# underdoc-wang/STC-GNN

Measured on AMD Instinct MI355X. Metric: STC-GNN fwd+bwd samples/sec at N=50k,C=32; SpMM HBM GB/s vs peak, 1/8 GPU, higher is better.
Workload: dtype f32; 1 GPU; full STC-GNN train step (fwd + ComboLoss + bwd + grad all-reduce + Adam), csr-fixed, 224x224 queen grid N=50176 nnz=398724, C=32, hidden=16, K=2, layers=2, T=18+6; global_batch=8, batch_per_gpu=8, parallelism=batch-shard x1, operand_format=f16x2, grad_bucket_bytes=88132, grad_large_bytes=0, input_seeds=X, Y: Bernoulli(0.1635), torch seed 1000 + rank

## Files before the change

### include/stc_hip.h

```cpp
#ifndef STC_HIP_H
#define STC_HIP_H

#include <stddef.h>
#include <stdint.h>

#ifdef __cplusplus
extern "C" {
#endif

#define STC_ABI_VERSION 37
#define STC_MAX_K 4

#define STC_FMT_BF16X3 0
#define STC_FMT_F16X2 1
#define STC_ACT_AMAX_SLOTS 256

#define STC_OK 0
#define STC_EINVAL (-1)
#define STC_EALIGN (-2)
#define STC_ELIMIT (-3)
#define STC_EUNSUPPORTED (-4)

int stc_version(void);
const char* stc_last_error(void);
int stc_set_dispatch_level(int32_t level);

int stc_csr_spmm_f32(const int32_t* rowptr, const int32_t* colidx, const float* val,
                     int32_t n_rows, int32_t n_cols,
                     const float* X, const float* Y0, float* Y,
                     int32_t batch, int32_t F, float alpha, float beta, void* stream);

#define STC_SPMM_BLOCK_ROWS 4
int stc_bcsr_spmm_f32(const int32_t* blk_ptr, const int32_t* blk_cols, const float* blk_vals,
                      int32_t n_rows, int32_t n_cols,
                      const float* X, const float* Y0, float* Y,
                      int32_t batch, int32_t F, float alpha, float beta, void* stream);

#define STC_PATCH_ROWS 32
#define STC_PATCH_MAX_SRC 64
#define STC_PATCH_MAX_WIDTH 32
int stc_patch_spmm_f32(const int32_t* patch_src, const int32_t* patch_rows, const int32_t* patch_cnt,
                       const uint8_t* patch_idx, const float* patch_val, int32_t n_patches, int32_t width,
                       int32_t n_rows, int32_t n_cols, const float* X, const float* Y0, float* Y,
                       int32_t batch, int32_t F, float alpha, float beta, void* stream);

int stc_csr_spmm_bf16(const int32_t* rowptr, const int32_t* colidx, const float* val,
                      int32_t n_rows, int32_t n_cols,
                      const void* X, const void* Y0, void* Y,
                      int32_t batch, int32_t F, float alpha, float beta, void* stream);
int stc_bcsr_spmm_bf16(const int32_t* blk_ptr, const int32_t* blk_cols, const float* blk_vals,
                       int32_t n_rows, int32_t n_cols,
                       const void* X, const void* Y0, void* Y,
                       int32_t batch, int32_t F, float alpha, float beta, void* stream);

int stc_patch_spmm_bf16(const int32_t* patch_src, const int32_t* patch_rows, const int32_t* patch_cnt,
                        const uint8_t* patch_idx, const float* patch_val, int32_t n_patches, int32_t width,
                        int32_t n_rows, int32_t n_cols, const void* X, const void* Y0, void* Y,
                        int32_t batch, int32_t F, float alpha, float beta, void* stream);

#define STC_RING2_INTERIOR 32
#define STC_RING2_FIRST 64
#define STC_RING2_SECOND 96
#define STC_RING2_WIDTH 8
int stc_ring2_sum_f32(const int32_t* l2_rows, const int32_t* l1_rows, const int32_t* int_rows, const int32_t* t1, const int32_t* t2,
                      int32_t n_patches, int32_t n_rows,
                      const float* A, const float* A2, int32_t n_add, const float* const* add,
                      const float* U, const float* Cand, float* Y, float* Z,
                      int32_t batch, int32_t C, int32_t h, void* stream);
int stc_ring2_blend_f32(const int32_t* l2_rows, const int32_t* l1_rows, const int32_t* int_rows, const int32_t* t1, const int32_t* t2,
                        int32_t n_patches, int32_t n_rows,
                        const float* Bm, const float* A, const float* U, const float* H,
                        float* Cand, float* Hnew, float* SHnew,
                        int32_t batch, int32_t C, int32_t h, void* stream);
int stc_ring2_blend_first_f32(const int32_t* l2_rows, const int32_t* l1_rows, const int32_t* int_rows, const int32_t* t1, const int32_t* t2,
                              int32_t n_patches, int32_t n_rows,
                              const float* Bm, const float* A, const float* U,
                              float* Cand, float* Hnew, float* SHnew,
                              int32_t batch, int32_t C, int32_t h, void* stream);
int stc_ring2_chain_f32(const int32_t* l2_rows, const int32_t* l1_rows, const int32_t* int_rows, const int32_t* t1, const int32_t* t2,
                        int32_t n_patches, int32_t n_rows,
                        const float* A, const float* A2, float alpha1, int32_t n_add1, const float* const* add1, float* V,
                        float alpha2, int32_t n_add0, const float* const* add0, const float* scale0, float* Z,
                        int32_t batch, int32_t C, int32_t h, void* stream);

int stc_bdg_node_bf16_supported(int32_t Ks, int32_t Kc, int32_t C, int32_t L, int32_t Ho);
int stc_bdg_node_fwd_bf16(const void* const* Z, int32_t Ks, const float* Tc, int32_t Kc,
                          const float* W, const float* bias, void* Y,
                          int64_t nodes, int32_t C, int32_t L, int32_t Lw, int32_t Ho, void* stream);
int stc_bdg_node_bwd_bf16(const void* const* Z, int32_t Ks, const float* Tc, int32_t Kc,
                          const float* W, const void* dY,
                          void* const* dZ, float* dW, float* db,
                          void* workspace, size_t workspace_bytes,
                          int64_t nodes, int32_t C, int32_t L, int32_t Lw, int32_t Ho, void* stream);

int stc_cell_planar_bf16_supported(int32_t Ks, int32_t Kc, int32_t C, int32_t h);
int stc_cell_gates_fwd_planar_bf16(const void* X, const void* H, const void* SX, const void* SH,
                                   const float* Tc, const float* W, const float* bias,
                                   void* U, void* Rg, void* RH,
                                   const float* Wc, const float* bc, void* A, void* Bm,
                                   int64_t nodes, int32_t C, int32_t Lw, int32_t h, void* stream);
int stc_cell_gates_bwd_planar_bf16(const void* X, const void* H, const void* SX, const void* SH,
                                   const float* Tc, const float* W,
                                   const void* dCandIn, const void* Cand, const void* U, const void* Rg, const void* dHnew,
                                   void* const* dZ, float* dW, float* db, void* dH,
                                   void* workspace, size_t workspace_bytes,
                                   int64_t nodes, int32_t C, int32_t Lw, int32_t h, void* stream);
int stc_cell_bwd_planar_bf16_supported(int32_t C, int32_t Lw, int32_t h);
int stc_cell_bwd_planar_bf16(const void* X, const void* H, const void* SX, const void* SH,
                             const float* Tc, const float* Wg, const float* Wc,
                             const void* U, const void* Rg, const void* Cand, const void* dHnew, const void* dBm,
                             void* dX, void* dSX, void* dH, void* dSH,
                             float* dWg, float* dbg, float* dWc, float* dbc,
                             void* workspace, size_t workspace_bytes,
                             int64_t nodes, int32_t C, int32_t Lw, int32_t h, void* stream);
int stc_bdg_node_post_bwd_bf16(const void* X, const void* X2, const float* Tc, const float* W, const void* dA, const void* dB,
                               void* dX, void* dX2, float* dW, float* db, void* workspace, size_t workspace_bytes,
                               int64_t nodes, int32_t C, int32_t Lw, int32_t Ho, void* stream);
int stc_spmm_blend_fwd_bf16(const int32_t* rowptr, const int32_t* colidx, const float* val,
                            const int32_t* blk_ptr, const int32_t* blk_cols, const float* blk_vals,
                            int32_t n_rows, int32_t n_cols, const void* Bm, const void* A,
                            const void* U, const void* H, void* Cand, void* Hnew,
                            int32_t batch, int32_t C, int32_t h, void* stream);
int stc_spmm_sum_bf16(const int32_t* rowptr, const int32_t* colidx, const float* val,
                      const int32_t* blk_ptr, const int32_t* blk_cols, const float* blk_vals,
                      int32_t n_rows, int32_t n_cols, const void* X, const void* X2,
                      int32_t n_add, const void* const* add,
                      void* Y, const void* U, const void* Cand, void* dY,
                      int32_t batch, int32_t C, int32_t h, void* stream);
int stc_gru_blend_bwd_bf16(const void* dHnew, const void* U, const void* Cand, void* dCpre, int64_t n, void* stream);
int stc_head_fwd_bf16(const void* H, const float* w, const float* b, float* y, int64_t rows, int32_t h, void* stream);
int stc_head_bwd_bf16(const void* H, const float* w, const float* y, const float* dy, void* dH, float* dwb,
                      void* workspace, size_t workspace_bytes, int64_t rows, int32_t h, void* stream);

int stc_dense_agg_f32(const float* S, int32_t n_rows, int32_t n_cols, const float* X, const float* Y0, float* Y,
                      int32_t batch, int32_t F, float alpha, float beta, void* stream);

int stc_csr_sddmm_f32(const int32_t* rowptr, const int32_t* colidx,
                      int32_t n_rows, int32_t n_cols,
                      const float* A, const float* Bm, float* out,
                      int32_t batch, int32_t F, float alpha, int32_t accumulate, void* stream);

int stc_cheby_dense_fwd_f32(const float* G, int32_t n, int32_t K, float* T, void* stream);
int stc_cheby_dense_bwd_f32(const float* G, const float* T, float* dT, int32_t n, int32_t K,
                            float* dG, void* stream);

int stc_bdg_node_fwd_f32(const float* const* Z, int32_t Ks, const float* Tc, int32_t Kc,
                         const float* W, const float* bias, float* Y,
                         int64_t nodes, int32_t C, int32_t L, int32_t Lw, int32_t Ho, void* stream);

size_t stc_bdg_node_bwd_workspace_bytes(int32_t Ks, int32_t Kc, int32_t C, int32_t L, int32_t Ho,
                                        int32_t want_dTc);
int stc_bdg_node_bwd_f32(const float* const* Z, int32_t Ks, const float* Tc, int32_t Kc,
                         const float* W, const float* dY,
                         float* const* dZ, float* dW, float* db, float* dTc,
                         void* workspace, size_t workspace_bytes,
                         int64_t nodes, int32_t C, int32_t L, int32_t Lw, int32_t Ho, void* stream);

int stc_gru_gates_fwd_f32(const float* G, const float* Xt, const float* H,
                          float* U, float* Rg, float* CandIn,
                          int64_t rows, int32_t cin, int32_t h, int32_t pad, void* stream);
int stc_gru_gates_bwd_f32(const float* dCandIn, const float* dU, const float* H,
// ... 45 lines not shown
                           float* copy1, int32_t copy1_ld, int32_t copy1_off,
                           int64_t nodes, int32_t C, int32_t L, int32_t Lw, int32_t h, void* stream);

int stc_cell_planar_supported(int32_t Ks, int32_t Kc, int32_t C, int32_t h);
int stc_cell_gates_fwd_planar_f32(const float* X, const float* H, const float* SX, const float* SH,
                                  const float* Tc, const float* W, const float* bias,
                                  float* U, float* Rg, float* RH,
                                  const float* Wc, const float* bc, float* A, float* Bm,
                                  int32_t operand_format,
                                  float* act_amax,
                                  int64_t nodes, int32_t C, int32_t Lw, int32_t h, void* stream);
int stc_cell_gates_bwd_planar_f32(const float* X, const float* H, const float* SX, const float* SH,
                                  const float* Tc, const float* W,
                                  const float* dCandIn, const float* Cand, const float* U, const float* Rg, const float* dHnew,
                                  float* const* dZ, float* dW, float* db, float* dH,
                                  int32_t operand_format,
                                  const float* act_amax,
                                  void* workspace, size_t workspace_bytes,
                                  int64_t nodes, int32_t C, int32_t Lw, int32_t h, void* stream);

int stc_cell_bwd_planar_supported(int32_t C, int32_t h);
size_t stc_cell_bwd_planar_workspace_bytes(int32_t C, int32_t Lw, int32_t h);
int stc_cell_bwd_planar_f32(const float* X, const float* H, const float* SX, const float* SH,
                            const float* Tc, const float* Wg, const float* Wc,
                            const float* U, const float* Rg, const float* Cand, const float* dHnew, const float* dBm,
                            float* dX, float* dSX, float* dH, float* dSH,
                            float* dWg, float* dbg, float* dWc, float* dbc,
                            int32_t accumulate_x, int32_t accumulate_h,
                            int32_t operand_format, const float* act_amax,
                            void* workspace, size_t workspace_bytes,
                            int64_t nodes, int32_t C, int32_t Lw, int32_t h, void* stream);

int stc_cell_first_supported(int32_t C, int32_t h);
int stc_cell_gates_fwd_first_f32(const float* X, const float* SX, const float* Tc, const float* W, const float* bias, float* U,
                                 const float* Wc, const float* bc, float* A, float* Bm,
                                 int32_t operand_format, float* act_amax,
                                 int64_t nodes, int32_t C, int32_t Lw, int32_t h, void* stream);
size_t stc_cell_bwd_first_workspace_bytes(int32_t C, int32_t Lw, int32_t h);
int stc_cell_bwd_first_f32(const float* X, const float* SX, const float* Tc, const float* Wg, const float* Wc,
                           const float* U, const float* Cand, const float* dHnew, const float* dBm,
                           float* dX, float* dSX, float* dWg, float* dbg, float* dWc, float* dbc,
                           int32_t accumulate_x, int32_t operand_format, const float* act_amax,
                           void* workspace, size_t workspace_bytes,
                           int64_t nodes, int32_t C, int32_t Lw, int32_t h, void* stream);

int stc_cell_planar_k_supported(int32_t K, int32_t C, int32_t h);
int stc_cell_gates_fwd_planar_k_f32(const float* const* Zx, const float* const* Zh, int32_t K, const float* Tc, const float* W, const float* bias,
                                    float* U, float* Rg, float* RH, int32_t operand_format,
                                    float* act_amax,
                                    int64_t nodes, int32_t C, int32_t Lw, int32_t h, void* stream);
int stc_cell_cand_fwd_planar_k_f32(const float* const* Zx, const float* const* Zh, int32_t K, const float* Tc, const float* W, const float* bias,
                                   const float* U, const float* H, float* Cand, float* Hnew, int32_t operand_format, float* act_amax,
                                   int64_t nodes, int32_t C, int32_t Lw, int32_t h, void* stream);
int stc_cell_gates_bwd_planar_k_f32(const float* const* Zx, const float* const* Zh, int32_t K, const float* Tc, const float* W,
                                    const float* dRH, const float* Cand, const float* U, const float* Rg, const float* dHnew,
                                    float* const* dZx, float* const* dZh, float* dW, float* db, float* dH, int32_t accumulate_x,
                                    int32_t operand_format,
                                    const float* act_amax,
                                    void* workspace, size_t workspace_bytes, int64_t nodes, int32_t C, int32_t Lw, int32_t h, void* stream);
int stc_cell_cand_bwd_planar_k_f32(const float* const* Zx, const float* const* Zh, int32_t K, const float* Tc, const float* W,
                                   const float* dHnew, const float* U, const float* Cand,
                                   float* const* dZx, float* const* dZh, float* dW, float* db,
                                   int32_t operand_format,
                                   const float* act_amax,
                                   void* workspace, size_t workspace_bytes, int64_t nodes, int32_t C, int32_t Lw, int32_t h, void* stream);

#define STC_SPMM_SUM_MAX_ADD 8
#define STC_SPMM_SUM_BF16_MAX_ADD 5
#define STC_RING2_MAX_ADD 5
int stc_spmm_sum_f32(const int32_t* rowptr, const int32_t* colidx, const float* val,
                     const int32_t* blk_ptr, const int32_t* blk_cols, const float* blk_vals,
                     int32_t n_rows, int32_t n_cols, const float* X, const float* X2, float alpha,
                     int32_t n_add, const float* const* add, const int32_t* add_ld, const int32_t* add_off, const float* add_scale,
                     float* Y, const float* U, const float* Cand, float* dY,
                     float* amax, int32_t n_amax,
                     int32_t batch, int32_t C, int32_t h, void* stream);

int stc_head_fwd_f32(const float* H, const float* w, const float* b, float* y,
                     int64_t rows, int32_t h, void* stream);
size_t stc_head_bwd_workspace_bytes(int32_t h);
int stc_head_bwd_f32(const float* H, const float* w, const float* y, const float* dy,
                     float* dH, float* dwb, void* workspace, size_t workspace_bytes,
                     int64_t rows, int32_t h, void* stream);

int stc_cell_small_supported(int32_t Ks, int32_t Kc, int32_t C, int32_t cin, int32_t h);
size_t stc_cell_small_workspace_bytes(int32_t n_nodes, int32_t C, int32_t cin, int32_t batch, int32_t Ks);
int stc_cell_small_param_rows(void);
int stc_cell_small_fwd_f32(const int32_t* rowptr, const int32_t* colidx, const float* val, int32_t n_nodes, int32_t nnz,
                           int32_t graph_is_dense, const int32_t* rowptr2, const int32_t* colidx2, const float* val2, int32_t nnz2,
                           const float* X, int32_t cin, const float* H, const float* Tc, int32_t Ks, int32_t Kc,
                           const float* Wg, const float* bg, const float* Wc, const float* bc,
                           float* U, float* R, float* Cand, float* Hnew, float* RH, float* Zg, float* Zc, float* Zg2, float* Zc2, float* Z0,
                           float* Z0c, float* Z1c, float* Z2c, int32_t phase, int32_t splits, int32_t batch, int32_t C, void* stream);
int stc_cell_small_bwd_f32(const int32_t* rowptr, const int32_t* colidx, const float* val, int32_t n_nodes, int32_t nnz,
                           int32_t graph_is_dense, const int32_t* rowptr2, const int32_t* colidx2, const float* val2, int32_t nnz2,
                           const float* X, int32_t cin, const float* H, const float* Tc, int32_t Ks, int32_t Kc,
                           const float* Wg, const float* Wc, const float* U, const float* R, const float* Cand,
                           const float* RH, const float* Zg, const float* Zc, const float* Zg2, const float* Zc2, const float* dHnew,
                           float* dX, int32_t accumulate_x, float* dH, int32_t accumulate_h,
                           float* dparams, int64_t params_ld, int32_t has_bg, int32_t has_bc,
                           float* dZ1c, float* dZ1g, float* dYg, float* dYc, float* dZ2c, float* dZ2g,
                           void* workspace, size_t workspace_bytes, int32_t phase, int32_t splits, int32_t batch, int32_t C, void* stream);

int stc_graph_grad_f32(const float* A, const float* B, double* partials, int32_t n_chunks, int32_t cell0, int32_t cell_step, int32_t n_sel,
                       int32_t batch, int32_t N, int32_t F, int64_t chunk_stride, void* stream);
int stc_mix_grad_f32(const float* A, const float* B, double* partials, int32_t n_chunks, int32_t cell0, int32_t cell_step, int32_t n_sel,
                     int32_t batch, int32_t N, int32_t Fa, int32_t Fb, int64_t chunk_stride, void* stream);

int stc_mix_dt_supported(int32_t Ks, int32_t Kc, int32_t C, int32_t L, int32_t Ho);
size_t stc_mix_dt_workspace_bytes(int32_t Ks);
int stc_mix_dt_f32(const float* const* Z, int32_t Ks, const float* W, const float* dY, float* dTc, void* workspace,
                   size_t workspace_bytes, int64_t rows, int32_t C, int32_t L, int32_t Lw, int32_t Ho, void* stream);

size_t stc_mixed_fusion_workspace_bytes(int32_t D, int32_t want_dA);
int stc_mixed_fusion_fwd_f32(const float* WA, const float* bA, const float* WP, const float* bP, const float* A, const float* P,
                             float* gate, float* G, int32_t D, void* stream);
int stc_mixed_fusion_bwd_f32(const float* WA, const float* WP, const float* A, const float* P, const float* gate, const float* dG,
                             float* dWA, float* dWP, float* db, float* dP, float* dA,
                             void* workspace, size_t workspace_bytes, int32_t D, void* stream);
int stc_mgp_uv_fwd_f32(const float* X, int64_t k_stride, int64_t r_stride, int64_t f_stride, const float* Wu, const float* Wv, float alpha,
                       float* U, float* V, int32_t K, int32_t R, int32_t F, int32_t h, void* stream);
int stc_mgp_uv_bwd_f32(const float* X, int64_t k_stride, int64_t r_stride, int64_t f_stride, const float* U, const float* V,
                       const float* dU, const float* dV, float alpha, float* partials, int32_t K, int32_t R, int32_t F, int32_t h, void* stream);
int stc_mgp_softmax_fwd_f32(const float* P, float* Ps, int32_t R, void* stream);
int stc_mgp_softmax_bwd_f32(const float* P, const float* Ps, const float* dPs, float* rowdot, float* dP, int32_t R, void* stream);
int stc_adam_f32(float* p, const float* g, float* m, float* v, int64_t n, const float* step, double lr, double beta1, double beta2, double eps,
                 double weight_decay, void* stream);


int stc_axpy_f32(float a, const float* x, float* y, int64_t n, void* stream);
int stc_concat2_f32(const float* A, const float* B, float* out,
                    int64_t rows, int32_t a, int32_t b, int32_t pad, void* stream);
int stc_split2_f32(const float* src, const float* addA, const float* addB, float* A, float* B,
                   int64_t rows, int32_t a, int32_t b, int32_t pad, int32_t addA_ld,
                   const float* addA2, const float* addB2, void* stream);

#ifdef __cplusplus
}
#endif
#endif
```

### stc-gnn_amd/STC_GNN.py

```python
from __future__ import annotations

from typing import List, Optional, Sequence, Union

import torch
from torch import nn

from stc_hip import ops
from stc_hip.graph import CsrGraph, SpatialOperand, csr_operand, dense_operand

GraphLike = Union[torch.Tensor, CsrGraph, 'GraphPair']


class GraphPair:

    def __init__(self, Gs, Gc: torch.Tensor, Ks: int, Kc: int):
        if isinstance(Gs, CsrGraph):
            self.spatial: SpatialOperand = csr_operand(Gs, Gc.device)
        elif isinstance(Gs, torch.Tensor) and Gs.layout != torch.strided:
            self.spatial = csr_operand(_as_csr_graph(Gs), Gc.device)
        elif isinstance(Gs, torch.Tensor):
            self.spatial = dense_operand(Gs)
        else:
            raise TypeError(f'Gs must be a tensor or a CsrGraph, got {type(Gs).__name__}')
        self.Ks, self.Kc = Ks, Kc
# ... 196 lines not shown
        params = nn.ParameterDict()
        for key in ('Wu', 'Wv'):
            params[key] = nn.Parameter(torch.randn(in_dim, hidden_dim))
        for p in params.values():
            nn.init.xavier_normal_(p)
        return params

    def _learned(self, X: torch.Tensor, params, rows_axis: int) -> torch.Tensor:
        reduce = None
        if self.batch_sharded:
            from stc_hip.dist import allreduce_sum
            reduce = allreduce_sum
        if ops.mgp_front_supported(X, params['Wu'], params['Wv']):
            return ops.mgp_front(X, params['Wu'], params['Wv'], rows_axis, float(self.alpha), reduce)
        if rows_axis == 3:
            X = X.transpose(2, 3)
        U = torch.tanh(self.alpha * torch.matmul(X, params['Wu']))
        V = torch.tanh(self.alpha * torch.matmul(X, params['Wv']))
        flat_u, flat_v = U.flatten(0, 1), V.flatten(0, 1)
        P = torch.einsum('knh,kmh->nm', flat_u, flat_v)
        if reduce is not None:
            P = reduce(P)
        return torch.softmax(torch.relu(P - P.t()), dim=-1)

    def forward(self, X_seq: torch.Tensor, As: torch.Tensor, Ac: torch.Tensor):
        Gs = self.aggreg_S(As, self._learned(X_seq, self.params_S, 2))
        Gc = self.aggreg_C(Ac, self._learned(X_seq, self.params_C, 3))
        return Gs, Gc


class STCGNN(nn.Module):

    def __init__(self, num_nodes: int, num_categories: int, Ks: int, Kc: int, input_dim: int, hidden_dim: int,
                 num_layers: int, out_horizon: int, use_bias=True, activation=None,
                 graph_mode: str = 'dense-learned', reorder_nodes: bool = True, batch_sharded: bool = False,
                 fusion_rank: Optional[int] = None, storage_dtype: torch.dtype = torch.float32):
        super().__init__()
        if graph_mode not in ('dense-learned', 'csr-fixed'):
            raise ValueError("graph_mode must be 'dense-learned' (reference semantics) or 'csr-fixed'")
        if storage_dtype not in (torch.float32, torch.bfloat16):
            raise ValueError('storage_dtype must be torch.float32 (reference arithmetic) or torch.bfloat16')
        if storage_dtype == torch.bfloat16 and graph_mode != 'csr-fixed':
            raise ValueError("storage_dtype=torch.bfloat16 needs graph_mode='csr-fixed' (BASELINE configuration 5)")
        self.storage_dtype = storage_dtype
        self.graph_mode = graph_mode
        self.reorder_nodes = reorder_nodes
        self.Ks, self.Kc = Ks, Kc
        if graph_mode == 'dense-learned':
            self.mix_graph_pair = MGP_Gen(num_nodes, num_categories, hidden_dim, fusion_rank=fusion_rank)
            self.mix_graph_pair.batch_sharded = batch_sharded
        self.encoder = STC_Encoder(num_nodes, num_categories, Ks, Kc, input_dim, hidden_dim, num_layers,
                                   use_bias, activation, return_all_layers=True)
        self.decoder = STC_Decoder(num_nodes, num_categories, Ks, Kc, hidden_dim, hidden_dim, num_layers,
                                   out_horizon, use_bias, activation)
        self.out_proj = nn.Sequential(nn.Linear(hidden_dim, hidden_dim // 2, bias=use_bias),
                                      nn.Linear(hidden_dim // 2, input_dim, bias=use_bias))

    def prepare_graph(self, graph: CsrGraph, device=None) -> CsrGraph:
        g = graph.with_locality()[0] if self.reorder_nodes else graph
        if device is not None:
            g.on(torch.device(device))
        return graph

    def forward(self, X_seq: torch.Tensor, As: GraphLike, Ac: torch.Tensor):
        assert X_seq.dim() == 4, 'STC-GNN must take in 4D tensor as input X_seq'
        inv = None
        if self.graph_mode == 'dense-learned':
            Gs, Gc = self.mix_graph_pair(X_seq, As, Ac)
        else:
            Gs, Gc = As, Ac
            if isinstance(Gs, torch.Tensor) and Gs.layout != torch.strided:
                Gs = _as_csr_graph(Gs)
            if self.reorder_nodes and isinstance(Gs, CsrGraph):
                Gs, order = Gs.with_locality()
                if order is not None:
                    idx = getattr(Gs, '_order_dev', {}).get(X_seq.device)
                    if idx is None:
                        o = torch.from_numpy(order).to(X_seq.device)
                        idx = (o, torch.argsort(o))
                        Gs._order_dev = {**getattr(Gs, '_order_dev', {}), X_seq.device: idx}
                    X_seq = X_seq.index_select(2, idx[0])
                    inv = idx[1]
        pair = _graphs(Gs, Gc, self.Ks, self.Kc)
        stacked = self._run_cell_graph(pair, X_seq.unsqueeze(-1).to(self.storage_dtype))
        if stacked is None and self.storage_dtype != torch.float32:
            raise ValueError('storage_dtype=torch.bfloat16: shape outside the bf16 cell kernels (Ks = Kc = 2, hidden 16, C in {32, 64}, input_dim <= 4)')
        if stacked is not None:
            y = self._head(stacked).transpose(0, 1)
        else:
            _, states = self.encoder._run(pair, None, X_seq.unsqueeze(-1))
            step_in = states[-1]
            outs = []
            for _ in range(self.decoder.out_horizon):
                step_in, states = self.decoder(pair, None, step_in, states)
                outs.append(step_in)
            y = self._head(torch.stack(outs, dim=1))
        return y if inv is None else y.index_select(2, inv)

    def _run_cell_graph(self, pair: GraphPair, X: torch.Tensor):
        enc, dec = self.encoder.cell_list, self.decoder.cell_list
        cells = list(enc) + list(dec)
        hidden = {c.hidden_dim for c in cells}
        if len(hidden) != 1 or any(c.gates.activation is not None or c.candi.activation is not None for c in cells):
            return None
        h = hidden.pop()
        B, T, N, C, cin0 = X.shape
        if X.requires_grad or not ops.cell_graph_supported(pair.spatial, pair.Tc, self.Ks, C, h, [cin0, h], dtype=X.dtype):
            return None
        n_layers, horizon = len(enc), self.decoder.out_horizon
        if ops.first_step_route(pair.spatial, pair.Tc, self.Ks, C, h, [cin0, h], dtype=X.dtype):
            ext = [X[:, t] for t in range(T)] + [ops.zero_state(c.gates.W, (B, c.num_nodes, c.num_categories, c.hidden_dim), X.dtype) for c in enc]
        else:
            ext = [X[:, t] for t in range(T)] + [c.init_hidden(B).to(X.dtype) for c in enc]
        eid = lambda l, t: l * T + t
        did = lambda l, s_: n_layers * T + s_ * n_layers + l
        schedule = []
        for l in range(n_layers):
            for t in range(T):
                x = ('ext', t) if l == 0 else ('cell', eid(l - 1, t))
                hs = ('ext', T + l) if t == 0 else ('cell', eid(l, t - 1))
                schedule.append((l, x, hs))
        for s_ in range(horizon):
            for l in range(n_layers):
                top_prev = eid(n_layers - 1, T - 1) if s_ == 0 else did(n_layers - 1, s_ - 1)
                x = ('cell', top_prev) if l == 0 else ('cell', did(l - 1, s_))
                hs = ('cell', eid(l, T - 1) if s_ == 0 else did(l, s_ - 1))
                schedule.append((n_layers + l, x, hs))
        stacks = [(c.gates.W, c.gates.b if c.gates.use_bias else None, c.candi.W, c.candi.b if c.candi.use_bias else None) for c in cells]
        outputs = [did(n_layers - 1, s_) for s_ in range(horizon)]
        return ops.stc_cell_graph(pair.spatial, pair.Tc, self.Ks, schedule, outputs, ext, stacks)

    def _head(self, H: torch.Tensor) -> torch.Tensor:
        lin1, lin2 = self.out_proj[0], self.out_proj[1]
        h = lin1.in_features
        if lin2.out_features != 1 or h % 4 or h > 64 or (H.dtype == torch.bfloat16 and h != 16):
            return torch.sigmoid(self.out_proj(H.float())).squeeze(dim=-1)
        w = (lin2.weight @ lin1.weight).reshape(h)
        if lin1.bias is not None:
            b = lin2.weight @ lin1.bias + lin2.bias
        else:
            b = w.new_zeros(1)
        return ops.head(H, w, b)
```

### stc-gnn_amd/csrc/stc_common.h

```cpp
#pragma once
#include <hip/hip_runtime.h>

#include <atomic>
#include <cstdarg>
#include <cstdint>
#include <cstdio>

#include "stc_hip.h"

namespace stc {

char* error_buffer();

inline int fail(int code, const char* fmt, ...) {
    va_list ap;
    va_start(ap, fmt);
    vsnprintf(error_buffer(), 512, fmt, ap);
    va_end(ap);
    return code;
}

inline int hip_status(hipError_t e, const char* what) {
    if (e == hipSuccess) return STC_OK;
    snprintf(error_buffer(), 512, "%s: %s", what, hipGetErrorString(e));
// ... 3 lines not shown
inline bool aligned16(const void* p) { return (reinterpret_cast<uintptr_t>(p) & 15u) == 0; }

constexpr int kNumXcd = 8;
constexpr int kNumCu = 256;
constexpr int kWave = 64;
constexpr size_t kMaxLdsBytes = 160 * 1024;

template <typename K>
inline hipError_t allow_lds(K kernel, size_t bytes) {
    if (bytes <= 48 * 1024) return hipSuccess;
    return hipFuncSetAttribute(reinterpret_cast<const void*>(kernel),
                               hipFuncAttributeMaxDynamicSharedMemorySize, (int)bytes);
}

constexpr int kMaxGrantDevices = 16;
struct Grants { std::atomic<size_t> per_device[kMaxGrantDevices]; };
template <class K>
inline hipError_t allow_lds_once(K kern, size_t bytes, Grants& grants) {
    int dev = -1;
    if (hipGetDevice(&dev) != hipSuccess) dev = -1;
    std::atomic<size_t>* granted = dev >= 0 && dev < kMaxGrantDevices ? &grants.per_device[dev] : nullptr;
    if (granted && bytes <= granted->load(std::memory_order_relaxed)) return hipSuccess;
    const hipError_t e = allow_lds(kern, bytes);
    if (e == hipSuccess && granted) granted->store(bytes, std::memory_order_relaxed);
    return e;
}

template <typename K>
inline int resident_blocks(K kernel, int threads, size_t lds, int fallback_per_cu = 1) {
    int per_cu = 0, dev = 0, cus = kNumCu;
    bool failed = false;
    if (hipOccupancyMaxActiveBlocksPerMultiprocessor(&per_cu, kernel, threads, lds) != hipSuccess || per_cu < 1) {
        per_cu = fallback_per_cu;
        failed = true;
    }
    if (hipGetDevice(&dev) == hipSuccess) {
        int v = 0;
        if (hipDeviceGetAttribute(&v, hipDeviceAttributeMultiprocessorCount, dev) == hipSuccess && v > 0) cus = v;
        else failed = true;
    } else {
        failed = true;
    }
    if (failed) (void)hipGetLastError();
    return per_cu * cus;
}

#define STC_REQUIRE(cond, code, ...) \
    do {                             \
        if (!(cond)) return ::stc::fail(code, __VA_ARGS__); \
    } while (0)

#define STC_LAUNCH_CHECK(what) \
    do {                        \
        hipError_t e__ = hipGetLastError(); \
        if (e__ != hipSuccess) return ::stc::hip_status(e__, what); \
    } while (0)

}

__device__ __forceinline__ int stc_xcd_tile(int bid, int n_tiles) {
    const int per = (n_tiles + stc::kNumXcd - 1) / stc::kNumXcd;
    const int tile = (bid % stc::kNumXcd) * per + bid / stc::kNumXcd;
    return tile < n_tiles && (bid / stc::kNumXcd) < per ? tile : -1;
}

template <class T>
__device__ __forceinline__ T stc_ld_once(const T* p) { return __builtin_nontemporal_load(p); }
template <class T>
__device__ __forceinline__ void stc_st_once(T* p, const T& v) { __builtin_nontemporal_store(v, p); }

__device__ __forceinline__ float stc_sigmoid(float v) {
    return __builtin_amdgcn_rcpf(1.f + __builtin_amdgcn_exp2f(-1.4426950408889634f * v));
}
__device__ __forceinline__ float stc_tanh(float v) {
    const float big = 1.f - 2.f * __builtin_amdgcn_rcpf(1.f + __builtin_amdgcn_exp2f(2.8853900817779268f * v));
    const float t = v * v;
    float p = fmaf(t, 62.f / 2835.f, -17.f / 315.f);
    p = fmaf(p, t, 2.f / 15.f);
    p = fmaf(p, t, -1.f / 3.f);
    const float small = fmaf(p * t, v, v);
    return fabsf(v) < 0.25f ? small : big;
}

__device__ __forceinline__ float stc_wave_sum(float v) {
#pragma unroll
    for (int off = 32; off > 0; off >>= 1) v += __shfl_xor(v, off, 64);
    return v;
}
```

### stc-gnn_amd/csrc/stc_gates.hip

```cpp
#include "stc_common.h"

#include <initializer_list>

namespace {

constexpr int EW_THREADS = 256;

inline dim3 ew_grid(long long n) {
    long long blocks = (n + EW_THREADS - 1) / EW_THREADS;
    const long long cap = (long long)stc::kNumCu * 8;
    return dim3((unsigned)(blocks < cap ? (blocks > 0 ? blocks : 1) : cap));
}

__device__ __forceinline__ float sigmoidf_(float x) { return 1.f / (1.f + expf(-x)); }

__global__ __launch_bounds__(EW_THREADS) void gru_gates_fwd_kernel(
    const float* __restrict__ G, const float* __restrict__ Xt, const float* __restrict__ H,
    float* __restrict__ U, float* __restrict__ Rg, float* __restrict__ CandIn,
    long long rows, int cin, int h, int pad) {
    const int L = cin + h + pad;
    const long long n = rows * L;
    for (long long e = (long long)blockIdx.x * EW_THREADS + threadIdx.x; e < n; e += (long long)gridDim.x * EW_THREADS) {
        const long long r = e / L;
        const int l = (int)(e - r * L);
        if (l < cin) {
            CandIn[e] = Xt[r * cin + l];
        } else if (l >= cin + h) {
            CandIn[e] = 0.f;
        } else {
            const int k = l - cin;
            const float u = sigmoidf_(G[r * 2 * h + k]);
            const float g = sigmoidf_(G[r * 2 * h + h + k]);
            U[r * h + k] = u;
            Rg[r * h + k] = g;
            CandIn[e] = g * H[r * h + k];
        }
    }
}

__global__ __launch_bounds__(EW_THREADS) void gru_gates_bwd_kernel(
    const float* __restrict__ dCandIn, const float* __restrict__ dU, const float* __restrict__ H,
    const float* __restrict__ U, const float* __restrict__ Rg, const float* dH_in,
    float* __restrict__ dG, float* __restrict__ dXt, float* dH,
    long long rows, int cin, int h, int pad) {
    const int L = cin + h + pad;
    const long long n = rows * L;
    for (long long e = (long long)blockIdx.x * EW_THREADS + threadIdx.x; e < n; e += (long long)gridDim.x * EW_THREADS) {
        const long long r = e / L;
        const int l = (int)(e - r * L);
        if (l < cin) {
            dXt[r * cin + l] = dCandIn[e];
        } else if (l < cin + h) {
            const int k = l - cin;
            const long long i = r * h + k;
            const float u = U[i], g = Rg[i], d = dCandIn[e];
            dG[r * 2 * h + k] = dU[i] * u * (1.f - u);
            dG[r * 2 * h + h + k] = d * H[i] * g * (1.f - g);
            dH[i] = dH_in ? fmaf(d, g, dH_in[i]) : d * g;
        }
    }
}

__global__ __launch_bounds__(EW_THREADS) void gru_blend_fwd_kernel(
    const float* __restrict__ Cpre, const float* __restrict__ U, const float* __restrict__ H,
    float* __restrict__ Cand, float* __restrict__ Hnew, long long n) {
    for (long long e = (long long)blockIdx.x * EW_THREADS + threadIdx.x; e < n; e += (long long)gridDim.x * EW_THREADS) {
        const float c = tanhf(Cpre[e]);
        const float u = U[e];
        Cand[e] = c;
        Hnew[e] = (1.f - u) * H[e] + u * c;
    }
}

__global__ __launch_bounds__(EW_THREADS) void gru_blend_bwd_kernel(
    const float* __restrict__ dHnew, const float* __restrict__ U, const float* __restrict__ H,
    const float* __restrict__ Cand, float* __restrict__ dCpre, float* __restrict__ dU, float* __restrict__ dH,
    long long n) {
    for (long long e = (long long)blockIdx.x * EW_THREADS + threadIdx.x; e < n; e += (long long)gridDim.x * EW_THREADS) {
        const float g = dHnew[e], u = U[e], c = Cand[e];
        dCpre[e] = g * u * (1.f - c * c);
        if (dU) dU[e] = g * (c - H[e]);
        if (dH) dH[e] = g * (1.f - u);
    }
}


__device__ __forceinline__ float4 sig4(float4 x) { return make_float4(sigmoidf_(x.x), sigmoidf_(x.y), sigmoidf_(x.z), sigmoidf_(x.w)); }
__device__ __forceinline__ float4 mul4(float4 a, float4 b) { return make_float4(a.x * b.x, a.y * b.y, a.z * b.z, a.w * b.w); }

__global__ __launch_bounds__(EW_THREADS) void gru_gates_fwd_vec_kernel(
    const float4* __restrict__ G, const float4* __restrict__ Xt, const float4* __restrict__ H,
    float4* __restrict__ U, float4* __restrict__ Rg, float4* __restrict__ CandIn,
    long long rows, int cin4, int h4, int pad4) {
    const int L4 = cin4 + h4 + pad4;
    const long long n = rows * L4;
    for (long long e = (long long)blockIdx.x * EW_THREADS + threadIdx.x; e < n; e += (long long)gridDim.x * EW_THREADS) {
        const long long r = e / L4;
// ... 79 lines not shown
}

__device__ __forceinline__ float4 add4(float4 a, float4 b) { return make_float4(a.x + b.x, a.y + b.y, a.z + b.z, a.w + b.w); }

__global__ __launch_bounds__(EW_THREADS) void split2_vec_kernel(const float4* __restrict__ src, const float4* addA, const float4* addB,
                                                                 float4* A, float4* B, long long rows, int a4, int b4, int pad4, int ldA4,
                                                                 const float4* addA2, const float4* addB2) {
    const int L4 = a4 + b4 + pad4;
    const long long n = rows * L4;
    for (long long e = (long long)blockIdx.x * EW_THREADS + threadIdx.x; e < n; e += (long long)gridDim.x * EW_THREADS) {
        const long long r = e / L4;
        const int l = (int)(e - r * L4);
        if (l < a4) {
            if (A) {
                const long long i = r * a4 + l;
                float4 v = addA ? add4(src[e], addA[r * ldA4 + l]) : src[e];
                if (addA2) v = add4(v, addA2[i]);
                A[i] = v;
            }
        } else if (l < a4 + b4) {
            if (B) {
                const long long i = r * b4 + (l - a4);
                float4 v = addB ? add4(src[e], addB[i]) : src[e];
                if (addB2) v = add4(v, addB2[i]);
                B[i] = v;
            }
        }
    }
}

inline bool vec_ok(std::initializer_list<const void*> ptrs, std::initializer_list<long long> widths) {
    for (const void* p : ptrs)
        if (p && !stc::aligned16(p)) return false;
    for (long long w : widths)
        if (w % 4) return false;
    return true;
}
#define F4C(p) reinterpret_cast<const float4*>(p)
#define F4M(p) reinterpret_cast<float4*>(p)

constexpr int HEAD_MAX_H = 64;
constexpr int HEAD_PARTS = 1024;

template <int LPR>
__global__ __launch_bounds__(EW_THREADS) void head_fwd_kernel(const float* __restrict__ H, const float* __restrict__ w,
                                                               const float* __restrict__ b, float* __restrict__ y,
                                                               long long rows, int h) {
    constexpr int RPB = EW_THREADS / LPR;
    const int h4 = h / 4, q = threadIdx.x % LPR;
    float4 wq = make_float4(0.f, 0.f, 0.f, 0.f);
    if (q < h4) wq = reinterpret_cast<const float4*>(w)[q];
    const float bias = b[0];
    for (long long r = (long long)blockIdx.x * RPB + threadIdx.x / LPR; r < rows; r += (long long)gridDim.x * RPB) {
        float s = 0.f;
        if (q < h4) {
            const float4 v = reinterpret_cast<const float4*>(H + r * h)[q];
            s = fmaf(v.x, wq.x, fmaf(v.y, wq.y, fmaf(v.z, wq.z, v.w * wq.w)));
        }
#pragma unroll
        for (int off = LPR / 2; off > 0; off >>= 1) s += __shfl_xor(s, off, 64);
        if (q == 0) y[r] = sigmoidf_(s + bias);
    }
}

template <int LPR>
__global__ __launch_bounds__(EW_THREADS) void head_bwd_kernel(const float* __restrict__ H, const float* __restrict__ w,
                                                               const float* __restrict__ y, const float* __restrict__ dy,
                                                               float* __restrict__ dH, float* __restrict__ partial,
                                                               long long rows, int h) {
    constexpr int RPB = EW_THREADS / LPR;
    __shared__ float red[EW_THREADS][5];
    const int h4 = h / 4, q = threadIdx.x % LPR;
    float4 wq = make_float4(0.f, 0.f, 0.f, 0.f);
    if (q < h4) wq = reinterpret_cast<const float4*>(w)[q];
    float4 acc = make_float4(0.f, 0.f, 0.f, 0.f);
    float accg = 0.f;
    for (long long r = (long long)blockIdx.x * RPB + threadIdx.x / LPR; r < rows; r += (long long)gridDim.x * RPB) {
        const float yy = y[r];
        const float g = dy[r] * yy * (1.f - yy);
        if (q == 0) accg += g;
        if (q < h4) {
            const float4 v = reinterpret_cast<const float4*>(H + r * h)[q];
            reinterpret_cast<float4*>(dH + r * h)[q] = make_float4(g * wq.x, g * wq.y, g * wq.z, g * wq.w);
            acc.x = fmaf(g, v.x, acc.x); acc.y = fmaf(g, v.y, acc.y); acc.z = fmaf(g, v.z, acc.z); acc.w = fmaf(g, v.w, acc.w);
        }
    }
    red[threadIdx.x][0] = acc.x; red[threadIdx.x][1] = acc.y; red[threadIdx.x][2] = acc.z; red[threadIdx.x][3] = acc.w;
    red[threadIdx.x][4] = accg;
    __syncthreads();
    if ((int)threadIdx.x <= h) {
        const int k = threadIdx.x;
        const int lane_q = k < h ? k / 4 : 0, comp = k < h ? k % 4 : 4;
        float v = 0.f;
        for (int t = lane_q; t < EW_THREADS; t += LPR) v += red[t][comp];
        partial[(size_t)blockIdx.x * (h + 1) + k] = v;
    }
}

using head_u4 = __attribute__((ext_vector_type(4))) unsigned;
using head_bf2 = __attribute__((ext_vector_type(2))) __bf16;
__device__ __forceinline__ void head_unpack8(const head_u4 v, float (&r)[8]) {
#pragma unroll
    for (int i = 0; i < 4; ++i) { r[2 * i] = __uint_as_float(v[i] << 16); r[2 * i + 1] = __uint_as_float(v[i] & 0xffff0000u); }
}
__device__ __forceinline__ unsigned head_pk(float a, float b) {
    const head_bf2 v = {(__bf16)a, (__bf16)b};
    return __builtin_bit_cast(unsigned, v);
}

__global__ __launch_bounds__(EW_THREADS) void head_fwd_bf16_kernel(const head_u4* __restrict__ H, const float* __restrict__ w,
                                                                    const float* __restrict__ b, float* __restrict__ y, long long rows) {
    constexpr int RPB = EW_THREADS / 2;
    const int q = threadIdx.x & 1;
    float wq[8];
#pragma unroll
    for (int i = 0; i < 8; ++i) wq[i] = w[8 * q + i];
    const float bias = b[0];
    for (long long r = (long long)blockIdx.x * RPB + threadIdx.x / 2; r < rows; r += (long long)gridDim.x * RPB) {
        float v[8];
        head_unpack8(H[2 * r + q], v);
        float s = 0.f;
#pragma unroll
        for (int i = 0; i < 8; ++i) s = fmaf(v[i], wq[i], s);
        s += __shfl_xor(s, 1, 64);
        if (q == 0) y[r] = sigmoidf_(s + bias);
    }
}

__global__ __launch_bounds__(EW_THREADS) void head_bwd_bf16_kernel(const head_u4* __restrict__ H, const float* __restrict__ w,
                                                                    const float* __restrict__ y, const float* __restrict__ dy,
                                                                    head_u4* __restrict__ dH, float* __restrict__ partial, long long rows) {
    constexpr int RPB = EW_THREADS / 2, h = 16;
    __shared__ float red[EW_THREADS][9];
    const int q = threadIdx.x & 1;
    float wq[8], acc[8], accg = 0.f;
#pragma unroll
    for (int i = 0; i < 8; ++i) { wq[i] = w[8 * q + i]; acc[i] = 0.f; }
    for (long long r = (long long)blockIdx.x * RPB + threadIdx.x / 2; r < rows; r += (long long)gridDim.x * RPB) {
        const float yy = y[r];
        const float g = dy[r] * yy * (1.f - yy);
        if (q == 0) accg += g;
        float v[8];
        head_unpack8(H[2 * r + q], v);
        dH[2 * r + q] = head_u4{head_pk(g * wq[0], g * wq[1]), head_pk(g * wq[2], g * wq[3]), head_pk(g * wq[4], g * wq[5]), head_pk(g * wq[6], g * wq[7])};
#pragma unroll
        for (int i = 0; i < 8; ++i) acc[i] = fmaf(g, v[i], acc[i]);
    }
#pragma unroll
    for (int i = 0; i < 8; ++i) red[threadIdx.x][i] = acc[i];
    red[threadIdx.x][8] = accg;
    __syncthreads();
    if ((int)threadIdx.x <= h) {
        const int k = threadIdx.x;
        const int lane_q = k < h ? k / 8 : 0, comp = k < h ? k % 8 : 8;
        float v = 0.f;
        for (int t = lane_q; t < EW_THREADS; t += 2) v += red[t][comp];
        partial[(size_t)blockIdx.x * (h + 1) + k] = v;
    }
}

__global__ __launch_bounds__(EW_THREADS) void head_reduce_kernel(const float* __restrict__ partial, int n_parts, int stride, float* __restrict__ out) {
    __shared__ float red[EW_THREADS];
    const int e = blockIdx.x;
    float s = 0.f;
    for (int p = threadIdx.x; p < n_parts; p += EW_THREADS) s += partial[(size_t)p * stride + e];
    red[threadIdx.x] = s;
// ... 107 lines not shown
        hipLaunchKernelGGL(gru_gates_fwd_kernel, ew_grid(n), dim3(EW_THREADS), 0, s, G, Xt, H, U, Rg, CandIn, (long long)rows, cin, h, pad);
    STC_LAUNCH_CHECK("stc_gru_gates_fwd_f32 launch");
    return STC_OK;
}

extern "C" int stc_gru_gates_bwd_f32(const float* dCandIn, const float* dU, const float* H, const float* U, const float* Rg,
                                     const float* dH_in, float* dG, float* dXt, float* dH,
                                     int64_t rows, int32_t cin, int32_t h, int32_t pad, void* stream) {
    STC_REQUIRE(cin >= 0 && h >= 1 && pad >= 0, STC_EINVAL, "stc_gru_gates_bwd_f32: bad widths cin=%d h=%d pad=%d", cin, h, pad);
    STC_EW_PROLOGUE("stc_gru_gates_bwd_f32", rows, dCandIn && dU && H && U && Rg && dG && dH && (cin == 0 || dXt));
    const long long n = (long long)rows * (cin + h + pad);
    if (vec_ok({dCandIn, dU, H, U, Rg, dH_in, dG, dXt, dH}, {cin, h, pad}))
        hipLaunchKernelGGL(gru_gates_bwd_vec_kernel, ew_grid(n / 4), dim3(EW_THREADS), 0, s, F4C(dCandIn), F4C(dU), F4C(H), F4C(U), F4C(Rg),
                           F4C(dH_in), F4M(dG), F4M(dXt), F4M(dH), (long long)rows, cin / 4, h / 4, pad / 4);
    else
        hipLaunchKernelGGL(gru_gates_bwd_kernel, ew_grid(n), dim3(EW_THREADS), 0, s, dCandIn, dU, H, U, Rg, dH_in, dG, dXt, dH, (long long)rows, cin, h, pad);
    STC_LAUNCH_CHECK("stc_gru_gates_bwd_f32 launch");
    return STC_OK;
}

extern "C" int stc_gru_blend_fwd_f32(const float* Cpre, const float* U, const float* H, float* Cand, float* Hnew,
                                     int64_t n, void* stream) {
    STC_EW_PROLOGUE("stc_gru_blend_fwd_f32", n, Cpre && U && H && Cand && Hnew);
    if (vec_ok({Cpre, U, H, Cand, Hnew}, {n}))
        hipLaunchKernelGGL(gru_blend_fwd_vec_kernel, ew_grid(n / 4), dim3(EW_THREADS), 0, s, F4C(Cpre), F4C(U), F4C(H), F4M(Cand), F4M(Hnew), (long long)n / 4);
    else
        hipLaunchKernelGGL(gru_blend_fwd_kernel, ew_grid(n), dim3(EW_THREADS), 0, s, Cpre, U, H, Cand, Hnew, (long long)n);
    STC_LAUNCH_CHECK("stc_gru_blend_fwd_f32 launch");
    return STC_OK;
}

extern "C" int stc_gru_blend_bwd_f32(const float* dHnew, const float* U, const float* H, const float* Cand,
                                     float* dCpre, float* dU, float* dH, int64_t n, void* stream) {
    STC_EW_PROLOGUE("stc_gru_blend_bwd_f32", n, dHnew && U && Cand && dCpre && (H || !dU));
    if (vec_ok({dHnew, U, H, Cand, dCpre, dU, dH}, {n}))
        hipLaunchKernelGGL(gru_blend_bwd_vec_kernel, ew_grid(n / 4), dim3(EW_THREADS), 0, s, F4C(dHnew), F4C(U), F4C(H), F4C(Cand), F4M(dCpre), F4M(dU),
                           F4M(dH), (long long)n / 4);
    else
        hipLaunchKernelGGL(gru_blend_bwd_kernel, ew_grid(n), dim3(EW_THREADS), 0, s, dHnew, U, H, Cand, dCpre, dU, dH, (long long)n);
    STC_LAUNCH_CHECK("stc_gru_blend_bwd_f32 launch");
    return STC_OK;
}


extern "C" int stc_head_fwd_f32(const float* H, const float* w, const float* b, float* y, int64_t rows, int32_t h, void* stream) {
    STC_REQUIRE(h >= 4 && h <= HEAD_MAX_H && h % 4 == 0, STC_ELIMIT, "stc_head_fwd_f32: h=%d must be a multiple of 4 in [4,%d]", h, HEAD_MAX_H);
    STC_EW_PROLOGUE("stc_head_fwd_f32", rows, H && w && b && y);
    STC_REQUIRE(stc::aligned16(H), STC_EALIGN, "stc_head_fwd_f32: H not 16-byte aligned");
    STC_REQUIRE(stc::aligned16(w), STC_EALIGN, "stc_head_fwd_f32: w not 16-byte aligned");
    const int h4 = h / 4;
#define STC_HEAD_FWD(LPR_) hipLaunchKernelGGL(head_fwd_kernel<LPR_>, ew_grid(rows * LPR_), dim3(EW_THREADS), 0, s, H, w, b, y, (long long)rows, h)
    if (h4 <= 1) STC_HEAD_FWD(1); else if (h4 <= 2) STC_HEAD_FWD(2); else if (h4 <= 4) STC_HEAD_FWD(4); else if (h4 <= 8) STC_HEAD_FWD(8); else STC_HEAD_FWD(16);
#undef STC_HEAD_FWD
    STC_LAUNCH_CHECK("stc_head_fwd_f32 launch");
    return STC_OK;
}

extern "C" size_t stc_head_bwd_workspace_bytes(int32_t h) { return h < 1 ? 0 : (size_t)HEAD_PARTS * (h + 1) * sizeof(float); }

extern "C" int stc_head_bwd_f32(const float* H, const float* w, const float* y, const float* dy, float* dH, float* dwb,
                                void* workspace, size_t workspace_bytes, int64_t rows, int32_t h, void* stream) {
    STC_REQUIRE(h >= 4 && h <= HEAD_MAX_H && h % 4 == 0, STC_ELIMIT, "stc_head_bwd_f32: h=%d must be a multiple of 4 in [4,%d]", h, HEAD_MAX_H);
    STC_REQUIRE(rows >= 0 && dwb, STC_EINVAL, "stc_head_bwd_f32: negative rows or null dwb");
    hipStream_t s = static_cast<hipStream_t>(stream);
    if (rows == 0) return stc::hip_status(hipMemsetAsync(dwb, 0, (size_t)(h + 1) * sizeof(float), s), "memset dwb");
    STC_REQUIRE(H && w && y && dy && dH, STC_EINVAL, "stc_head_bwd_f32: null pointer");
    STC_REQUIRE(stc::aligned16(H) && stc::aligned16(dH) && workspace && stc::aligned16(workspace), STC_EALIGN,
                "stc_head_bwd_f32: H/dH/workspace must be 16-byte aligned");
    STC_REQUIRE(workspace_bytes >= stc_head_bwd_workspace_bytes(h), STC_EINVAL, "stc_head_bwd_f32: workspace too small");
    STC_REQUIRE(stc::aligned16(w), STC_EALIGN, "stc_head_bwd_f32: w not 16-byte aligned");
    const int h4 = h / 4;
    const int lpr = h4 <= 1 ? 1 : h4 <= 2 ? 2 : h4 <= 4 ? 4 : h4 <= 8 ? 8 : 16;
    long long blocks = (rows * lpr + EW_THREADS - 1) / EW_THREADS;
    const int grid = (int)(blocks < HEAD_PARTS ? blocks : HEAD_PARTS);
    float* partial = static_cast<float*>(workspace);
#define STC_HEAD_BWD(LPR_) hipLaunchKernelGGL(head_bwd_kernel<LPR_>, dim3(grid), dim3(EW_THREADS), 0, s, H, w, y, dy, dH, partial, (long long)rows, h)
    if (lpr == 1) STC_HEAD_BWD(1); else if (lpr == 2) STC_HEAD_BWD(2); else if (lpr == 4) STC_HEAD_BWD(4); else if (lpr == 8) STC_HEAD_BWD(8); else STC_HEAD_BWD(16);
#undef STC_HEAD_BWD
    hipLaunchKernelGGL(head_reduce_kernel, dim3(h + 1), dim3(EW_THREADS), 0, s, partial, grid, h + 1, dwb);
    STC_LAUNCH_CHECK("stc_head_bwd_f32 launch");
    return STC_OK;
}

extern "C" int stc_head_fwd_bf16(const void* H, const float* w, const float* b, float* y, int64_t rows, int32_t h, void* stream) {
    STC_REQUIRE(h == 16, STC_EUNSUPPORTED, "stc_head_fwd_bf16: hidden width %d (built for 16)", h);
    STC_EW_PROLOGUE("stc_head_fwd_bf16", rows, H && w && b && y);
    STC_REQUIRE(stc::aligned16(H), STC_EALIGN, "stc_head_fwd_bf16: H not 16-byte aligned");
    hipLaunchKernelGGL(head_fwd_bf16_kernel, ew_grid(rows * 2), dim3(EW_THREADS), 0, s, static_cast<const head_u4*>(H), w, b, y, (long long)rows);
    STC_LAUNCH_CHECK("stc_head_fwd_bf16 launch");
    return STC_OK;
}

extern "C" int stc_head_bwd_bf16(const void* H, const float* w, const float* y, const float* dy, void* dH, float* dwb,
                                 void* workspace, size_t workspace_bytes, int64_t rows, int32_t h, void* stream) {
    STC_REQUIRE(h == 16, STC_EUNSUPPORTED, "stc_head_bwd_bf16: hidden width %d (built for 16)", h);
    STC_REQUIRE(rows >= 0 && dwb, STC_EINVAL, "stc_head_bwd_bf16: negative rows or null dwb");
    hipStream_t s = static_cast<hipStream_t>(stream);
    if (rows == 0) return stc::hip_status(hipMemsetAsync(dwb, 0, (size_t)(h + 1) * sizeof(float), s), "memset dwb");
    STC_REQUIRE(H && w && y && dy && dH, STC_EINVAL, "stc_head_bwd_bf16: null pointer");
    STC_REQUIRE(stc::aligned16(H) && stc::aligned16(dH) && workspace && stc::aligned16(workspace), STC_EALIGN,
                "stc_head_bwd_bf16: H/dH/workspace must be 16-byte aligned");
    STC_REQUIRE(workspace_bytes >= stc_head_bwd_workspace_bytes(h), STC_EINVAL, "stc_head_bwd_bf16: workspace too small");
    long long blocks = (rows * 2 + EW_THREADS - 1) / EW_THREADS;
    const int grid = (int)(blocks < HEAD_PARTS ? blocks : HEAD_PARTS);
    float* partial = static_cast<float*>(workspace);
    hipLaunchKernelGGL(head_bwd_bf16_kernel, dim3(grid), dim3(EW_THREADS), 0, s, static_cast<const head_u4*>(H), w, y, dy,
                       static_cast<head_u4*>(dH), partial, (long long)rows);
    hipLaunchKernelGGL(head_reduce_kernel, dim3(h + 1), dim3(EW_THREADS), 0, s, partial, grid, h + 1, dwb);
    STC_LAUNCH_CHECK("stc_head_bwd_bf16 launch");
    return STC_OK;
}

extern "C" int stc_axpy_f32(float a, const float* x, float* y, int64_t n, void* stream) {
    STC_EW_PROLOGUE("stc_axpy_f32", n, x && y);
    hipLaunchKernelGGL(axpy_kernel, ew_grid(n), dim3(EW_THREADS), 0, s, a, x, y, (long long)n);
    STC_LAUNCH_CHECK("stc_axpy_f32 launch");
    return STC_OK;
}

extern "C" int stc_concat2_f32(const float* A, const float* B, float* out, int64_t rows, int32_t a, int32_t b, int32_t pad, void* stream) {
    STC_REQUIRE(a >= 0 && b >= 0 && pad >= 0, STC_EINVAL, "stc_concat2_f32: negative width");
    const long long n = (long long)rows * (a + b + pad);
    STC_EW_PROLOGUE("stc_concat2_f32", n, out && (a == 0 || A) && (b == 0 || B));
    if (vec_ok({A, B, out}, {a, b, pad}))
        hipLaunchKernelGGL(concat2_vec_kernel, ew_grid(n / 4), dim3(EW_THREADS), 0, s, F4C(A), F4C(B), F4M(out), (long long)rows, a / 4, b / 4, pad / 4);
    else
        hipLaunchKernelGGL(concat2_kernel, ew_grid(n), dim3(EW_THREADS), 0, s, A, B, out, (long long)rows, a, b, pad);
    STC_LAUNCH_CHECK("stc_concat2_f32 launch");
    return STC_OK;
}

extern "C" int stc_split2_f32(const float* src, const float* addA, const float* addB, float* A, float* B,
                              int64_t rows, int32_t a, int32_t b, int32_t pad, int32_t addA_ld,
                              const float* addA2, const float* addB2, void* stream) {
    STC_REQUIRE(a >= 0 && b >= 0 && pad >= 0, STC_EINVAL, "stc_split2_f32: negative width");
    STC_REQUIRE(addA_ld == 0 || addA_ld >= a, STC_EINVAL, "stc_split2_f32: addA_ld=%d is smaller than the width a=%d", addA_ld, a);
    const int ldA = addA_ld ? addA_ld : a;
    const long long n = (long long)rows * (a + b + pad);
    STC_EW_PROLOGUE("stc_split2_f32", n, src && (A || B));
    if (vec_ok({src, addA, addB, A, B, addA2, addB2}, {a, b, pad, ldA}))
        hipLaunchKernelGGL(split2_vec_kernel, ew_grid(n / 4), dim3(EW_THREADS), 0, s, F4C(src), F4C(addA), F4C(addB), F4M(A), F4M(B),
                           (long long)rows, a / 4, b / 4, pad / 4, ldA / 4, F4C(addA2), F4C(addB2));
    else
        hipLaunchKernelGGL(split2_kernel, ew_grid(n), dim3(EW_THREADS), 0, s, src, addA, addB, A, B, (long long)rows, a, b, pad, ldA, addA2, addB2);
    STC_LAUNCH_CHECK("stc_split2_f32 launch");
    return STC_OK;
}

extern "C" int stc_cheby_dense_fwd_f32(const float* G, int32_t n, int32_t K, float* T, void* stream) {
    STC_REQUIRE(n >= 1 && n <= 128 && K >= 1 && K <= STC_MAX_K, STC_ELIMIT, "stc_cheby_dense_fwd_f32: n=%d (<=128) K=%d (<=%d)", n, K, STC_MAX_K);
    STC_REQUIRE(G && T, STC_EINVAL, "stc_cheby_dense_fwd_f32: null pointer");
    hipStream_t s = static_cast<hipStream_t>(stream);
    const int nn = n * n;
    const dim3 grid((nn + EW_THREADS - 1) / EW_THREADS), block(EW_THREADS);
    hipLaunchKernelGGL(cheby_init_kernel, grid, block, 0, s, G, n, K, T);
    for (int k = 2; k < K; ++k)
        hipLaunchKernelGGL(cheby_step_kernel, grid, block, 0, s, G, T + (size_t)(k - 1) * nn, T + (size_t)(k - 2) * nn, T + (size_t)k * nn, n);
    STC_LAUNCH_CHECK("stc_cheby_dense_fwd_f32 launch");
    return STC_OK;
}

extern "C" int stc_cheby_dense_bwd_f32(const float* G, const float* T, float* dT, int32_t n, int32_t K, float* dG, void* stream) {
    STC_REQUIRE(n >= 1 && n <= 128 && K >= 1 && K <= STC_MAX_K, STC_ELIMIT, "stc_cheby_dense_bwd_f32: n=%d (<=128) K=%d (<=%d)", n, K, STC_MAX_K);
    STC_REQUIRE(G && T && dT && dG, STC_EINVAL, "stc_cheby_dense_bwd_f32: null pointer");
    hipStream_t s = static_cast<hipStream_t>(stream);
    const int nn = n * n;
// ... 24 lines not shown
```

### stc-gnn_amd/csrc/stc_spmm_ring2.hip

```cpp
#include "stc_spmm_host.h"

namespace {

constexpr int R2_THREADS = 256, R2_WAVES = R2_THREADS / 64;
constexpr int R2_INT = STC_RING2_INTERIOR;
constexpr int R2_L1 = STC_RING2_FIRST;
constexpr int R2_L2 = STC_RING2_SECOND;
constexpr int R2_W = STC_RING2_WIDTH;
constexpr int R2_Q = 32;
constexpr int R2_STAGE = R2_L2 / (2 * R2_WAVES);
constexpr int R2_S1 = R2_L1 / (2 * R2_WAVES);
constexpr int R2_S2 = R2_INT / (2 * R2_WAVES);
constexpr int R2_MAX_ADD = STC_RING2_MAX_ADD;

using v4f = __attribute__((ext_vector_type(4))) float;

struct Ring2Plan {
    const int32_t *l2_rows, *l1_rows, *int_rows;
    const int32_t *t1, *t2;
    int n_patches;
};

struct Ring2Args {
    Ring2Plan pl;
    const v4f *A, *A2;
    const v4f* add[R2_MAX_ADD];
    int n_add;
    const v4f *U, *Cand;
    v4f *Y, *Y2, *Z;
    int n, F4;
    float alpha1, alpha2;
    const v4f* add0[R2_MAX_ADD];
    float scale0[R2_MAX_ADD];
};

enum { R2_SUM = 0, R2_BLEND = 1, R2_CHAIN = 2, R2_BLEND0 = 3 };

__device__ __forceinline__ void lds_only_barrier() { asm volatile("s_waitcnt lgkmcnt(0)\n\ts_barrier" ::: "memory"); }

template <int MODE, bool HAS_A2, int NADD, int N0 = 0>
__global__ __launch_bounds__(R2_THREADS, 2) void ring2_sum_kernel(Ring2Args a) {
    static_assert((MODE != R2_BLEND && MODE != R2_BLEND0) || (NADD == 1 && !HAS_A2), "the blend forms: one addend (A), one gathered operand (Bm)");
    static_assert((MODE == R2_CHAIN) == (N0 > 0), "interior addends: the chain form, at least one");
    extern __shared__ __attribute__((aligned(16))) unsigned char lds[];
    v4f* tile = reinterpret_cast<v4f*>(lds);
    int2* tab1 = reinterpret_cast<int2*>(lds + (size_t)R2_L2 * R2_Q * 16);
    int2* tab2 = tab1 + R2_L1 * R2_W;

    const int p = stc_xcd_tile(blockIdx.x, a.pl.n_patches);
    if (p < 0) return;
    const int b = blockIdx.y;
    const int tid = threadIdx.x, lane = tid & 63, half = lane >> 5, q = lane & 31;
    const int wave = __builtin_amdgcn_readfirstlane(tid >> 6);
    const int hw = wave * 2 + half;
    const int n_chunks = a.F4 / R2_Q;

    for (int e = tid; e < R2_L1 * R2_W; e += R2_THREADS) tab1[e] = reinterpret_cast<const int2*>(a.pl.t1)[(size_t)p * R2_L1 * R2_W + e];
    for (int e = tid; e < R2_INT * R2_W; e += R2_THREADS) tab2[e] = reinterpret_cast<const int2*>(a.pl.t2)[(size_t)p * R2_INT * R2_W + e];

    int stage_row[R2_STAGE], l1_row[R2_S1], in_row[R2_S2];
#pragma unroll
    for (int k = 0; k < R2_STAGE; ++k) stage_row[k] = a.pl.l2_rows[(size_t)p * R2_L2 + k * 8 + hw];
#pragma unroll
    for (int i = 0; i < R2_S1; ++i) l1_row[i] = a.pl.l1_rows[(size_t)p * R2_L1 + i * 8 + hw];
#pragma unroll
    for (int i = 0; i < R2_S2; ++i) in_row[i] = a.pl.int_rows[(size_t)p * R2_INT + i * 8 + hw];

    const unsigned base = (unsigned)b * (unsigned)a.n * (unsigned)a.F4 + (unsigned)q;
    unsigned stage_off[R2_STAGE], l1_off[R2_S1];
#pragma unroll
    for (int k = 0; k < R2_STAGE; ++k) stage_off[k] = base + (unsigned)stage_row[k] * (unsigned)a.F4;
#pragma unroll
    for (int i = 0; i < R2_S1; ++i) l1_off[i] = base + (unsigned)(l1_row[i] >= 0 ? (l1_row[i] & 0x3FFFFFFF) : 0) * (unsigned)a.F4;
    v4f st[R2_STAGE];
    auto request = [&](int chunk) {
#pragma unroll
        for (int k = 0; k < R2_STAGE; ++k) {
            const unsigned at = stage_off[k] + chunk * R2_Q;
            st[k] = a.A[at];
            if (HAS_A2) st[k] += a.A2[at];
        }
    };
    constexpr int NOP = MODE == R2_CHAIN ? NADD : MODE == R2_BLEND0 ? NADD + 1 : NADD + 2, NOPA = NOP > 0 ? NOP : 1;
    auto slot_at = [&](int i, int chunk) { return l1_off[i] + (unsigned)(chunk * R2_Q); };
    auto request_slot = [&](v4f (&o)[NOPA], int i, int chunk) {
        const unsigned at = slot_at(i, chunk);
#pragma unroll
        for (int k = 0; k < NADD; ++k) o[k] = a.add[k][at];
        if constexpr (MODE != R2_CHAIN) {
            o[NADD] = a.U[at];
            if constexpr (MODE != R2_BLEND0) o[NADD + 1] = a.Cand[at];
        }
    };
    v4f opn[NOPA];
    request(0);
    request_slot(opn, 0, 0);
    for (int chunk = 0; chunk < n_chunks; ++chunk) {
        if (chunk) lds_only_barrier();
#pragma unroll
        for (int k = 0; k < R2_STAGE; ++k) tile[(k * 8 + hw) * R2_Q + q] = st[k];
        lds_only_barrier();
        const bool more = chunk + 1 < n_chunks;
        v4f dy[R2_S1];
#pragma unroll
        for (int i = 0; i < R2_S1; ++i) {
            const int slot = i * 8 + hw, row = l1_row[i];
            const bool interior = row >= 0 && (row & (1 << 30));
            v4f cur[NOPA];
#pragma unroll
            for (int k = 0; k < NOP; ++k) cur[k] = opn[k];
            if (i + 1 < R2_S1) {
                request_slot(opn, i + 1, chunk);
            } else if (more) {
                request(chunk + 1);
                request_slot(opn, 0, chunk + 1);
            }
            v4f acc = {0.f, 0.f, 0.f, 0.f};
#pragma unroll
            for (int w = 0; w < R2_W; ++w) {
                const int2 t = tab1[slot * R2_W + w];
                const v4f x = *reinterpret_cast<const v4f*>(lds + t.x + q * 16);
                const float v = __int_as_float(t.y);
#pragma unroll
                for (int c = 0; c < 4; ++c) acc[c] = fmaf(v, x[c], acc[c]);
            }
            v4f dh = MODE == R2_CHAIN ? a.alpha1 * acc : acc;
#pragma unroll
            for (int k = 0; k < NADD; ++k) dh += cur[k];
            if constexpr (MODE == R2_CHAIN) {
                if (a.Y != nullptr && interior) __builtin_nontemporal_store(dh, a.Y + slot_at(i, chunk));
                dy[i] = dh;
            } else if constexpr (MODE == R2_SUM) {
                const v4f u = cur[NOPA - 2], cd = cur[NOPA - 1];
                if (interior) __builtin_nontemporal_store(dh, a.Y + slot_at(i, chunk));
#pragma unroll
                for (int c = 0; c < 4; ++c) dy[i][c] = dh[c] * u[c] * (1.f - cd[c] * cd[c]);
            } else {
                const v4f u = cur[NADD], cd = MODE == R2_BLEND0 ? v4f{0.f, 0.f, 0.f, 0.f} : cur[NOPA - 1];
                v4f cand;
#pragma unroll
                for (int c = 0; c < 4; ++c) {
                    cand[c] = stc_tanh(dh[c]);
                    if constexpr (MODE == R2_BLEND0) dy[i][c] = u[c] * cand[c];
                    else dy[i][c] = (1.f - u[c]) * cd[c] + u[c] * cand[c];
                }
                if (interior) {
                    if (a.Y != nullptr) __builtin_nontemporal_store(cand, a.Y + slot_at(i, chunk));
                    __builtin_nontemporal_store(dy[i], a.Y2 + slot_at(i, chunk));
                }
            }
        }
        lds_only_barrier();
#pragma unroll
        for (int i = 0; i < R2_S1; ++i) tile[(i * 8 + hw) * R2_Q + q] = dy[i];
        v4f own[R2_S2][N0 > 0 ? N0 : 1];
        if constexpr (MODE == R2_CHAIN) {
#pragma unroll
            for (int i = 0; i < R2_S2; ++i)
#pragma unroll
                for (int k = 0; k < N0; ++k)
                    own[i][k] = a.add0[k][base + (unsigned)(in_row[i] >= 0 ? in_row[i] : 0) * (unsigned)a.F4 + (unsigned)(chunk * R2_Q)];
        }
        lds_only_barrier();
#pragma unroll
        for (int i = 0; i < R2_S2; ++i) {
            const int r = i * 8 + hw, row = in_row[i];
            v4f acc = {0.f, 0.f, 0.f, 0.f};
#pragma unroll
            for (int w = 0; w < R2_W; ++w) {
                const int2 t = tab2[r * R2_W + w];
                const v4f x = *reinterpret_cast<const v4f*>(lds + t.x + q * 16);
                const float v = __int_as_float(t.y);
#pragma unroll
                for (int c = 0; c < 4; ++c) acc[c] = fmaf(v, x[c], acc[c]);
            }
            if constexpr (MODE == R2_CHAIN) {
                acc *= a.alpha2;
#pragma unroll
                for (int k = 0; k < N0; ++k) acc += a.scale0[k] * own[i][k];
            }
            if (row >= 0) __builtin_nontemporal_store(acc, a.Z + (base + (unsigned)row * (unsigned)a.F4 + (unsigned)(chunk * R2_Q)));
        }
    }
}

template <int MODE, bool HAS_A2>
int launch_ring2(const Ring2Args& a, int batch, hipStream_t s, int n_add0 = 0) {
    const size_t lds = (size_t)R2_L2 * R2_Q * 16 + (size_t)(R2_L1 + R2_INT) * R2_W * sizeof(int2);
    static_assert((size_t)R2_L2 * R2_Q * 16 + (size_t)(R2_L1 + R2_INT) * R2_W * sizeof(int2) <= 64 * 1024, "within the default dynamic-LDS limit: no attribute to set");
    using Kernel = void (*)(Ring2Args);
    Kernel kern = nullptr;
    if constexpr (MODE == R2_BLEND || MODE == R2_BLEND0) {
        kern = ring2_sum_kernel<MODE, false, 1>;
    } else if constexpr (MODE == R2_CHAIN) {
        static constexpr Kernel table[3][R2_MAX_ADD] = {
#define STC_R2_ROW(NA) {ring2_sum_kernel<R2_CHAIN, HAS_A2, NA, 1>, ring2_sum_kernel<R2_CHAIN, HAS_A2, NA, 2>, ring2_sum_kernel<R2_CHAIN, HAS_A2, NA, 3>, \
                        ring2_sum_kernel<R2_CHAIN, HAS_A2, NA, 4>, ring2_sum_kernel<R2_CHAIN, HAS_A2, NA, 5>}
            STC_R2_ROW(0), STC_R2_ROW(1), STC_R2_ROW(2)};
#undef STC_R2_ROW
        kern = table[a.n_add][n_add0 - 1];
    } else {
        switch (a.n_add) {
            case 0: kern = ring2_sum_kernel<R2_SUM, HAS_A2, 0>; break;
            case 1: kern = ring2_sum_kernel<R2_SUM, HAS_A2, 1>; break;
            case 2: kern = ring2_sum_kernel<R2_SUM, HAS_A2, 2>; break;
            case 3: kern = ring2_sum_kernel<R2_SUM, HAS_A2, 3>; break;
            case 4: kern = ring2_sum_kernel<R2_SUM, HAS_A2, 4>; break;
            default: kern = ring2_sum_kernel<R2_SUM, HAS_A2, 5>; break;
        }
    }
    const int per = (a.pl.n_patches + stc::kNumXcd - 1) / stc::kNumXcd;
    hipLaunchKernelGGL(kern, dim3(per * stc::kNumXcd, batch), dim3(R2_THREADS), lds, s, a);
    return stc::launched("stc_ring2 launch");
}

int check_ring2(const char* who, const void* l2_rows, const void* l1_rows, const void* int_rows, const void* t1, const void* t2, int n_patches, int n_rows,
                int batch, int C, int h) {
    STC_REQUIRE(h == 16 && C >= 1 && (C * h) % (4 * R2_Q) == 0, STC_EUNSUPPORTED, "%s: rows of C * h = %d floats (hidden 16, whole 512-byte chunks)", who, C * h);
    STC_REQUIRE(batch <= 65535 && n_patches >= 0, STC_EINVAL, "%s: bad sizes", who);
    if (int rc = stc::check_state_rows(who, n_rows, batch, C, h, true)) return rc;
    STC_REQUIRE((long long)batch * n_rows * (C * h / 4) < (1ll << 28), STC_ELIMIT, "%s: planes of %lld 16-byte pieces (32-bit offsets: < 2^28)", who,
                (long long)batch * n_rows * (C * h / 4));
    if (batch == 0 || n_rows == 0) return STC_OK;
    STC_REQUIRE(n_patches >= 1 && (long long)n_patches * R2_INT >= n_rows, STC_EINVAL, "%s: %d patches cannot cover %d rows", who, n_patches, n_rows);
    STC_REQUIRE(l2_rows && l1_rows && int_rows && t1 && t2, STC_EINVAL, "%s: null plan array", who);
    STC_REQUIRE(reinterpret_cast<uintptr_t>(t1) % 8 == 0 && reinterpret_cast<uintptr_t>(t2) % 8 == 0, STC_EALIGN, "%s: tables must be 8-byte aligned", who);
    return STC_OK;
}

}

#if !defined(STC_RING2_FIRST_UNIT)

extern "C" int stc_ring2_sum_f32(const int32_t* l2_rows, const int32_t* l1_rows, const int32_t* int_rows, const int32_t* t1, const int32_t* t2,
                                 int32_t n_patches, int32_t n_rows,
                                 const float* A, const float* A2, int32_t n_add, const float* const* add,
                                 const float* U, const float* Cand, float* Y, float* Z,
                                 int32_t batch, int32_t C, int32_t h, void* stream) {
    if (int rc = stc::check_addend_count("stc_ring2_sum_f32", "addend", n_add, 0, R2_MAX_ADD, STC_ELIMIT)) return rc;
    if (int rc = check_ring2("stc_ring2_sum_f32", l2_rows, l1_rows, int_rows, t1, t2, n_patches, n_rows, batch, C, h)) return rc;
    if (batch == 0 || n_rows == 0) return STC_OK;
    STC_REQUIRE(A && U && Cand && Y && Z && (n_add == 0 || add), STC_EINVAL, "stc_ring2_sum_f32: null pointer");
    STC_REQUIRE(stc::aligned16(A) && (!A2 || stc::aligned16(A2)) && stc::aligned16(U) && stc::aligned16(Cand) && stc::aligned16(Y) && stc::aligned16(Z),
                STC_EALIGN, "stc_ring2_sum_f32: planes must be 16-byte aligned");
    STC_REQUIRE(Y != A && Y != A2 && Z != A && Z != A2 && Y != Z && Y != U && Y != Cand && Z != U && Z != Cand, STC_EINVAL,
                "stc_ring2_sum_f32: results must not alias the gathered operands, the first ring's gate planes or each other");
    Ring2Args a{};
    a.pl = Ring2Plan{l2_rows, l1_rows, int_rows, t1, t2, n_patches};
    a.A = reinterpret_cast<const v4f*>(A);
    a.A2 = reinterpret_cast<const v4f*>(A2);
    a.n_add = n_add;
    if (int rc = stc::check_addends("stc_ring2_sum_f32", "addend", add, n_add, Y, Z)) return rc;
    for (int i = 0; i < n_add; ++i) a.add[i] = reinterpret_cast<const v4f*>(add[i]);
    a.U = reinterpret_cast<const v4f*>(U);
    a.Cand = reinterpret_cast<const v4f*>(Cand);
    a.Y = reinterpret_cast<v4f*>(Y);
    a.Z = reinterpret_cast<v4f*>(Z);
    a.n = n_rows;
    a.F4 = C * h / 4;
    hipStream_t s = static_cast<hipStream_t>(stream);
    return A2 ? launch_ring2<R2_SUM, true>(a, batch, s) : launch_ring2<R2_SUM, false>(a, batch, s);
}

extern "C" int stc_ring2_blend_f32(const int32_t* l2_rows, const int32_t* l1_rows, const int32_t* int_rows, const int32_t* t1, const int32_t* t2,
                                   int32_t n_patches, int32_t n_rows,
                                   const float* Bm, const float* A, const float* U, const float* H,
                                   float* Cand, float* Hnew, float* SHnew,
                                   int32_t batch, int32_t C, int32_t h, void* stream) {
    if (int rc = check_ring2("stc_ring2_blend_f32", l2_rows, l1_rows, int_rows, t1, t2, n_patches, n_rows, batch, C, h)) return rc;
    if (batch == 0 || n_rows == 0) return STC_OK;
    STC_REQUIRE(Bm && A && U && H && Hnew && SHnew, STC_EINVAL, "stc_ring2_blend_f32: null pointer");
    for (const void* q : {(const void*)Bm, (const void*)A, (const void*)U, (const void*)H, (const void*)Cand, (const void*)Hnew, (const void*)SHnew})
        STC_REQUIRE(stc::aligned16(q), STC_EALIGN, "stc_ring2_blend_f32: planes must be 16-byte aligned");
    for (const float* out : {Cand, Hnew, SHnew})
        STC_REQUIRE(out != Bm && out != A && out != U && out != H, STC_EINVAL, "stc_ring2_blend_f32: a result aliases an operand (the first ring re-reads them)");
    STC_REQUIRE(Cand != Hnew && Cand != SHnew && Hnew != SHnew, STC_EINVAL, "stc_ring2_blend_f32: results alias each other");
    Ring2Args a{};
    a.pl = Ring2Plan{l2_rows, l1_rows, int_rows, t1, t2, n_patches};
    a.A = reinterpret_cast<const v4f*>(Bm);
    a.n_add = 1;
    a.add[0] = reinterpret_cast<const v4f*>(A);
    a.U = reinterpret_cast<const v4f*>(U);
    a.Cand = reinterpret_cast<const v4f*>(H);
    a.Y = reinterpret_cast<v4f*>(Cand);
    a.Y2 = reinterpret_cast<v4f*>(Hnew);
    a.Z = reinterpret_cast<v4f*>(SHnew);
    a.n = n_rows;
    a.F4 = C * h / 4;
    return launch_ring2<R2_BLEND, false>(a, batch, static_cast<hipStream_t>(stream));
}

extern "C" int stc_ring2_chain_f32(const int32_t* l2_rows, const int32_t* l1_rows, const int32_t* int_rows, const int32_t* t1, const int32_t* t2,
                                   int32_t n_patches, int32_t n_rows,
                                   const float* A, const float* A2, float alpha1, int32_t n_add1, const float* const* add1, float* V,
                                   float alpha2, int32_t n_add0, const float* const* add0, const float* scale0, float* Z,
                                   int32_t batch, int32_t C, int32_t h, void* stream) {
    if (int rc = stc::check_addend_count("stc_ring2_chain_f32", "first-ring addend", n_add1, 0, 2, STC_ELIMIT)) return rc;
    if (int rc = stc::check_addend_count("stc_ring2_chain_f32", "interior addend", n_add0, 1, R2_MAX_ADD, STC_ELIMIT)) return rc;
    if (int rc = check_ring2("stc_ring2_chain_f32", l2_rows, l1_rows, int_rows, t1, t2, n_patches, n_rows, batch, C, h)) return rc;
    if (batch == 0 || n_rows == 0) return STC_OK;
    STC_REQUIRE(A && Z && add0 && (n_add1 == 0 || add1), STC_EINVAL, "stc_ring2_chain_f32: null pointer");
    STC_REQUIRE(stc::aligned16(A) && (!A2 || stc::aligned16(A2)) && (!V || stc::aligned16(V)) && stc::aligned16(Z), STC_EALIGN,
                "stc_ring2_chain_f32: planes must be 16-byte aligned");
    STC_REQUIRE(Z != A && Z != A2 && V != A && (!V || V != A2) && V != Z, STC_EINVAL, "stc_ring2_chain_f32: results must not alias the gathered operands or each other");
    Ring2Args a{};
    a.pl = Ring2Plan{l2_rows, l1_rows, int_rows, t1, t2, n_patches};
    a.A = reinterpret_cast<const v4f*>(A);
    a.A2 = reinterpret_cast<const v4f*>(A2);
    a.n_add = n_add1;
    if (int rc = stc::check_addends("stc_ring2_chain_f32", "first-ring addend", add1, n_add1, Z, V)) return rc;
    if (int rc = stc::check_addends("stc_ring2_chain_f32", "interior addend", add0, n_add0, Z, V)) return rc;
    for (int i = 0; i < n_add1; ++i) a.add[i] = reinterpret_cast<const v4f*>(add1[i]);
    for (int i = 0; i < n_add0; ++i) {
        a.add0[i] = reinterpret_cast<const v4f*>(add0[i]);
        a.scale0[i] = scale0 ? scale0[i] : 1.f;
// ... 42 lines not shown
```

### stc-gnn_amd/stc_hip/_lib.py

```python
from __future__ import annotations

import ctypes as C
import os
from typing import Optional, Sequence

import torch

from .graph import is_full_pattern

_PKG_ROOT = os.path.dirname(os.path.dirname(os.path.abspath(__file__)))
LIB_PATH = os.path.join(_PKG_ROOT, 'libstc_hip.so')
ABI_VERSION = 37
FMT_BF16X3, FMT_F16X2 = 0, 1
MAX_K = 4
SPMM_SUM_MAX_ADD, SPMM_SUM_BF16_MAX_ADD, RING2_MAX_ADD = 8, 5, 5
PATCH_ROWS, PATCH_MAX_SRC = 32, 64
RING2_INTERIOR, RING2_FIRST, RING2_SECOND, RING2_WIDTH = 32, 64, 96, 8


class StcError(RuntimeError):
    """A C-ABI call returned non-zero, or the HIP extension cannot be used."""


_p = C.c_void_p
_i32 = C.c_int32
_i64 = C.c_int64
_f32 = C.c_float
_int, _size = C.c_int, C.c_size_t
_pp, _pi, _pf = C.POINTER(_p), C.POINTER(_i32), C.POINTER(_f32)

_ABI = {
    'stc_version': (_int, []),
    'stc_last_error': (C.c_char_p, []),
    'stc_set_dispatch_level': (_int, [_i32]),
    'stc_csr_spmm_f32': (_int, [_p, _p, _p, _i32, _i32, _p, _p, _p, _i32, _i32, _f32, _f32, _p]),
    'stc_bcsr_spmm_f32': (_int, [_p, _p, _p, _i32, _i32, _p, _p, _p, _i32, _i32, _f32, _f32, _p]),
    'stc_patch_spmm_f32': (_int, [_p] * 5 + [_i32] * 4 + [_p, _p, _p, _i32, _i32, _f32, _f32, _p]),
    'stc_patch_spmm_bf16': (_int, [_p] * 5 + [_i32] * 4 + [_p, _p, _p, _i32, _i32, _f32, _f32, _p]),
    'stc_csr_spmm_bf16': (_int, [_p, _p, _p, _i32, _i32, _p, _p, _p, _i32, _i32, _f32, _f32, _p]),
    'stc_bcsr_spmm_bf16': (_int, [_p, _p, _p, _i32, _i32, _p, _p, _p, _i32, _i32, _f32, _f32, _p]),
    'stc_dense_agg_f32': (_int, [_p, _i32, _i32, _p, _p, _p, _i32, _i32, _f32, _f32, _p]),
    'stc_csr_sddmm_f32': (_int, [_p, _p, _i32, _i32, _p, _p, _p, _i32, _i32, _f32, _i32, _p]),
    'stc_ring2_sum_f32': (_int, [_p] * 5 + [_i32, _i32, _p, _p, _i32, _pp, _p, _p, _p, _p, _i32, _i32, _i32, _p]),
    'stc_ring2_blend_f32': (_int, [_p] * 5 + [_i32, _i32] + [_p] * 7 + [_i32, _i32, _i32, _p]),
    'stc_ring2_blend_first_f32': (_int, [_p] * 5 + [_i32, _i32] + [_p] * 6 + [_i32, _i32, _i32, _p]),
    'stc_ring2_chain_f32': (_int, [_p] * 5 + [_i32, _i32, _p, _p, _f32, _i32, _pp, _p, _f32, _i32, _pp, _pf, _p, _i32, _i32, _i32, _p]),
    'stc_spmm_blend_fwd_f32': (_int, [_p] * 6 + [_i32, _i32] + [_p] * 6 + [_p, _i32, _i32, _p, _i32, _p, _i32, _i32] + [_i32] * 3 + [_p]),
    'stc_spmm_blend_fwd_bf16': (_int, [_p] * 6 + [_i32, _i32] + [_p] * 6 + [_i32] * 3 + [_p]),
    'stc_spmm_sum_f32': (_int, [_p] * 6 + [_i32, _i32, _p, _p, _f32, _i32, _pp, _pi, _pi, _pf, _p, _p, _p, _p, _p, _i32, _i32, _i32, _i32, _p]),
    'stc_spmm_sum_bf16': (_int, [_p] * 6 + [_i32, _i32, _p, _p, _i32, _pp, _p, _p, _p, _p, _i32, _i32, _i32, _p]),
    'stc_cheby_dense_fwd_f32': (_int, [_p, _i32, _i32, _p, _p]),
    'stc_cheby_dense_bwd_f32': (_int, [_p, _p, _p, _i32, _i32, _p, _p]),
    'stc_bdg_node_fwd_f32': (_int, [_pp, _i32, _p, _i32, _p, _p, _p, _i64, _i32, _i32, _i32, _i32, _p]),
    'stc_bdg_node_bwd_workspace_bytes': (_size, [_i32, _i32, _i32, _i32, _i32, _i32]),
    'stc_bdg_node_bwd_f32': (_int, [_pp, _i32, _p, _i32, _p, _p, _pp, _p, _p, _p, _p, _size, _i64, _i32, _i32, _i32, _i32, _p]),
    'stc_bdg_node_bf16_supported': (_int, [_i32, _i32, _i32, _i32, _i32]),
    'stc_bdg_node_fwd_bf16': (_int, [_pp, _i32, _p, _i32, _p, _p, _p, _i64, _i32, _i32, _i32, _i32, _p]),
    'stc_bdg_node_bwd_bf16': (_int, [_pp, _i32, _p, _i32, _p, _p, _pp, _p, _p, _p, _size, _i64, _i32, _i32, _i32, _i32, _p]),
    'stc_mix_dt_supported': (_int, [_i32] * 5),
    'stc_mix_dt_workspace_bytes': (_size, [_i32]),
    'stc_mix_dt_f32': (_int, [_pp, _i32, _p, _p, _p, _p, _size, _i64, _i32, _i32, _i32, _i32, _p]),
    'stc_bdg_node_post_supported': (_int, [_i32, _i32, _i32, _i32, _i32]),
    'stc_bdg_node_post_fwd_f32': (_int, [_p, _p, _p, _p, _p, _p, _p, _i64, _i32, _i32, _i32, _i32, _p]),
    'stc_bdg_node_post_bwd_f32': (_int, [_p, _p, _p, _p, _p, _p, _p, _p, _p, _p, _i32, _p, _p, _p, _size, _i64, _i32, _i32, _i32, _i32, _p]),
    'stc_bdg_node_post_bwd_bf16': (_int, [_p] * 11 + [_size, _i64, _i32, _i32, _i32, _p]),
    'stc_cell_planar_supported': (_int, [_i32, _i32, _i32, _i32]),
    'stc_cell_gates_fwd_planar_f32': (_int, [_p] * 14 + [_i32, _p, _i64, _i32, _i32, _i32, _p]),
    'stc_cell_gates_bwd_planar_f32': (_int, [_p] * 11 + [_pp, _p, _p, _p, _i32, _p, _p, _size, _i64, _i32, _i32, _i32, _p]),
    'stc_cell_bwd_planar_supported': (_int, [_i32, _i32]),
    'stc_cell_bwd_planar_workspace_bytes': (_size, [_i32, _i32, _i32]),
    'stc_cell_bwd_planar_f32': (_int, [_p] * 20 + [_i32, _i32, _i32, _p, _p, _size, _i64, _i32, _i32, _i32, _p]),
    'stc_cell_first_supported': (_int, [_i32, _i32]),
    'stc_cell_gates_fwd_first_f32': (_int, [_p] * 10 + [_i32, _p, _i64, _i32, _i32, _i32, _p]),
    'stc_cell_bwd_first_workspace_bytes': (_size, [_i32, _i32, _i32]),
    'stc_cell_bwd_first_f32': (_int, [_p] * 15 + [_i32, _i32, _p, _p, _size, _i64, _i32, _i32, _i32, _p]),
    'stc_cell_planar_bf16_supported': (_int, [_i32, _i32, _i32, _i32]),
    'stc_cell_gates_fwd_planar_bf16': (_int, [_p] * 14 + [_i64, _i32, _i32, _i32, _p]),
    'stc_cell_gates_bwd_planar_bf16': (_int, [_p] * 11 + [_pp, _p, _p, _p, _p, _size, _i64, _i32, _i32, _i32, _p]),
    'stc_cell_bwd_planar_bf16_supported': (_int, [_i32, _i32, _i32]),
    'stc_cell_bwd_planar_bf16': (_int, [_p] * 20 + [_p, _size, _i64, _i32, _i32, _i32, _p]),
    'stc_cell_planar_k_supported': (_int, [_i32, _i32, _i32]),
    'stc_cell_gates_fwd_planar_k_f32': (_int, [_pp, _pp, _i32, _p, _p, _p, _p, _p, _p, _i32, _p, _i64, _i32, _i32, _i32, _p]),
    'stc_cell_cand_fwd_planar_k_f32': (_int, [_pp, _pp, _i32, _p, _p, _p, _p, _p, _p, _p, _i32, _p, _i64, _i32, _i32, _i32, _p]),
    'stc_cell_gates_bwd_planar_k_f32': (_int, [_pp, _pp, _i32, _p, _p, _p, _p, _p, _p, _p, _pp, _pp, _p, _p, _p, _i32, _i32, _p, _p, _size, _i64, _i32, _i32, _i32, _p]),
    'stc_cell_cand_bwd_planar_k_f32': (_int, [_pp, _pp, _i32, _p, _p, _p, _p, _p, _pp, _pp, _p, _p, _i32, _p, _p, _size, _i64, _i32, _i32, _i32, _p]),
    'stc_cell_fused_supported': (_int, [_i32, _i32, _i32, _i32, _i32]),
    'stc_cell_gates_fwd_f32': (_int, [_pp, _i32, _p, _i32, _p, _p, _p, _p, _p, _p, _i64, _i32, _i32, _i32, _i32, _i32, _p]),
    'stc_cell_gates_bwd_f32': (_int, [_pp, _i32, _p, _i32, _p, _p, _p, _p, _p, _p, _p, _p, _i32, _pp, _p, _p, _p, _p, _p, _size, _i64, _i32, _i32, _i32, _i32, _i32, _p]),
    'stc_cell_cand_bwd_f32': (_int, [_pp, _i32, _p, _i32, _p, _p, _p, _p, _pp, _p, _p, _p, _size, _i64, _i32, _i32, _i32, _i32, _p]),
    'stc_cell_blend_fwd_f32': (_int, [_pp, _i32, _p, _i32, _p, _p, _p, _p, _p, _p, _p, _i32, _i32, _p, _i32, _p, _i32, _i32, _i64, _i32, _i32, _i32, _i32, _p]),
    'stc_cell_small_supported': (_int, [_i32, _i32, _i32, _i32, _i32]),
    'stc_cell_small_workspace_bytes': (_size, [_i32, _i32, _i32, _i32, _i32]),
    'stc_cell_small_param_rows': (_int, []),
    'stc_cell_small_fwd_f32': (_int, [_p, _p, _p, _i32, _i32, _i32, _p, _p, _p, _i32, _p, _i32, _p, _p, _i32, _i32] + [_p] * 17 + [_i32, _i32, _i32, _i32, _p]),
    'stc_cell_small_bwd_f32': (_int, [_p, _p, _p, _i32, _i32, _i32, _p, _p, _p, _i32, _p, _i32, _p, _p, _i32, _i32] + [_p] * 12
                               + [_i32, _p, _i32, _p, _i64, _i32, _i32, _p, _p, _p, _p, _p, _p, _p, _size, _i32, _i32, _i32, _i32, _p]),
    'stc_graph_grad_f32': (_int, [_p, _p, _p, _i32, _i32, _i32, _i32, _i32, _i32, _i32, _i64, _p]),
    'stc_mix_grad_f32': (_int, [_p, _p, _p, _i32, _i32, _i32, _i32, _i32, _i32, _i32, _i32, _i64, _p]),
    'stc_mixed_fusion_workspace_bytes': (_size, [_i32, _i32]),
    'stc_mixed_fusion_fwd_f32': (_int, [_p] * 8 + [_i32, _p]),
    'stc_mixed_fusion_bwd_f32': (_int, [_p] * 12 + [_size, _i32, _p]),
    'stc_mgp_uv_fwd_f32': (_int, [_p, _i64, _i64, _i64, _p, _p, _f32, _p, _p, _i32, _i32, _i32, _i32, _p]),
    'stc_mgp_uv_bwd_f32': (_int, [_p, _i64, _i64, _i64, _p, _p, _p, _p, _f32, _p, _i32, _i32, _i32, _i32, _p]),
    'stc_mgp_softmax_fwd_f32': (_int, [_p, _p, _i32, _p]),
    'stc_mgp_softmax_bwd_f32': (_int, [_p, _p, _p, _p, _p, _i32, _p]),
    'stc_adam_f32': (_int, [_p] * 4 + [_i64, _p] + [C.c_double] * 5 + [_p]),
    'stc_gru_gates_fwd_f32': (_int, [_p, _p, _p, _p, _p, _p, _i64, _i32, _i32, _i32, _p]),
    'stc_gru_gates_bwd_f32': (_int, [_p, _p, _p, _p, _p, _p, _p, _p, _p, _i64, _i32, _i32, _i32, _p]),
    'stc_gru_blend_fwd_f32': (_int, [_p, _p, _p, _p, _p, _i64, _p]),
    'stc_gru_blend_bwd_f32': (_int, [_p, _p, _p, _p, _p, _p, _p, _i64, _p]),
    'stc_gru_blend_bwd_bf16': (_int, [_p, _p, _p, _p, _i64, _p]),
    'stc_head_fwd_f32': (_int, [_p, _p, _p, _p, _i64, _i32, _p]),
    'stc_head_fwd_bf16': (_int, [_p, _p, _p, _p, _i64, _i32, _p]),
    'stc_head_bwd_workspace_bytes': (_size, [_i32]),
    'stc_head_bwd_f32': (_int, [_p, _p, _p, _p, _p, _p, _p, _size, _i64, _i32, _p]),
    'stc_head_bwd_bf16': (_int, [_p, _p, _p, _p, _p, _p, _p, _size, _i64, _i32, _p]),
    'stc_axpy_f32': (_int, [_f32, _p, _p, _i64, _p]),
    'stc_concat2_f32': (_int, [_p, _p, _p, _i64, _i32, _i32, _i32, _p]),
    'stc_split2_f32': (_int, [_p, _p, _p, _p, _p, _i64, _i32, _i32, _i32, _i32, _p, _p, _p]),
}
EXPORTS = tuple(_ABI)


def _declare(lib):
    for name, (restype, argtypes) in _ABI.items():
        fn = getattr(lib, name)
        fn.restype, fn.argtypes = restype, argtypes


_LIB = None


def load_library(path: str = LIB_PATH):
    global _LIB
    if _LIB is not None:
        return _LIB
    if not os.path.exists(path):
        raise StcError(
            f'{path} not found: the HIP kernels are not built. Run '
            f'`make -C {os.path.join(_PKG_ROOT, "csrc")}` (or `python -c "import __graft_entry__ as g; g.build()"`). '
            'There is no CPU fallback for the STC-GNN hot path.')
    lib = C.CDLL(path)
    _declare(lib)
    v = lib.stc_version()
    if v != ABI_VERSION:
        raise StcError(f'{path}: ABI version {v}, host expects {ABI_VERSION}')
    _LIB = lib
    return lib


class KernelTimer:

    def __init__(self, only=None):
        self.spans = []
        self.only = None if only is None else frozenset(only)

    def add(self, name, start, end, nbytes, tag=None):
        self.spans.append((name, start, end, nbytes, tag))

    def summary(self):
        torch.cuda.synchronize()
        out = {}
        for name, s, e, nb, tag in self.spans:
            d = out.setdefault(name, dict(launches=0, ms=0.0, bytes=0))
            ms = s.elapsed_time(e)
            for acc in (d,) if tag is None else (d, d.setdefault('tags', {}).setdefault(tag, dict(launches=0, ms=0.0, bytes=0))):
                acc['launches'] += 1
                acc['ms'] += ms
                acc['bytes'] += nb
        self.spans = []
        return out


def _ptr(t: Optional[torch.Tensor]):
    return None if t is None else t.data_ptr()


def _tensor(name, t, shape=None, dtype=torch.float32):
    if not isinstance(t, torch.Tensor) or not t.is_cuda:
        raise StcError(f'{name}: expected a ROCm (cuda) tensor, got {type(t).__name__}'
                       f'{"" if not isinstance(t, torch.Tensor) else " on " + str(t.device)}; no CPU fallback')
    if t.dtype != dtype:
        raise StcError(f'{name}: expected {dtype}, got {t.dtype}' + (' (the reference path is fp32-only)' if dtype == torch.float32 else ''))
    if not t.is_contiguous():
        raise StcError(f'{name}: tensor must be contiguous')
    if shape is not None and tuple(t.shape) != tuple(shape):
        raise StcError(f'{name}: shape {tuple(t.shape)}, expected {tuple(shape)}')
    return t


def _storage(t):
    return torch.bfloat16 if t.dtype == torch.bfloat16 else torch.float32


class HipKernels:

    name = 'hip-gfx950'
    operand_format = {'f16x2': FMT_F16X2, 'bf16x3': FMT_BF16X3}[os.environ.get('STC_OPERAND_FORMAT', 'f16x2')]
    HEAVY_ROW_SUM = 24.0
    patch_spmm = os.environ.get('STC_PATCH_SPMM', '1') != '0'
    patch_min_items = 1000
    optional_gate_stores = True
    first_step_cells = True

    def __init__(self):
        self.lib = load_library()
        if not torch.cuda.is_available():
            raise StcError('no ROCm device visible: the STC-GNN hot path runs on MI355X only (no CPU fallback)')
        self._workspace = {}
        self._retired = []
        self.timer: Optional[KernelTimer] = None

    ACT_AMAX_SLOTS = 256

    def act_amax_buffer(self, like, *lead):
        if self.operand_format != FMT_F16X2:
            return None
        return torch.zeros(*lead, self.ACT_AMAX_SLOTS, dtype=torch.float32, device=like.device)

    def _act_amax(self, what, given, rows, on):
        if given is None or self.operand_format != FMT_F16X2:
            return None
        _tensor(what + '.act_amax', given, (rows, self.ACT_AMAX_SLOTS))
        self._same_device(on, given)
        return given.data_ptr()

    def for_graph(self, row_sum_bound: float):
        if self.operand_format != FMT_F16X2 or not (row_sum_bound > self.HEAVY_ROW_SUM):
            return self
        view = getattr(self, '_b3_view', None)
        if view is None:
            import copy
            view = copy.copy(self)
            view.operand_format = FMT_BF16X3
            view._bf16_front = None
            self._b3_view = view
        view.timer = self.timer
        return view

    def set_dispatch_level(self, level: int):
        rc = self.lib.stc_set_dispatch_level(int(level))
        if rc != 0:
            self._failed(f'stc_set_dispatch_level({level})', rc)

    def _failed(self, what, rc):
        msg = self.lib.stc_last_error()
        raise StcError(f'{what} failed with code {rc}: {msg.decode() if msg else "?"}')

    def _launch(self, name, on, *args, nbytes=0, tag=None):
        fn = getattr(self.lib, name)
        index = on.device.index
        timer = self.timer
        if timer is not None and timer.only is not None and name not in timer.only:
            timer = None
        if timer is None and index == torch._C._cuda_getDevice():
            rc = fn(*args, torch._C._cuda_getCurrentRawStream(index))
        else:
            with torch.cuda.device(on.device):
                stream = torch.cuda.current_stream(on.device)
                if timer is None:
                    rc = fn(*args, stream.cuda_stream)
                else:
                    start, end = torch.cuda.Event(enable_timing=True), torch.cuda.Event(enable_timing=True)
                    start.record(stream)
                    rc = fn(*args, stream.cuda_stream)
                    end.record(stream)
                    timer.add(name, start, end, nbytes, tag)
        if rc != 0:
            self._failed(name, rc)

    @staticmethod
    def _i32(name, t, numel=None):
        _tensor(name, t, None, torch.int32)
        if numel is not None and t.numel() != numel:
            raise StcError(f'{name}: {t.numel()} elements, expected {numel}')
        return t

    def _same_device(self, *ts):
        devs = {t.device for t in ts if t is not None}
        if len(devs) > 1:
            raise StcError(f'tensors on different devices: {devs}')

    def csr_spmm(self, rowptr, colidx, val, n_rows, n_cols, X, Y0, Y, alpha, beta, plan=None):
        self._spmm(_storage(X), rowptr, colidx, val, n_rows, n_cols, X, Y0, Y, alpha, beta, plan)

    def csr_spmm_bf16(self, rowptr, colidx, val, n_rows, n_cols, X, Y0, Y, alpha, beta, plan=None):
# ... 36 lines not shown
        self._i32('spmm.pt_src', pt_src, n_p * PATCH_MAX_SRC)
        self._i32('spmm.pt_rows', pt_rows, n_p * PATCH_ROWS)
        self._i32('spmm.pt_cnt', pt_cnt, n_p * PATCH_ROWS)
        if pt_idx.dtype != torch.uint8 or not pt_idx.is_contiguous() or pt_idx.shape != (n_p, PATCH_ROWS, width):
            raise StcError(f'spmm.pt_idx must be a contiguous uint8 tensor of shape {(n_p, PATCH_ROWS, width)}')
        _tensor('spmm.pt_val', pt_val, (n_p, PATCH_ROWS, width))
        self._same_device(on, pt_src, pt_rows, pt_cnt, pt_idx, pt_val)
        return [_ptr(pt_src), _ptr(pt_rows), _ptr(pt_cnt), _ptr(pt_idx), _ptr(pt_val), n_p, width]

    def _patch_wanted(self, plan, items, wide, plain):
        return plan is not None and len(plan) > 3 and self.patch_spmm and items >= self.patch_min_items * ((6 if wide else 3) if plain else 1)

    def _csr_ptrs(self, rowptr, colidx, val, n_rows):
        self._i32('spmm.rowptr', rowptr, n_rows + 1)
        self._i32('spmm.colidx', colidx)
        _tensor('spmm.val', val, (colidx.numel(),))
        return [_ptr(rowptr), _ptr(colidx), _ptr(val)]

    def _blk_ptrs(self, plan, n_rows):
        blk_ptr, blk_cols, blk_vals = plan[:3]
        self._i32('spmm.blk_ptr', blk_ptr, (n_rows + 3) // 4 + 1)
        self._i32('spmm.blk_cols', blk_cols)
        _tensor('spmm.blk_vals', blk_vals, (blk_cols.numel(), 4))
        return [_ptr(blk_ptr), _ptr(blk_cols), _ptr(blk_vals)]

    def _graph_ptrs(self, rowptr, colidx, val, plan, n_rows):
        return self._csr_ptrs(rowptr, colidx, val, n_rows) + ([None, None, None] if plan is None else self._blk_ptrs(plan, n_rows))

    def _spmm_sum_checked(self, dt, max_add, rowptr, colidx, val, X, X2, addends, Y, blend):
        B, n, Cc, h = Y.shape
        _tensor('spmm_sum.Y', Y, None, dt)
        _tensor('spmm_sum.X', X, (B, n, Cc, h), dt)
        if X2 is not None:
            _tensor('spmm_sum.X2', X2, (B, n, Cc, h), dt)
        if len(addends) > max_add:
            raise StcError(f'spmm_sum: at most {max_add} addends, got {len(addends)}')
        for i, ent in enumerate(addends):
            t, off = ent[0], ent[1]
            _tensor(f'spmm_sum.add{i}', t, None, dt)
            if t.shape[:3] != (B, n, Cc) or off < 0 or off + h > t.shape[-1] or (t.shape[-1] | off) & 3:
                raise StcError(f'spmm_sum: addend {i} of shape {tuple(t.shape)} / offset {off} does not fit')
        U = Cand = dY = None
        if blend is not None:
            U, Cand, dY = blend
            for name, t in (('U', U), ('Cand', Cand), ('dY', dY)):
                _tensor('spmm_sum.' + name, t, (B, n, Cc, h), dt)
        self._same_device(rowptr, colidx, val, X, X2, Y, U, Cand, dY, *[ent[0] for ent in addends])
        return B, n, Cc, h, (U, Cand, dY), (colidx.numel() * 8 + 4 * (n + 1)
                                            + dt.itemsize * B * n * Cc * h * (2 + (X2 is not None) + len(addends) + (3 if blend else 0)))

    def spmm_sum(self, rowptr, colidx, val, plan, X, X2, addends, Y, blend=None, alpha=1.0, amax=None):
        B, n, Cc, h, (U, Cand, dY), nbytes = self._spmm_sum_checked(torch.float32, SPMM_SUM_MAX_ADD, rowptr, colidx, val, X, X2, addends, Y, blend)
        ptrs, lds, offs, scales = (_p * SPMM_SUM_MAX_ADD)(), (_i32 * SPMM_SUM_MAX_ADD)(), (_i32 * SPMM_SUM_MAX_ADD)(), (_f32 * SPMM_SUM_MAX_ADD)()
        for i, ent in enumerate(addends):
            ptrs[i], lds[i], offs[i], scales[i] = ent[0].data_ptr(), ent[0].shape[-1], ent[1], (float(ent[2]) if len(ent) > 2 else 1.0)
        if amax is not None:
            _tensor('spmm_sum.amax', amax)
            self._same_device(Y, amax)
        g = self._graph_ptrs(rowptr, colidx, val, plan, n)
        self._launch('stc_spmm_sum_f32', Y, *g, n, n, _ptr(X), _ptr(X2), float(alpha), len(addends), ptrs, lds, offs, scales, _ptr(Y), _ptr(U), _ptr(Cand), _ptr(dY),
                     _ptr(amax), 0 if amax is None else amax.numel(), B, Cc, h, nbytes=nbytes)

    RING2_MAX_ADD = RING2_MAX_ADD

    @staticmethod
    def ring2_fits(B, n, Cc, h) -> bool:
        return h == 16 and (Cc * h) % 128 == 0 and B * n * (Cc * h // 4) < (1 << 28) and B <= 65535

    def ring2_sum(self, rowptr, colidx, val, ring2, X, X2, addends, U, Cand, Y, Z):
        B, n, Cc, h = Y.shape
        for name, t in (('Y', Y), ('Z', Z), ('X', X), ('U', U), ('Cand', Cand)) + ((('X2', X2),) if X2 is not None else ()):
            _tensor('ring2_sum.' + name, t, (B, n, Cc, h))
        if len(addends) > self.RING2_MAX_ADD:
            raise StcError(f'ring2_sum: at most {self.RING2_MAX_ADD} addends, got {len(addends)}')
        ptrs = (_p * self.RING2_MAX_ADD)()
        for i, t in enumerate(addends):
            _tensor(f'ring2_sum.add{i}', t, (B, n, Cc, h))
            ptrs[i] = t.data_ptr()
        self._same_device(X, X2, U, Cand, Y, Z, *addends)
        self._launch('stc_ring2_sum_f32', Y, *self._ring2_ptrs('ring2_sum', ring2, Y), n, _ptr(X), _ptr(X2), len(addends), ptrs,
                     _ptr(U), _ptr(Cand), _ptr(Y), _ptr(Z), B, Cc, h,
                     nbytes=colidx.numel() * 8 + 4 * (n + 1) + 4 * B * n * Cc * h * (1 + (X2 is not None) + len(addends) + 2 + 2))

    def _ring2_ptrs(self, what, ring2, on):
        l2, l1, own, t1, t2 = ring2
        n_p = l2.shape[0]
        for name, t, shape in (('l2_rows', l2, (n_p, RING2_SECOND)), ('l1_rows', l1, (n_p, RING2_FIRST)), ('int_rows', own, (n_p, RING2_INTERIOR)),
                               ('t1', t1, (n_p, RING2_FIRST, RING2_WIDTH, 2)), ('t2', t2, (n_p, RING2_INTERIOR, RING2_WIDTH, 2))):
            _tensor(f'{what}.{name}', t, shape, torch.int32)
        self._same_device(on, l2, l1, own, t1, t2)
        return [_ptr(l2), _ptr(l1), _ptr(own), _ptr(t1), _ptr(t2), n_p]

    def ring2_blend(self, rowptr, colidx, val, ring2, Bm, A, U, H, Cand, Hnew, SHnew):
        B, n, Cc, h = H.shape
        for name, t in (('Bm', Bm), ('A', A), ('U', U), ('H', H), ('Hnew', Hnew), ('SHnew', SHnew)) + ((('Cand', Cand),) if Cand is not None else ()):
            _tensor('ring2_blend.' + name, t, (B, n, Cc, h))
        self._same_device(Bm, A, U, H, Cand, Hnew, SHnew)
        self._launch('stc_ring2_blend_f32', H, *self._ring2_ptrs('ring2_blend', ring2, H), n, _ptr(Bm), _ptr(A), _ptr(U), _ptr(H), _ptr(Cand), _ptr(Hnew), _ptr(SHnew),
                     B, Cc, h, nbytes=colidx.numel() * 8 + 4 * (n + 1) + 4 * B * n * Cc * h * (6 + (Cand is not None)))

    def ring2_blend_first(self, rowptr, colidx, val, ring2, Bm, A, U, Cand, Hnew, SHnew):
        B, n, Cc, h = U.shape
        for name, t in (('Bm', Bm), ('A', A), ('U', U), ('Hnew', Hnew), ('SHnew', SHnew)) + ((('Cand', Cand),) if Cand is not None else ()):
            _tensor('ring2_blend_first.' + name, t, (B, n, Cc, h))
        self._same_device(Bm, A, U, Cand, Hnew, SHnew)
        self._launch('stc_ring2_blend_first_f32', U, *self._ring2_ptrs('ring2_blend_first', ring2, U), n, _ptr(Bm), _ptr(A), _ptr(U), _ptr(Cand), _ptr(Hnew),
                     _ptr(SHnew), B, Cc, h, nbytes=colidx.numel() * 8 + 4 * (n + 1) + 4 * B * n * Cc * h * (5 + (Cand is not None)))

    def ring2_chain(self, rowptr, colidx, val, ring2, X, X2, alpha1, add1, V, alpha2, add0, Z):
        B, n, Cc, h = Z.shape
        for name, t in (('Z', Z), ('X', X)) + ((('X2', X2),) if X2 is not None else ()) + ((('V', V),) if V is not None else ()):
            _tensor('ring2_chain.' + name, t, (B, n, Cc, h))
        if len(add1) > 2 or not 1 <= len(add0) <= self.RING2_MAX_ADD:
            raise StcError(f'ring2_chain: 0..2 first-ring and 1..{self.RING2_MAX_ADD} interior addends, got {len(add1)} and {len(add0)}')
        p1, p0, s0 = (_p * 2)(), (_p * self.RING2_MAX_ADD)(), (_f32 * self.RING2_MAX_ADD)()
        for i, t in enumerate(add1):
            _tensor(f'ring2_chain.add1[{i}]', t, (B, n, Cc, h))
            p1[i] = t.data_ptr()
        for i, (t, scale) in enumerate(add0):
            _tensor(f'ring2_chain.add0[{i}]', t, (B, n, Cc, h))
            p0[i], s0[i] = t.data_ptr(), float(scale)
        self._same_device(X, X2, V, Z, *add1, *[t for t, _ in add0])
        self._launch('stc_ring2_chain_f32', Z, *self._ring2_ptrs('ring2_chain', ring2, Z), n, _ptr(X), _ptr(X2), float(alpha1), len(add1), p1, _ptr(V),
                     float(alpha2), len(add0), p0, s0, _ptr(Z), B, Cc, h,
                     nbytes=colidx.numel() * 8 + 4 * (n + 1) + 4 * B * n * Cc * h * (1 + (X2 is not None) + len(add1) + (V is not None) + len(add0) + 1))

    def csr_sddmm(self, rowptr, colidx, n_rows, n_cols, A, Bm, out, alpha, accumulate):
        B, nr, F = A.shape
        _tensor('sddmm.A', A, (B, n_rows, F))
        _tensor('sddmm.Bm', Bm, (B, n_cols, F))
        self._i32('sddmm.rowptr', rowptr, n_rows + 1)
        self._i32('sddmm.colidx', colidx)
        _tensor('sddmm.out', out, (colidx.numel(),))
        self._same_device(rowptr, colidx, A, Bm, out)
        self._launch('stc_csr_sddmm_f32', A, _ptr(rowptr), _ptr(colidx), n_rows, n_cols, _ptr(A), _ptr(Bm), _ptr(out), B, F, float(alpha), int(bool(accumulate)))

    def cheby_dense_fwd(self, G, K, T):
        n = G.shape[0]
        _tensor('cheby.G', G, (n, n))
        _tensor('cheby.T', T, (K, n, n))
        self._launch('stc_cheby_dense_fwd_f32', G, _ptr(G), n, K, _ptr(T))

    def cheby_dense_bwd(self, G, T, dT, dG):
        K, n, _ = T.shape
        _tensor('cheby.G', G, (n, n))
        _tensor('cheby.T', T, (K, n, n))
        _tensor('cheby.dT', dT, (K, n, n))
        _tensor('cheby.dG', dG, (n, n))
        self._launch('stc_cheby_dense_bwd_f32', G, _ptr(G), _ptr(T), _ptr(dT), n, K, _ptr(dG))

    @staticmethod
    def _ptr_array(tensors):
        arr = (_p * len(tensors))()
        for i, t in enumerate(tensors):
            arr[i] = t.data_ptr()
        return arr

    def _node_shapes(self, Zs, Tc, W, dt=torch.float32):
        Ks, Kc = len(Zs), Tc.shape[0]
        if not (1 <= Ks <= MAX_K and 1 <= Kc <= MAX_K):
            raise StcError(f'Chebyshev orders Ks={Ks}, Kc={Kc} outside [1,{MAX_K}]')
        R, Cc, L = Zs[0].shape
        Ho = W.shape[1]
        Lw = W.shape[0] // (Ks * Kc)
        if Lw < 1 or Lw > L:
            raise StcError(f'node.W: {W.shape[0]} rows give Lw={Lw} per block, slabs are {L} wide')
# ... 745 lines not shown

    def cell_blend_fwd(self, Zs, Tc, W, bias, U, H, Cand, Hnew, copies=(), side=None):
        Ks, Kc, R, Cc, L, Lw, Ho = self._node_shapes(Zs, Tc, W)
        h = H.shape[-1]
        if Ho != h:
            raise StcError(f'cell_blend: W gives Ho={Ho} for hidden {h}')
        if bias is not None:
            _tensor('cell.bias', bias, (Ho,))
        for name, t in (('U', U), ('H', H), ('Cand', Cand), ('Hnew', Hnew)):
            _tensor('cell.' + name, t, (R, Cc, h))
        cp = self._state_copies('cell_blend', copies, side, R, Cc, h, H)
        self._same_device(*Zs, Tc, W, bias, U, H, Cand, Hnew)
        self._launch('stc_cell_blend_fwd_f32', H, self._ptr_array(Zs), Ks, _ptr(Tc), Kc, _ptr(W), _ptr(bias), _ptr(U), _ptr(H),
                     _ptr(Cand), _ptr(Hnew), *cp, R, Cc, L, Lw, h)

    def gru_gates_fwd(self, G, Xt, H, U, Rg, CandIn):
        rows, h = H.shape[:-1].numel(), H.shape[-1]
        cin = Xt.shape[-1]
        pad = CandIn.shape[-1] - cin - h
        if pad < 0:
            raise StcError(f'gates.CandIn: width {CandIn.shape[-1]} < cin + h = {cin + h}')
        for name, t, w in (('G', G, 2 * h), ('Xt', Xt, cin), ('H', H, h), ('U', U, h), ('Rg', Rg, h),
                           ('CandIn', CandIn, cin + h + pad)):
            _tensor('gates.' + name, t)
            if t.shape[-1] != w or t.numel() != rows * w:
                raise StcError(f'gates.{name}: shape {tuple(t.shape)} does not match rows={rows}, width={w}')
        self._launch('stc_gru_gates_fwd_f32', H, _ptr(G), _ptr(Xt), _ptr(H), _ptr(U), _ptr(Rg), _ptr(CandIn), rows, cin, h, pad)

    def gru_gates_bwd(self, dCandIn, dU, H, U, Rg, dG, dXt, dH, dH_in=None):
        rows, h = H.shape[:-1].numel(), H.shape[-1]
        cin = dXt.shape[-1]
        pad = dCandIn.shape[-1] - cin - h
        if pad < 0:
            raise StcError(f'gates_bwd.dCandIn: width {dCandIn.shape[-1]} < cin + h = {cin + h}')
        for name, t, w in (('dCandIn', dCandIn, cin + h + pad), ('dU', dU, h), ('H', H, h), ('U', U, h), ('Rg', Rg, h),
                           ('dG', dG, 2 * h), ('dXt', dXt, cin), ('dH', dH, h)) + ((('dH_in', dH_in, h),) if dH_in is not None else ()):
            _tensor('gates_bwd.' + name, t)
            if t.shape[-1] != w or t.numel() != rows * w:
                raise StcError(f'gates_bwd.{name}: shape {tuple(t.shape)} does not match rows={rows}, width={w}')
        self._launch('stc_gru_gates_bwd_f32', H, _ptr(dCandIn), _ptr(dU), _ptr(H), _ptr(U), _ptr(Rg), _ptr(dH_in), _ptr(dG), _ptr(dXt), _ptr(dH), rows, cin, h, pad)

    def _same_numel(self, what, *ts):
        n = ts[0].numel()
        for i, t in enumerate(ts):
            _tensor(f'{what}[{i}]', t)
            if t.numel() != n:
                raise StcError(f'{what}: operand {i} has {t.numel()} elements, expected {n}')
        return n

    def gru_blend_fwd(self, Cpre, U, H, Cand, Hnew):
        n = self._same_numel('blend', Cpre, U, H, Cand, Hnew)
        self._launch('stc_gru_blend_fwd_f32', H, _ptr(Cpre), _ptr(U), _ptr(H), _ptr(Cand), _ptr(Hnew), n)

    def gru_blend_bwd(self, dHnew, U, H, Cand, dCpre, dU, dH):
        n = self._same_numel('blend_bwd', dHnew, U, Cand, dCpre, *(t for t in (H, dU, dH) if t is not None))
        if dU is not None and H is None:
            raise StcError('blend_bwd: dU needs H')
        self._launch('stc_gru_blend_bwd_f32', U, _ptr(dHnew), _ptr(U), _ptr(H), _ptr(Cand), _ptr(dCpre), _ptr(dU), _ptr(dH), n)

    def head_fwd(self, H, w, b, y):
        h = H.shape[-1]
        rows = H.shape[:-1].numel()
        dt = _storage(H)
        _tensor('head.H', H, None, dt)
        _tensor('head.w', w, (h,))
        _tensor('head.b', b, (1,))
        _tensor('head.y', y, tuple(H.shape[:-1]))
        self._launch('stc_head_fwd_bf16' if dt == torch.bfloat16 else 'stc_head_fwd_f32', H, _ptr(H), _ptr(w), _ptr(b), _ptr(y), rows, h)

    def head_bwd(self, H, w, y, dy, dH, dwb):
        h = H.shape[-1]
        rows = H.shape[:-1].numel()
        dt = _storage(H)
        _tensor('head.H', H, None, dt)
        _tensor('head.w', w, (h,))
        _tensor('head.y', y, tuple(H.shape[:-1]))
        _tensor('head.dy', dy, tuple(H.shape[:-1]))
        _tensor('head.dH', dH, tuple(H.shape), dt)
        _tensor('head.dwb', dwb, (h + 1,))
        ws = self._get_workspace(H.device, self.lib.stc_head_bwd_workspace_bytes(h))
        self._launch('stc_head_bwd_bf16' if dt == torch.bfloat16 else 'stc_head_bwd_f32', H,
                     _ptr(H), _ptr(w), _ptr(y), _ptr(dy), _ptr(dH), _ptr(dwb), _ptr(ws), ws.numel(), rows, h)

    def axpy(self, a, x, y):
        n = self._same_numel('axpy', x, y)
        self._launch('stc_axpy_f32', x, float(a), _ptr(x), _ptr(y), n)

    def _cat_shapes(self, what, A, Bm, whole):
        a, b = A.shape[-1], Bm.shape[-1]
        rows = whole.shape[:-1].numel()
        pad = whole.shape[-1] - a - b
        if pad < 0:
            raise StcError(f'{what}: joined width {whole.shape[-1]} < {a} + {b}')
        for name, t, w in (('A', A, a), ('B', Bm, b), ('whole', whole, a + b + pad)):
            _tensor(f'{what}.{name}', t)
            if t.shape[-1] != w or t.numel() != rows * w:
                raise StcError(f'{what}.{name}: shape {tuple(t.shape)} does not match rows={rows}, width={w}')
        return rows, a, b, pad

    def concat2(self, A, Bm, out):
        rows, a, b, pad = self._cat_shapes('concat2', A, Bm, out)
        self._launch('stc_concat2_f32', out, _ptr(A), _ptr(Bm), _ptr(out), rows, a, b, pad)

    def split2(self, src, A, Bm, addA=None, addB=None, addA_ld=0, addA2=None, addB2=None):
        rows, a, b, pad = self._cat_shapes('split2', A, Bm, src)
        if addA is not None:
            _tensor('split2.addA', addA, A.shape if not addA_ld else A.shape[:-1] + (addA_ld,))
            if addA_ld and addA_ld < a:
                raise StcError(f'split2: addA_ld={addA_ld} is smaller than the width {a}')
        for name, t, like in (('addB', addB, Bm), ('addA2', addA2, A), ('addB2', addB2, Bm)):
            if t is not None:
                _tensor('split2.' + name, t, like.shape)
        self._launch('stc_split2_f32', src, _ptr(src), _ptr(addA), _ptr(addB), _ptr(A), _ptr(Bm), rows, a, b, pad,
                     int(addA_ld if addA is not None else 0), _ptr(addA2), _ptr(addB2))


class _Bf16Planar:

    name = 'hip-gfx950-bf16'

    def __init__(self, base: HipKernels):
        self.b = base

    def cell_fused_supported(self, Ks, Kc, Cc, L, h) -> bool:
        return self.cell_planar_supported(Ks, Kc, Cc, h)

    def cell_planar_supported(self, Ks, Kc, Cc, h) -> bool:
        return bool(self.b.lib.stc_cell_planar_bf16_supported(Ks, Kc, Cc, h))

    def node_post_supported(self, Ks, Kc, Cc, L, Ho) -> bool:
        return self.cell_planar_supported(Ks, Kc, Cc, Ho) and L in (20, 32)

    def csr_spmm(self, rowptr, colidx, val, n_rows, n_cols, X, Y0, Y, alpha, beta, plan=None):
        self.b.csr_spmm_bf16(rowptr, colidx, val, n_rows, n_cols, X, Y0, Y, alpha, beta, plan=plan)

    def cell_gates_fwd_planar(self, X, H, SX, SH, Tc, W, bias, U, Rg, RH, post=None):
        b = self.b
        R, Cc, h, cin, (Wc, bc, A, Bm), nbytes = b._gates_fwd_planar_checked(torch.bfloat16, X, H, SX, SH, Tc, W, bias, U, Rg, RH, post)
        b._launch('stc_cell_gates_fwd_planar_bf16', H, _ptr(X), _ptr(H), _ptr(SX), _ptr(SH), _ptr(Tc), _ptr(W), _ptr(bias),
                  _ptr(U), _ptr(Rg), _ptr(RH), _ptr(Wc), _ptr(bc), _ptr(A), _ptr(Bm), R, Cc, cin + h, h, nbytes=nbytes)

    def spmm_blend_fwd(self, rowptr, colidx, val, plan, Bm, A, U, H, Cand, Hnew, copies=(), side=None):
        b = self.b
        if copies or side is not None:
            raise StcError('bf16 planar path: state copies into interleaved rows do not exist (every cell reads planes)')
        B, n, Cc, h, nbytes = b._spmm_blend_checked(torch.bfloat16, rowptr, colidx, val, Bm, A, U, H, Cand, Hnew)
        g = b._graph_ptrs(rowptr, colidx, val, plan, n)
        b._launch('stc_spmm_blend_fwd_bf16', H, *g, n, n, _ptr(Bm), _ptr(A), _ptr(U), _ptr(H), _ptr(Cand), _ptr(Hnew), B, Cc, h, nbytes=nbytes)

    def spmm_sum(self, rowptr, colidx, val, plan, X, X2, addends, Y, blend=None):
        b = self.b
        B, n, Cc, h, (U, Cand, dY), nbytes = b._spmm_sum_checked(torch.bfloat16, SPMM_SUM_BF16_MAX_ADD, rowptr, colidx, val, X, X2, addends, Y, blend)
        for t, off in addends:
            if off != 0 or tuple(t.shape) != tuple(Y.shape):
                raise StcError('spmm_sum (bf16): addends are whole planes')
        ptrs = (_p * SPMM_SUM_BF16_MAX_ADD)(*[t.data_ptr() for t, _ in addends])
        g = b._graph_ptrs(rowptr, colidx, val, plan, n)
        b._launch('stc_spmm_sum_bf16', Y, *g, n, n, _ptr(X), _ptr(X2), len(addends), ptrs, _ptr(Y), _ptr(U), _ptr(Cand), _ptr(dY), B, Cc, h, nbytes=nbytes)

    def gru_blend_bwd(self, dHnew, U, H, Cand, dCpre, dU, dH):
        if dU is not None or dH is not None:
            raise StcError('gru_blend_bwd (bf16): only the dCpre form exists')
        for name, t in (('dHnew', dHnew), ('U', U), ('Cand', Cand), ('dCpre', dCpre)):
            _tensor('blend_bwd.' + name, t, tuple(dHnew.shape), torch.bfloat16)
        self.b._launch('stc_gru_blend_bwd_bf16', dHnew, _ptr(dHnew), _ptr(U), _ptr(Cand), _ptr(dCpre), dHnew.numel())

# ... 33 lines not shown
```

### stc-gnn_amd/stc_hip/ops.py

```python
from __future__ import annotations

import enum
from typing import Optional

import torch
from torch.autograd import Function
from torch.autograd.function import once_differentiable

from .graph import SpatialOperand
from .small import _alias, _check_guard, _guard, _out_slots, _stacks, _unpack, last_uses, small_graph_supported, stc_small_graph, wavefront

_kernels = None


def kernels():
    global _kernels
    if _kernels is None:
        from ._lib import HipKernels
        _kernels = HipKernels()
    return _kernels


def _c(t: torch.Tensor) -> torch.Tensor:
    return t if t.is_contiguous() else t.contiguous()
# ... 329 lines not shown
            Tcp = Tc if pack == 1 else _block_diag(Tc, pack)
            Zg = _spatial_slabs(XH, fwd_val, op, Ks)
            k.cell_gates_fwd(rows(Zg), Tcp, Wg, bg, *rows((H, U, Rg, CandIn)))
            Zc = _spatial_slabs(CandIn, fwd_val, op, Ks)
            k.cell_blend_fwd(rows(Zc), Tcp, Wc, bc, *rows((U, H, Cand, Hnew)))
        else:
            G, Zg = _bdg_forward(XH, Wg, bg, Tc, fwd_val, op, Ks)
            k.gru_gates_fwd(G, Xt, H, U, Rg, CandIn)
            del G
            Cpre, Zc = _bdg_forward(CandIn, Wc, bc, Tc, fwd_val, op, Ks)
            k.gru_blend_fwd(Cpre, U, H, Cand, Hnew)
        ctx.save_for_backward(H, U, Rg, Cand, Wg, Wc, Tc, *Zg, *Zc)
        ctx.op, ctx.Ks, ctx.cin = op, Ks, cin
        ctx.bias = (bg is not None, bc is not None)
        return Hnew

    @staticmethod
    @once_differentiable
    def backward(ctx, dHnew):
        k = kernels()
        H, U, Rg, Cand, Wg, Wc, Tc, *Z = ctx.saved_tensors
        Ks, op, cin = ctx.Ks, ctx.op, ctx.cin
        Zg, Zc = Z[:Ks], Z[Ks:]
        need_Xt, need_H = ctx.needs_input_grad[0], ctx.needs_input_grad[1]
        need_Tc, need_val = ctx.needs_input_grad[6], ctx.needs_input_grad[7]
        B, N, C, L = Zc[0].shape
        v3 = lambda t: t.view(B, N, C * L)
        bwd = (op.bwd_rowptr, op.bwd_colidx, op.bwd_val, op.bwd_plan)
        pack = 0 if (need_Tc or need_val) else _cell_pack(k, B * N, C, Ks, Tc.shape[0], L, H.shape[-1])
        pro = pack > 0
        dHnew = _c(dHnew)
        dH = torch.empty_like(H)
        dXt = H.new_empty(H.shape[:-1] + (cin,))
        if pro:
            dCpre = dU = dG = None
            g, dWc, dbc, dTc, dval = _bdg_backward_slabs(None, Zc, Wc, Tc, op, Ks, ctx.bias[1], False, False, cand=(dHnew, U, Cand), pack=pack)
        else:
            dCpre, dU = torch.empty_like(H), torch.empty_like(H)
            k.gru_blend_bwd(dHnew, U, H, Cand, dCpre, dU, dH)
            dG = H.new_empty(H.shape[:-1] + (2 * H.shape[-1],))
            g, dWc, dbc, dTc, dval = _bdg_backward_slabs(dCpre, Zc, Wc, Tc, op, Ks, ctx.bias[1], need_Tc, need_val)
        gates_pro, dci = None, g[0]
        if Ks > 1:
            k.csr_spmm(*bwd[:3], N, N, v3(g[1]), v3(g[0]), v3(g[0]), 1.0, 1.0, plan=op.bwd_plan)
        if pro:
            gates_pro = (dci, Cand, H, U, Rg, dHnew, dH)
        else:
            k.gru_gates_bwd(dci, dU, H, U, Rg, dG, dXt, dH, dH_in=dH)
        g, dWg, dbg, dTc2, dval2 = _bdg_backward_slabs(dG, Zg, Wg, Tc, op, Ks, ctx.bias[0], need_Tc, need_val, gates=gates_pro, pack=max(1, pack))
        if need_Xt or need_H:
            if Ks > 1:
                k.csr_spmm(*bwd[:3], N, N, v3(g[1]), v3(g[0]), v3(g[0]), 1.0, 1.0, plan=op.bwd_plan)
            if pro:
                k.split2(g[0], dXt, dH, addA=dci, addB=dH, addA_ld=L)
            else:
                k.split2(g[0], dXt, dH, addA=dXt, addB=dH)
        if need_Tc:
            dTc = dTc + dTc2
        if need_val:
            dval = dval + dval2
        return (dXt if need_Xt else None), (dH if need_H else None), dWg, dbg, dWc, dbc, dTc, dval, None, None


def stc_cell(Xt, H, op: SpatialOperand, Tc, Wg, bg, Wc, bc, Ks: int):
    if Xt.dim() != 4 or H.dim() != 4 or Xt.shape[:-1] != H.shape[:-1]:
        raise ValueError(f'stc_cell: Xt {tuple(Xt.shape)} and H {tuple(H.shape)} must be (B,N,C,*) with equal leading shape')
    B, N, C, h = H.shape
    L = Xt.shape[-1] + h
    Kc = Tc.shape[0]
    if N != op.n or Tc.shape[1] != C:
        raise ValueError(f'stc_cell: graphs are for N={op.n}, C={Tc.shape[1]}; got N={N}, C={C}')
    if Wg.shape != (Ks * Kc * L, 2 * h) or Wc.shape != (Ks * Kc * L, h):
        raise ValueError(f'stc_cell: W shapes {tuple(Wg.shape)}, {tuple(Wc.shape)} do not match Ks*Kc*L={Ks * Kc * L}, h={h}')
    return _StcCell.apply(Xt, H, Wg, bg, Wc, bc, Tc, op.fwd_val, op, Ks)


_CELL_GRAPH = True
_PLANAR = True
_POST_AGG = True
_SMALL = True
_RING2 = True
_RING2_FWD = True
_FIRST_STEP = True

_ZEROS = {}


def _first_step_kernels(k, dtype, C: int, h: int) -> bool:
    return bool(_FIRST_STEP and dtype == torch.float32 and getattr(k, 'first_step_cells', False) and k.cell_first_supported(C, h))


def first_step_route(op: SpatialOperand, Tc, Ks: int, C: int, h: int, x_widths, dtype=torch.float32) -> bool:
    k = kernels()
    return Ks == 2 and _first_step_kernels(k, dtype, C, h) and not (_SMALL and small_graph_supported(k, op, Tc, Ks, C, h, x_widths, dtype))


def zero_state(ref: torch.Tensor, shape, dtype=None) -> torch.Tensor:
    key = (ref.device, dtype or ref.dtype)
    if key not in _ZEROS:
        _ZEROS[key] = torch.zeros((), device=key[0], dtype=key[1])
    return _ZEROS[key].expand(*shape)


def _is_zero_state(t: torch.Tensor) -> bool:
    z = _ZEROS.get((t.device, t.dtype))
    return z is not None and t.dim() == 4 and not any(t.stride()) and t.untyped_storage().data_ptr() == z.untyped_storage().data_ptr()


def cell_graph_supported(op: SpatialOperand, Tc, Ks: int, C: int, h: int, x_widths, dtype=torch.float32) -> bool:
    if not _CELL_GRAPH or h != 16:
        return False
    k = kernels()
    if _SMALL and small_graph_supported(k, op, Tc, Ks, C, h, x_widths, dtype):
        return True
    if Tc.requires_grad or op.fwd_val.requires_grad:
        return False
    if dtype == torch.bfloat16:
        return (_PLANAR and _POST_AGG and Ks == 2 and Tc.shape[0] == 2 and k.bf16.cell_planar_supported(Ks, 2, C, h)
                and all(w == h or 1 <= w <= 4 for w in x_widths))
    return all(k.cell_fused_supported(Ks, Tc.shape[0], C, w + h + (-(w + h)) % 4, h) for w in set(x_widths))


def _amplification(op: SpatialOperand, Ks: int) -> float:
    return float(op.row_sum_bound) ** max(1, Ks - 1)


class _Form(enum.Enum):
    PLANAR3 = 'order-3 planar'
    PLANAR_ONE_BWD = 'planar, one-launch backward'
    PLANAR = 'planar'
    ROWS_POST = 'rows, post-aggregation'
    ROWS_SLABS = 'rows, slabs'

    def saved(self, Ks: int) -> int:
        return 4 + {'PLANAR3': 8, 'PLANAR_ONE_BWD': 3, 'PLANAR': 4, 'ROWS_POST': Ks + 1, 'ROWS_SLABS': 2 * Ks}[self.name]

    @property
    def planar(self) -> bool:
        return self not in (_Form.ROWS_POST, _Form.ROWS_SLABS)


def _cell_forms(k, Ks: int, Kc: int, C: int, h: int, cin, bf16: bool):
    planar2 = (_PLANAR and _POST_AGG and Ks == 2 and k.cell_planar_supported(Ks, Kc, C, h)
               and k.node_post_supported(Ks, Kc, C, 2 * h, h))
    post20 = bool(planar2) and k.node_post_supported(Ks, Kc, C, 20, h)
    planar3 = bool(_PLANAR and not bf16 and Ks == 3 and Kc == 3 and k.cell_planar_k_supported(Ks, C, h))
    forms = []
    for w in cin:
        if planar3 and (w == h or 1 <= w <= 4):
            forms.append(_Form.PLANAR3)
        elif planar2 and (w == h or (post20 and 1 <= w <= 4)):
            one_bwd = k.cell_bwd_planar_supported(C, h, w) if bf16 else k.cell_bwd_planar_supported(C, h)
            forms.append(_Form.PLANAR_ONE_BWD if one_bwd else _Form.PLANAR)
        else:
            post = Ks > 1 and _POST_AGG and k.node_post_supported(Ks, Kc, C, w + h + (-(w + h)) % 4, h)
            forms.append(_Form.ROWS_POST if post else _Form.ROWS_SLABS)
    return forms


class _Pass:

    def __init__(self, k, op: SpatialOperand, Ks: int, Tc, schedule, cin, forms, dims, bf16: bool, zmax_all, graph):
        self.k, self.op, self.Ks, self.Tc, self.schedule, self.cin, self.forms = k, op, Ks, Tc, schedule, cin, forms
        (self.B, self.N, self.C), self.h, self.bf16, self.zmax_all = dims, 16, bf16, zmax_all
        self.graph = graph

    def spmm(self, X, Y0=None, Y=None, alpha=1.0, beta=0.0):
        Y = torch.empty_like(X) if Y is None else Y
        v3 = lambda t: None if t is None else t.view(self.B, self.N, -1)
        self.k.csr_spmm(*self.graph[:3], self.N, self.N, v3(X), v3(Y0), v3(Y), alpha, beta, plan=self.graph[3])
        return Y

    def rows(self, ts):
        return [None if t is None else t.view(self.B * self.N, self.C, t.shape[-1]) for t in ts]

    def act_slots(self, j, which=0):
        return {} if self.zmax_all is None else dict(act_amax=self.zmax_all[j, which])


class _ForwardPass(_Pass):

    def __init__(self, k, op: SpatialOperand, Ks: int, Tc, fwd_val, schedule, ext, cin, forms, bf16: bool, forward_only: bool = False):
        zmax_all = k.act_amax_buffer(ext[0], len(schedule), 2, 2 * Ks) if (not forward_only and not bf16 and any(f.planar for f in forms)) else None
        super().__init__(k, op, Ks, Tc, schedule, cin, forms, ext[0].shape[:3], bf16, zmax_all, (op.fwd_rowptr, op.fwd_colidx, fwd_val, op.fwd_plan))
        self.fwd_val, self.ext = fwd_val, ext
        self.state = [None] * len(schedule)
        self.XH, self.agg = {}, {}
        self.consumers = [[] for _ in schedule]
        for j, (_, x, hs) in enumerate(schedule):
            for src, role in ((hs, 'h'), (x, 'x')):
                if src[0] == 'cell':
                    self.consumers[src[1]].append((j, role))
        self.ring2 = _RING2_FWD and not bf16 and op.fwd_ring2 is not None and k.ring2_fits(self.B, self.N, self.C, self.h)
        self.lean = forward_only and bool(getattr(k, 'optional_gate_stores', False))
        zero = {('ext', i) for i, t in enumerate(ext) if _is_zero_state(t)}
        can = _first_step_kernels(k, ext[0].dtype, self.C, self.h)
        self.first = [can and hs in zero and f is _Form.PLANAR_ONE_BWD for (_, _, hs), f in zip(schedule, forms)]

    def source(self, src):
        if src[0] != 'ext':
            return self.state[src[1]]
        t = self.ext[src[1]]
        if not t.is_contiguous() and _is_zero_state(t):
            t = self.ext[src[1]] = t.new_zeros(t.shape)
        return t

    def plane(self):
        return self.ext[0].new_empty(self.B, self.N, self.C, self.h)

    def rows_of(self, j):
        if j not in self.XH:
            w = self.cin[j]
            self.XH[j] = self.ext[0].new_empty(self.B, self.N, self.C, w + self.h + (-(w + self.h)) % 4)
        return self.XH[j]

    def aggregated(self, src, planes=False):
        if src not in self.agg:
            self.agg[src] = self.cheb_planes(self.source(src)) if planes else self.spmm(self.source(src))
        return self.agg[src]

    def cheb_planes(self, t):
        if not (self.ring2 and t.shape[-1] == self.h):
            s1 = self.spmm(t)
            return [t, s1, self.spmm(s1, t, alpha=2.0, beta=-1.0)]
        s1, s2 = torch.empty_like(t), torch.empty_like(t)
        self.k.ring2_chain(*self.graph[:3], self.op.fwd_ring2, t, None, 1.0, [], s1, 2.0, [(t, -1.0)], s2)
        return [t, s1, s2]

    def copy_plan(self, j):
        B, N, C, h, cin, schedule = self.B, self.N, self.C, self.h, self.cin, self.schedule
        copies, side, late_copies, late_rows = [], None, [], []
        for (d, role) in self.consumers[j]:
            if self.forms[d].planar:
                continue
            Xd = self.rows_of(d)
            view = Xd.view(B * N, C, Xd.shape[-1])
            if role == 'x':
                copies.append((view, 0))
            elif schedule[d][1][0] == 'ext':
                if side is None:
                    copies.insert(0, (view, cin[d]))
                    side = self.ext[schedule[d][1][1]].view(B * N, C, cin[d])
                else:
                    late_rows.append(d)
            elif Xd.shape[-1] > cin[d] + h:
                late_rows.append(d)
            else:
                copies.append((view, cin[d]))
        first = 1 if side is not None else 0
        while len(copies) > 2:
            late_copies.append(copies.pop(len(copies) - 1 if len(copies) - 1 >= first else first))
        return copies, side, late_copies, late_rows

    def finish(self, j, Hnew, late_copies, late_rows):
        for buf, off in late_copies:
            buf[..., off:off + self.h].copy_(Hnew.view(self.B * self.N, self.C, self.h))
        for d in late_rows:
            Xd, xs, w = self.rows_of(d), self.schedule[d][1], self.cin[d]
            if xs[0] == 'ext':
                self.k.concat2(self.ext[xs[1]], Hnew, Xd)
            else:
                Xd[..., w:w + self.h].copy_(Hnew)
                Xd[..., w + self.h:].zero_()
        self.state[j] = Hnew

    def planar3(self, j, Wg, bg, Wc, bc, Hprev, U, Rg, Cand, Hnew, copies, side):
        k, rows, (_, x, hs) = self.k, self.rows, self.schedule[j]
        Zx, Zh, RH = self.aggregated(x, planes=True), self.aggregated(hs, planes=True), torch.empty_like(Hprev)
        k.cell_gates_fwd_planar_k(rows(Zx), rows(Zh), self.Tc, Wg, bg, *rows((U, Rg, RH)), **self.act_slots(j, 0))
        Zr = self.cheb_planes(RH)
        k.cell_cand_fwd_planar_k(rows(Zx), rows(Zr), self.Tc, Wc, bc, *rows((U, Hprev, Cand, Hnew)), **self.act_slots(j, 1))
        return [*Zx, *Zh[1:], *Zr]

    def planar(self, j, Wg, bg, Wc, bc, Hprev, U, Rg, Cand, Hnew, copies, side):
        k, op, rows, (_, x, hs) = self.k, self.op, self.rows, self.schedule[j]
        first = Hprev is None
        Xp, SXp, SHp = self.source(x), self.aggregated(x), None if first else self.aggregated(hs)
        RH = None if (self.forms[j] is _Form.PLANAR_ONE_BWD or self.lean) else self.plane()
        A, Bm = self.plane(), self.plane()
        if first:
            k.cell_gates_fwd_first(*rows((Xp, SXp)), self.Tc, Wg, bg, *rows((U,)), (Wc, bc, *rows((A, Bm))), **self.act_slots(j))
        else:
            k.cell_gates_fwd_planar(*rows((Xp, Hprev, SXp, SHp)), self.Tc, Wg, bg, *rows((U, Rg, RH)), post=(Wc, bc, *rows((A, Bm))), **self.act_slots(j))
        if (self.ring2 and not op.ring2_clusters and not copies and side is None
                and any(self.forms[d].planar for d, _ in self.consumers[j])):
            SHn = self.plane()
            if first:
                k.ring2_blend_first(*self.graph[:3], op.fwd_ring2, Bm, A, U, Cand, Hnew, SHn)
            else:
                k.ring2_blend(*self.graph[:3], op.fwd_ring2, Bm, A, U, Hprev, Cand, Hnew, SHn)
            self.agg[('cell', j)] = SHn
        else:
            k.spmm_blend_fwd(*self.graph, Bm, A, U, self.source(hs) if first else Hprev, Cand, Hnew, copies=copies, side=side)
        return [Xp, SXp, SHp] + ([] if RH is None else [RH])

    def rows_cell(self, j, Wg, bg, Wc, bc, Hprev, U, Rg, Cand, Hnew, copies, side):
        k, op, rows, Tc, (_, x, hs) = self.k, self.op, self.rows, self.Tc, self.schedule[j]
        Xj = self.rows_of(j)
        w = self.cin[j]
        if x[0] == 'ext' and hs[0] == 'ext':
            k.concat2(self.ext[x[1]], Hprev, Xj)
        elif x[0] == 'cell' and hs[0] == 'ext':
            Xj[..., w:w + self.h].copy_(Hprev)
            if Xj.shape[-1] > w + self.h:
                Xj[..., w + self.h:].zero_()
        CandIn = torch.empty_like(Xj)
        Zg = _spatial_slabs(Xj, self.fwd_val, op, self.Ks)
        k.cell_gates_fwd(rows(Zg), Tc, Wg, bg, *rows((Hprev, U, Rg, CandIn)))
        if self.forms[j] is _Form.ROWS_POST:
            A, Bm = torch.empty_like(Hprev), torch.empty_like(Hprev)
            k.node_post_fwd(*rows((CandIn,)), Tc, Wc, bc, *rows((A, Bm)))
            k.spmm_blend_fwd(*self.graph, Bm, A, U, Hprev, Cand, Hnew, copies=copies, side=side)
            return [*Zg, CandIn]
        Zc = _spatial_slabs(CandIn, self.fwd_val, op, self.Ks)
        k.cell_blend_fwd(rows(Zc), Tc, Wc, bc, *rows((U, Hprev, Cand, Hnew)), copies=copies, side=side)
        return [*Zg, *Zc]

    def cell(self, j, stack, out=None):
        first = self.first[j]
        Hprev = None if first else self.source(self.schedule[j][2])
        copies, side, late_copies, late_rows = self.copy_plan(j)
        form = self.forms[j]
        U = self.plane()
        Rg, Cand = (None, None) if (self.lean and form.planar) else (None if first else self.plane(), self.plane())
        Hnew = self.plane() if out is None else out
        run = self.planar3 if form is _Form.PLANAR3 else self.planar if form.planar else self.rows_cell
        more = run(j, *stack, Hprev, U, Rg, Cand, Hnew, copies, side)
        self.finish(j, Hnew, late_copies, late_rows)
        return [Hprev, U, Rg, Cand, *more]

    def wavefront(self):
        return wavefront(self.schedule)

    def last_uses(self, order):
        return last_uses(self.schedule, order)

    def release(self, j, last, keep):
        self.XH.pop(j, None)
        for src in set(self.schedule[j][1:]) | {('cell', j)}:
            if last.get(src, j) == j:
                self.agg.pop(src, None)
                if src[0] == 'cell' and src[1] not in keep:
                    self.state[src[1]] = None


class _BackwardPass(_Pass):

    def __init__(self, k, op: SpatialOperand, Ks: int, Tc, schedule, stacks, cin, forms, dims, bf16: bool, zmax_all):
        super().__init__(k, op, Ks, Tc, schedule, cin, forms, dims, bf16, zmax_all, (op.bwd_rowptr, op.bwd_colidx, op.bwd_val, op.bwd_plan))
        self.stacks = stacks
        self.ring2 = _RING2 and not bf16 and op.bwd_ring2 is not None and k.ring2_fits(self.B, self.N, self.C, self.h)
        self.G = {}
        self.pieces = {}
        self.rows_of_set = {}

    def grads_for(self, s_id):
        if s_id not in self.rows_of_set:
            Wg_, bg_, Wc_, bc_ = self.stacks[s_id]
            sizes = [Wg_.numel(), 0 if bg_ is None else 2 * self.h, Wc_.numel(), 0 if bc_ is None else self.h]
            self.rows_of_set[s_id] = [Wg_.new_zeros(sum(1 for sc in self.schedule if sc[0] == s_id), sum(sizes)), 0, sizes]
        entry = self.rows_of_set[s_id]
        entry[1] += 1
        return self.param_views(s_id, entry[0][entry[1] - 1])

    def param_views(self, s_id, row):
        Wg_, bg_, Wc_, bc_ = self.stacks[s_id]
        parts = row.split(self.rows_of_set[s_id][2])
        return parts[0].view_as(Wg_), None if bg_ is None else parts[1], parts[2].view_as(Wc_), None if bc_ is None else parts[3]

    def leave(self, kid, direct, aggregated):
        pc = self.pieces.setdefault(kid, dict(direct=[], agg=[]))
        pc['direct'] += direct
        pc['agg'].append(aggregated)

    def owed(self, kid, blend=None):
        base = self.G.pop(kid, None)
        pc = self.pieces.pop(kid, None)
        if pc is None:
            if blend is None:
                return base
            dY = torch.empty_like(base)
            self.k.gru_blend_bwd(base, blend[0], None, blend[1], dY, None, None)
            return base, dY
        if 'd2' in pc:
            return self.clenshaw(pc['d0'] + ([base] if base is not None else []), pc['d1'], pc['d2'])
        add = pc['direct'] + ([base] if base is not None else [])
        aggs = pc['agg']
        while len(add) > 5:
            add.append(add.pop() + add.pop())
        while len(aggs) > 2:
            aggs = [aggs[0] + aggs[1]] + aggs[2:]
        out = torch.empty_like(aggs[0])
        dY = torch.empty_like(out) if blend is not None else None
        self.k.spmm_sum(*self.graph, aggs[0], aggs[1] if len(aggs) > 1 else None, [(t, 0) for t in add], out,
                   blend=None if blend is None else (blend[0], blend[1], dY))
        return out if blend is None else (out, dY)

    def owed_ring2(self, kid, U_, Cand_):
        pc = self.pieces.get(kid)
        if not self.ring2 or pc is None:
            return None
        add = pc['direct'] + ([self.G[kid]] if kid in self.G else [])
        if len(add) > 2 or len(pc['agg']) != 1:
            return None
        self.G.pop(kid, None)
        self.pieces.pop(kid)
        out, dBm_ = torch.empty_like(pc['agg'][0]), torch.empty_like(pc['agg'][0])
        self.k.ring2_sum(*self.graph[:3], self.op.bwd_ring2, pc['agg'][0], None, add, U_, Cand_, out, dBm_)
        return out, dBm_

    def leave3(self, kid, d0, d1, d2):
        pc = self.pieces.setdefault(kid, dict(d0=[], d1=[], d2=[]))
        pc['d0'] += list(d0); pc['d1'] += list(d1); pc['d2'] += list(d2)

    def clenshaw(self, d0, d1, d2):
        k = self.k
        while len(d2) > 2:
            d2 = [d2[0] + d2[1]] + d2[2:]
        if self.ring2 and len(d1) <= 2 and 1 <= len(d0) + len(d2) <= k.RING2_MAX_ADD:
            out = torch.empty_like(d2[0])
            k.ring2_chain(*self.graph[:3], self.op.bwd_ring2, d2[0], d2[1] if len(d2) > 1 else None, 2.0, list(d1), None, 1.0,
                          [(a, 1.0) for a in d0] + [(a, -1.0) for a in d2], out)
            return out
        t = torch.empty_like(d2[0])
        k.spmm_sum(*self.graph, d2[0], d2[1] if len(d2) > 1 else None, [(a, 0) for a in d1], t, alpha=2.0)
        adds = [(a, 0) for a in d0] + [(a, 0, -1.0) for a in d2]
        while len(adds) > 8:
            (a, _), (b_, _) = adds.pop(0), adds.pop(0)
            adds.insert(0, (a + b_, 0))
        out = torch.empty_like(t)
        k.spmm_sum(*self.graph, t, None, adds, out, blend=None)
        return out

    def planar3(self, j, Wg, bg, Wc, bc, saved):
        k, rows, Tc, (s_id, x, hs) = self.k, self.rows, self.Tc, self.schedule[j]
        Hprev, U, Rg, Cand, Zx0, Zx1, Zx2, Zh1, Zh2, *Zr = saved
        Zx, Zh = [Zx0, Zx1, Zx2], [Hprev, Zh1, Zh2]
        wide = self.cin[j] == self.h
        new = lambda: torch.empty_like(Hprev)
        dWg, dbg, dWc, dbc = self.grads_for(s_id)
        dHnew = self.owed(j)
        dX, dR = ([new(), new(), new()] if wide else [None] * 3), [new(), new(), new()]
        k.cell_cand_bwd_planar_k(rows(Zx), rows(Zr), Tc, Wc, *rows((dHnew, U, Cand)), rows(dX), rows(dR), dWc, dbc, **self.act_slots(j, 1))
        dRH = self.clenshaw([dR[0]], [dR[1]], [dR[2]])
        del dR
        dHg = [new(), new(), new()]
        k.cell_gates_bwd_planar_k(rows(Zx), rows(Zh), Tc, Wg, *rows((dRH, Cand, U, Rg, dHnew)), rows(dX), rows(dHg), dWg, dbg, None,
                                  accumulate_x=wide, **self.act_slots(j, 0))
        if wide and x[0] == 'cell':
            self.leave3(x[1], dX[:1], dX[1:2], dX[2:])
        if hs[0] == 'cell':
            self.leave3(hs[1], dHg[:1], dHg[1:2], dHg[2:])

    def planar_one_bwd(self, j, Wg, bg, Wc, bc, saved):
        k, (s_id, x, hs) = self.k, self.schedule[j]
        Hprev, U, Rg, Cand, Xp, SXp, SHp = saved
        fused = self.owed_ring2(j, U, Cand)
        if fused is not None:
            dHnew, dBm = fused
        else:
            dHnew, dY = self.owed(j, (U, Cand))
            dBm = self.spmm(dY)
            del dY
        new = lambda: torch.empty_like(U)
        dWg, dbg, dWc, dbc = self.grads_for(s_id)
        taken = set()

        def planes_of_state(src):
            if src[0] != 'cell':
                return new(), new(), False
            pc = self.pieces.get(src[1])
            if not self.bf16 and pc is not None and pc.get('own') is not None and src[1] not in taken:
                taken.add(src[1])
                return pc['own'][0], pc['own'][1], True
            d, a_ = new(), new()
            self.leave(src[1], (d,), a_)
            if self.pieces[src[1]].get('own') is None:
                self.pieces[src[1]]['own'] = (d, a_)
                taken.add(src[1])
            return d, a_, False

        dXd, dSX, acc_x = planes_of_state(x) if self.cin[j] == self.h else (None, None, False)
        if Hprev is None:
            k.cell_bwd_first(*self.rows((Xp, SXp)), self.Tc, Wg, Wc, *self.rows((U, Cand, dHnew, dBm)), self.rows((dXd, dSX)), dWg, dbg, dWc, dbc,
                             accumulate_x=acc_x, **self.act_slots(j))
            return
        dHd, dSH, acc_h = planes_of_state(hs)
        k.cell_bwd_planar(*self.rows((Xp, Hprev, SXp, SHp)), self.Tc, Wg, Wc, *self.rows((U, Rg, Cand, dHnew, dBm)),
                          self.rows((dXd, dSX, dHd, dSH)), dWg, dbg, dWc, dbc,
                          **(dict(accumulate_x=acc_x, accumulate_h=acc_h, **self.act_slots(j)) if not self.bf16 else {}))

    def planar(self, j, Wg, bg, Wc, bc, saved):
        k, rows, Tc, (s_id, x, hs) = self.k, self.rows, self.Tc, self.schedule[j]
        Hprev, U, Rg, Cand, Xp, SXp, SHp, RH = saved
        dHnew, dY = self.owed(j, (U, Cand))
        wide = self.cin[j] == self.h
        zr = None if self.zmax_all is None else self.zmax_all[j, 0]
        post_kw, gates_kw = ({}, {}) if zr is None else (dict(act_amax=(zr[0], zr[2])), dict(act_amax=zr))
        dBm = self.spmm(dY)
        dRH = torch.empty_like(Hprev)
        dWg, dbg, dWc, dbc = self.grads_for(s_id)
        dHd, dSH = torch.empty_like(Hprev), torch.empty_like(Hprev)
        if wide:
            dXc, dXd, dSX = (torch.empty_like(Hprev) for _ in range(3))
            k.node_post_bwd(*rows((Xp,)), Tc, Wc, *rows((dY, dBm, dXc)), dWc, dbc, X2=RH.view(-1, self.C, self.h), dX2=dRH.view(-1, self.C, self.h),
                            **post_kw)
            planes = rows((dXd, dSX, dHd, dSH))
        else:
            k.node_post_bwd(*rows((RH,)), Tc, Wc, *rows((dY, dBm, dRH)), dWc, dbc, X2=Xp.view(-1, self.C, self.cin[j]), **post_kw)
            planes = [None, None] + rows((dHd, dSH))
        del dY, dBm
        k.cell_gates_bwd_planar(*rows((Xp, Hprev, SXp, SHp)), Tc, Wg, *rows((dRH, Cand, U, Rg, dHnew)), planes, dWg, dbg, None, **gates_kw)
        if wide and x[0] == 'cell':
            self.leave(x[1], (dXd, dXc), dSX)
        if hs[0] == 'cell':
            self.leave(hs[1], (dHd,), dSH)

    def rows_cell(self, j, Wg, bg, Wc, bc, saved):
        k, op, Ks, h, Tc, (s_id, x, hs) = self.k, self.op, self.Ks, self.h, self.Tc, self.schedule[j]
        Hprev, U, Rg, Cand, *Z = saved
        Zg, Zc = Z[:Ks], Z[Ks:]
        post = self.forms[j] is _Form.ROWS_POST
        dHnew, dY = self.owed(j, (U, Cand)) if post else (self.owed(j), None)
        dH = torch.empty_like(Hprev)
        if post:
            dBm = self.spmm(dY)
            dci, dWc = torch.empty_like(Zc[0]), torch.empty_like(Wc)
            dbc = Wc.new_empty(h) if bc is not None else None
            k.node_post_bwd(*self.rows((Zc[0],)), Tc, Wc, *self.rows((dY, dBm, dci)), dWc, dbc)
        else:
            g, dWc, dbc, _, _ = _bdg_backward_slabs(None, Zc, Wc, Tc, op, Ks, bc is not None, False, False, cand=(dHnew, U, Cand))
            if Ks > 1:
                self.spmm(g[1], g[0], g[0], 1.0, 1.0)
            dci = g[0]
        g, dWg, dbg, _, _ = _bdg_backward_slabs(None, Zg, Wg, Tc, op, Ks, bg is not None, False, False, gates=(dci, Cand, Hprev, U, Rg, dHnew, dH))
        need_x, need_h = x[0] == 'cell', hs[0] == 'cell'
        if need_x or need_h:
            if Ks > 1:
                self.spmm(g[1], g[0], g[0], 1.0, 1.0)
            dXt = Hprev.new_empty(Hprev.shape[:-1] + (self.cin[j],))
            same = need_x and need_h and x[1] == hs[1]
            owedA = self.G.get(x[1]) if need_x else None
            owedB = self.G.get(hs[1]) if (need_h and not same) else None
            k.split2(g[0], dXt, dH, addA=dci, addB=dH, addA_ld=Zc[0].shape[-1], addA2=owedA, addB2=owedB)
            if need_h and not same:
                self.G[hs[1]] = dH
            if need_x:
                self.G[x[1]] = dXt.add_(dH) if same else dXt
        return dWg, dbg, dWc, dbc


def _begin_forward(op: SpatialOperand, Ks: int, schedule, outputs, n_ext: int, Tc, fwd_val, tensors, forward_only: bool = False):
    k = kernels().for_graph(_amplification(op, Ks))
    _, stacks, Tc, fwd_val = _unpack(0, Tc, fwd_val, tensors[n_ext:])
    ext = [t if _is_zero_state(t) else _c(t) for t in tensors[:n_ext]]
    bf16 = ext[0].dtype == torch.bfloat16
    if bf16:
        k = k.bf16
    h = 16
    B, N, C = ext[0].shape[:3]
    cin = [ext[x[1]].shape[-1] if x[0] == 'ext' else h for _, x, _ in schedule]
    forms = _cell_forms(k, Ks, Tc.shape[0], C, h, cin, bf16)
    if bf16 and not all(f.planar for f in forms):
        raise ValueError('stc_cell_graph: bfloat16 states need an all-planar schedule (Ks = 2, inputs 16 or 1..4 columns wide)')
    p = _ForwardPass(k, op, Ks, Tc, fwd_val, schedule, ext, cin, forms, bf16, forward_only)
    out_stack = ext[0].new_empty(len(outputs), B, N, C, h)
    return p, stacks, out_stack, _out_slots(outputs)


def _forward_only(op: SpatialOperand, Ks: int, schedule, outputs, n_ext: int, Tc, fwd_val, tensors):
    p, stacks, out_stack, out_slot = _begin_forward(op, Ks, schedule, outputs, n_ext, Tc, fwd_val, tensors, forward_only=True)
    order = p.wavefront()
    last = p.last_uses(order)
    for j in order:
        p.cell(j, stacks[schedule[j][0]], out_stack[out_slot[j]] if j in out_slot else None)
        p.release(j, last, out_slot)
    return out_stack


class _StcCellGraph(Function):

    @staticmethod
    def forward(ctx, op: SpatialOperand, Ks: int, schedule, outputs, n_ext: int, Tc, fwd_val, *tensors):
        p, stacks, out_stack, out_slot = _begin_forward(op, Ks, schedule, outputs, n_ext, Tc, fwd_val, tensors)
        saved = []
        for j, (s_id, _, _) in enumerate(schedule):
            saved += p.cell(j, stacks[s_id], _alias(out_stack, out_slot[j]) if j in out_slot else None)
        ctx.save_for_backward(p.Tc, *[t for st in stacks for t in st], *saved)
        ctx.meta = (op, Ks, schedule, tuple(outputs), p.cin, len(stacks), (p.B, p.N, p.C), p.forms)
        ctx.zmax_all = p.zmax_all
        _guard(ctx, out_stack)
        return out_stack

    @staticmethod
    @once_differentiable
    def backward(ctx, grad_stack):
        k = kernels().for_graph(_amplification(ctx.meta[0], ctx.meta[1]))
        bf16 = grad_stack.dtype == torch.bfloat16
        if bf16:
            k = k.bf16
        op, Ks, schedule, outputs, cin, n_sets, dims, forms = ctx.meta
        _check_guard(ctx)
        Tc, *sv = ctx.saved_tensors
        stacks, sv = _stacks(sv[:4 * n_sets]), sv[4 * n_sets:]
        cells = []
        for f in forms:
            cells, sv = cells + [sv[:f.saved(Ks)]], sv[f.saved(Ks):]
        p = _BackwardPass(k, op, Ks, Tc, schedule, stacks, cin, forms, dims, bf16, ctx.zmax_all)
        grad_stack = _c(grad_stack)
        for i, j in enumerate(outputs):
            p.G[j] = grad_stack[i]
        acc = [[None] * 4 for _ in stacks]

        def add_to(s_id, grads):
            acc[s_id] = [a if t is None else t if a is None else a.add_(t) for a, t in zip(acc[s_id], grads)]

        for j in range(len(schedule) - 1, -1, -1):
            if j not in p.G and j not in p.pieces:
                continue
            s_id, f = schedule[j][0], forms[j]
            run = {_Form.PLANAR3: p.planar3, _Form.PLANAR_ONE_BWD: p.planar_one_bwd, _Form.PLANAR: p.planar}.get(f, p.rows_cell)
            grads = run(j, *stacks[s_id], cells[j])
            if not f.planar:
                add_to(s_id, grads)
        for s_id, (buf, _, _) in p.rows_of_set.items():
            add_to(s_id, p.param_views(s_id, buf[0] if buf.shape[0] == 1 else buf.sum(0)))
        flat = [None if prm is None else (g if g is not None else torch.zeros_like(prm)) for st, a in zip(stacks, acc) for prm, g in zip(st, a)]
        n_ext = len(ctx.needs_input_grad) - 7 - len(flat)
        return (None,) * 7 + (None,) * n_ext + tuple(flat)


def stc_cell_graph(op: SpatialOperand, Tc, Ks: int, schedule, outputs, ext, stacks):
    k = kernels()
    if _SMALL and small_graph_supported(k, op, Tc, Ks, ext[0].shape[2], 16, {ext[x[1]].shape[-1] if x[0] == 'ext' else 16 for _, x, _ in schedule},
                                        ext[0].dtype):
        return stc_small_graph(k, op, Tc, Ks, schedule, outputs, ext, stacks)
    flat = [p for st in stacks for p in st]
    if not torch.is_grad_enabled() or not any(t is not None and t.requires_grad for t in (Tc, op.fwd_val, *ext, *flat)):
        with torch.no_grad():
            return _forward_only(op, Ks, list(schedule), list(outputs), len(ext), Tc, op.fwd_val, (*ext, *flat))
    return _StcCellGraph.apply(op, Ks, list(schedule), list(outputs), len(ext), Tc, op.fwd_val, *ext, *flat)


class _MixedFusion(torch.autograd.Function):

    @staticmethod
    def forward(ctx, A, P, WA, bA, WP, bP):
        k = kernels()
        A_, P_ = A.detach().contiguous(), P.detach().contiguous()
        gate, G = k.mixed_fusion_fwd(WA.detach(), bA.detach(), WP.detach(), bP.detach(), A_, P_)
        ctx.save_for_backward(A_, P_, WA, WP, gate)
        return G

    @staticmethod
    def backward(ctx, dG):
        A, P, WA, WP, gate = ctx.saved_tensors
        want_dA = ctx.needs_input_grad[0]
        need = ctx.needs_input_grad
        dWA, dWP, db, dP, dA = kernels().mixed_fusion_bwd(WA.detach(), WP.detach(), A, P, gate, dG.contiguous(), want_dA, want_dW=need[2] or need[4])
        return (dA if need[0] else None, dP if need[1] else None, dWA if need[2] else None, db if need[3] else None,
                dWP if need[4] else None, db if need[5] else None)


def mixed_fusion_supported(A: torch.Tensor, P: torch.Tensor, *params: torch.Tensor) -> bool:
    ts = (A, P) + params
    return (all(t.is_cuda and t.dtype == torch.float32 for t in ts) and all(t.is_contiguous() for t in params)
            and all(t.data_ptr() % 16 == 0 for t in ts)
            and kernels().mixed_fusion_supported(A.numel()))


def mixed_fusion(A, P, WA, bA, WP, bP):
    return _MixedFusion.apply(A, P, WA, bA, WP, bP)


class _MgpUV(torch.autograd.Function):

    @staticmethod
    def forward(ctx, X, Wu, Wv, rows_axis, alpha):
        X_ = X.detach().contiguous()
        U, V = kernels().mgp_uv_fwd(X_, rows_axis, Wu.detach().contiguous(), Wv.detach().contiguous(), alpha)
        ctx.save_for_backward(X_, U, V)
        ctx.meta = (rows_axis, alpha)
        return U, V

    @staticmethod
    @once_differentiable
    def backward(ctx, dU, dV):
        X_, U, V = ctx.saved_tensors
        dWu, dWv = kernels().mgp_uv_bwd(X_, ctx.meta[0], U, V, dU.contiguous(), dV.contiguous(), ctx.meta[1])
        return None, dWu, dWv, None, None


class _MgpSoftmax(torch.autograd.Function):

    @staticmethod
    def forward(ctx, P):
        P_ = P.detach().contiguous()
        Ps = kernels().mgp_softmax_fwd(P_)
        ctx.save_for_backward(P_, Ps)
        return Ps

    @staticmethod
    @once_differentiable
    def backward(ctx, dPs):
        P_, Ps = ctx.saved_tensors
        return kernels().mgp_softmax_bwd(P_, Ps, dPs.contiguous())


def mgp_front_supported(X: torch.Tensor, Wu: torch.Tensor, Wv: torch.Tensor) -> bool:
    return (X.is_cuda and X.dim() == 4 and all(t.is_cuda and t.dtype == torch.float32 for t in (X, Wu, Wv)) and not X.requires_grad
            and Wu.dim() == 2 and Wu.shape == Wv.shape and hasattr(kernels(), 'mgp_uv_fwd'))


def mgp_front(X, Wu, Wv, rows_axis: int, alpha: float, reduce=None):
    U, V = _MgpUV.apply(X, Wu, Wv, rows_axis, alpha)
    P = U.flatten(1) @ V.flatten(1).t()
    if reduce is not None:
        P = reduce(P)
    return _MgpSoftmax.apply(P)
```

Baseline: 32.10 samples/s.

## Fuse output head into ring2 decoder blend and backward sum kernels

Folds the two-layer output projection into a single weight vector and bias and computes the sigmoid head inside the ring2 blend kernel that produces the decoder hidden state. In backward, a new head_bwd_g kernel produces the per-row scalar gradient, and the ring2 sum kernel adds g*w in place of a materialized dH. The aim is to avoid separate head launches and the extra HBM round-trips for the stacked decoder outputs and dH. In exchange it adds a new autograd Function, more template variants and rounding-controlled arithmetic to keep results bit-matched.

```diff
diff --git a/include/stc_hip.h b/include/stc_hip.h
--- a/include/stc_hip.h
+++ b/include/stc_hip.h
@@ -8,7 +8,7 @@
 extern "C" {
 #endif
 
-#define STC_ABI_VERSION 37
+#define STC_ABI_VERSION 38
 #define STC_MAX_K 4
 
 #define STC_FMT_BF16X3 0
@@ -77,6 +77,16 @@
                               const float* Bm, const float* A, const float* U,
                               float* Cand, float* Hnew, float* SHnew,
                               int32_t batch, int32_t C, int32_t h, void* stream);
+int stc_ring2_sum_head_f32(const int32_t* l2_rows, const int32_t* l1_rows, const int32_t* int_rows, const int32_t* t1, const int32_t* t2,
+                           int32_t n_patches, int32_t n_rows,
+                           const float* A, int32_t n_add, const float* const* add, const float* g, const float* w,
+                           const float* U, const float* Cand, float* Y, float* Z,
+                           int32_t batch, int32_t C, int32_t h, void* stream);
+int stc_ring2_blend_head_f32(const int32_t* l2_rows, const int32_t* l1_rows, const int32_t* int_rows, const int32_t* t1, const int32_t* t2,
+                             int32_t n_patches, int32_t n_rows,
+                             const float* Bm, const float* A, const float* U, const float* H, const float* w, const float* b,
+                             float* Cand, float* Hnew, float* SHnew, float* y,
+                             int32_t batch, int32_t C, int32_t h, void* stream);
 int stc_ring2_chain_f32(const int32_t* l2_rows, const int32_t* l1_rows, const int32_t* int_rows, const int32_t* t1, const int32_t* t2,
                         int32_t n_patches, int32_t n_rows,
                         const float* A, const float* A2, float alpha1, int32_t n_add1, const float* const* add1, float* V,
@@ -288,6 +298,9 @@
 int stc_head_bwd_f32(const float* H, const float* w, const float* y, const float* dy,
                      float* dH, float* dwb, void* workspace, size_t workspace_bytes,
                      int64_t rows, int32_t h, void* stream);
+int stc_head_bwd_g_f32(const float* H, const float* w, const float* y, const float* dy,
+                       float* g, float* dH, int64_t dH_from_row, float* dwb, void* workspace, size_t workspace_bytes,
+                       int64_t rows, int32_t h, void* stream);
 
 int stc_cell_small_supported(int32_t Ks, int32_t Kc, int32_t C, int32_t cin, int32_t h);
 size_t stc_cell_small_workspace_bytes(int32_t n_nodes, int32_t C, int32_t cin, int32_t batch, int32_t Ks);
diff --git a/stc-gnn_amd/STC_GNN.py b/stc-gnn_amd/STC_GNN.py
--- a/stc-gnn_amd/STC_GNN.py
+++ b/stc-gnn_amd/STC_GNN.py
@@ -302,11 +302,11 @@
                     X_seq = X_seq.index_select(2, idx[0])
                     inv = idx[1]
         pair = _graphs(Gs, Gc, self.Ks, self.Kc)
-        stacked = self._run_cell_graph(pair, X_seq.unsqueeze(-1).to(self.storage_dtype))
+        stacked = self._run_cell_graph(pair, X_seq.unsqueeze(-1).to(self.storage_dtype), with_head=True)
         if stacked is None and self.storage_dtype != torch.float32:
             raise ValueError('storage_dtype=torch.bfloat16: shape outside the bf16 cell kernels (Ks = Kc = 2, hidden 16, C in {32, 64}, input_dim <= 4)')
         if stacked is not None:
-            y = self._head(stacked).transpose(0, 1)
+            y = (stacked if stacked.dim() == 4 else self._head(stacked)).transpose(0, 1)
         else:
             _, states = self.encoder._run(pair, None, X_seq.unsqueeze(-1))
             step_in = states[-1]
@@ -317,7 +317,7 @@
             y = self._head(torch.stack(outs, dim=1))
         return y if inv is None else y.index_select(2, inv)
 
-    def _run_cell_graph(self, pair: GraphPair, X: torch.Tensor):
+    def _run_cell_graph(self, pair: GraphPair, X: torch.Tensor, with_head: bool = False):
         enc, dec = self.encoder.cell_list, self.decoder.cell_list
         cells = list(enc) + list(dec)
         hidden = {c.hidden_dim for c in cells}
@@ -348,16 +348,19 @@
                 schedule.append((n_layers + l, x, hs))
         stacks = [(c.gates.W, c.gates.b if c.gates.use_bias else None, c.candi.W, c.candi.b if c.candi.use_bias else None) for c in cells]
         outputs = [did(n_layers - 1, s_) for s_ in range(horizon)]
-        return ops.stc_cell_graph(pair.spatial, pair.Tc, self.Ks, schedule, outputs, ext, stacks)
-
-    def _head(self, H: torch.Tensor) -> torch.Tensor:
+        head = self._folded_head(X.dtype) if with_head and ops.head_route(pair.spatial, pair.Tc, self.Ks, C, h, [cin0, h], dtype=X.dtype) else None
+        return ops.stc_cell_graph(pair.spatial, pair.Tc, self.Ks, schedule, outputs, ext, stacks, head=head)
+
+    def _folded_head(self, dtype):
         lin1, lin2 = self.out_proj[0], self.out_proj[1]
         h = lin1.in_features
-        if lin2.out_features != 1 or h % 4 or h > 64 or (H.dtype == torch.bfloat16 and h != 16):
+        if lin2.out_features != 1 or h % 4 or h > 64 or (dtype == torch.bfloat16 and h != 16):
+            return None
+        w = (lin2.weight @ lin1.weight).reshape(h)
+        return w, (lin2.weight @ lin1.bias + lin2.bias if lin1.bias is not None else w.new_zeros(1))
+
+    def _head(self, H: torch.Tensor) -> torch.Tensor:
+        folded = self._folded_head(H.dtype)
+        if folded is None:
             return torch.sigmoid(self.out_proj(H.float())).squeeze(dim=-1)
-        w = (lin2.weight @ lin1.weight).reshape(h)
-        if lin1.bias is not None:
-            b = lin2.weight @ lin1.bias + lin2.bias
-        else:
-            b = w.new_zeros(1)
-        return ops.head(H, w, b)
+        return ops.head(H, *folded)
diff --git a/stc-gnn_amd/csrc/stc_common.h b/stc-gnn_amd/csrc/stc_common.h
--- a/stc-gnn_amd/csrc/stc_common.h
+++ b/stc-gnn_amd/csrc/stc_common.h
@@ -109,6 +109,8 @@
     return fabsf(v) < 0.25f ? small : big;
 }
 
+__device__ __forceinline__ float stc_sigmoid_ieee(float x) { return 1.f / (1.f + expf(-x)); }
+
 __device__ __forceinline__ float stc_wave_sum(float v) {
 #pragma unroll
     for (int off = 32; off > 0; off >>= 1) v += __shfl_xor(v, off, 64);
diff --git a/stc-gnn_amd/csrc/stc_gates.hip b/stc-gnn_amd/csrc/stc_gates.hip
--- a/stc-gnn_amd/csrc/stc_gates.hip
+++ b/stc-gnn_amd/csrc/stc_gates.hip
@@ -12,7 +12,7 @@
     return dim3((unsigned)(blocks < cap ? (blocks > 0 ? blocks : 1) : cap));
 }
 
-__device__ __forceinline__ float sigmoidf_(float x) { return 1.f / (1.f + expf(-x)); }
+__device__ __forceinline__ float sigmoidf_(float x) { return stc_sigmoid_ieee(x); }
 
 __global__ __launch_bounds__(EW_THREADS) void gru_gates_fwd_kernel(
     const float* __restrict__ G, const float* __restrict__ Xt, const float* __restrict__ H,
@@ -258,6 +258,43 @@
         if (q < h4) {
             const float4 v = reinterpret_cast<const float4*>(H + r * h)[q];
             reinterpret_cast<float4*>(dH + r * h)[q] = make_float4(g * wq.x, g * wq.y, g * wq.z, g * wq.w);
+            acc.x = fmaf(g, v.x, acc.x); acc.y = fmaf(g, v.y, acc.y); acc.z = fmaf(g, v.z, acc.z); acc.w = fmaf(g, v.w, acc.w);
+        }
+    }
+    red[threadIdx.x][0] = acc.x; red[threadIdx.x][1] = acc.y; red[threadIdx.x][2] = acc.z; red[threadIdx.x][3] = acc.w;
+    red[threadIdx.x][4] = accg;
+    __syncthreads();
+    if ((int)threadIdx.x <= h) {
+        const int k = threadIdx.x;
+        const int lane_q = k < h ? k / 4 : 0, comp = k < h ? k % 4 : 4;
+        float v = 0.f;
+        for (int t = lane_q; t < EW_THREADS; t += LPR) v += red[t][comp];
+        partial[(size_t)blockIdx.x * (h + 1) + k] = v;
+    }
+}
+
+template <int LPR>
+__global__ __launch_bounds__(EW_THREADS) void head_bwd_g_kernel(const float* __restrict__ H, const float* __restrict__ w,
+                                                                 const float* __restrict__ y, const float* __restrict__ dy,
+                                                                 float* __restrict__ gout, float* __restrict__ dH, long long dH_from,
+                                                                 float* __restrict__ partial, long long rows, int h) {
+    constexpr int RPB = EW_THREADS / LPR;
+    __shared__ float red[EW_THREADS][5];
+    const int h4 = h / 4, q = threadIdx.x % LPR;
+    float4 wq = make_float4(0.f, 0.f, 0.f, 0.f);
+    if (q < h4) wq = reinterpret_cast<const float4*>(w)[q];
+    float4 acc = make_float4(0.f, 0.f, 0.f, 0.f);
+    float accg = 0.f;
+    for (long long r = (long long)blockIdx.x * RPB + threadIdx.x / LPR; r < rows; r += (long long)gridDim.x * RPB) {
+        const float yy = y[r];
+        const float g = dy[r] * yy * (1.f - yy);
+        if (q == 0) {
+            accg += g;
+            gout[r] = g;
+        }
+        if (q < h4) {
+            const float4 v = reinterpret_cast<const float4*>(H + r * h)[q];
+            if (r >= dH_from) reinterpret_cast<float4*>(dH + r * h)[q] = make_float4(g * wq.x, g * wq.y, g * wq.z, g * wq.w);
             acc.x = fmaf(g, v.x, acc.x); acc.y = fmaf(g, v.y, acc.y); acc.z = fmaf(g, v.z, acc.z); acc.w = fmaf(g, v.w, acc.w);
         }
     }
@@ -531,6 +568,32 @@
     return STC_OK;
 }
 
+extern "C" int stc_head_bwd_g_f32(const float* H, const float* w, const float* y, const float* dy, float* g, float* dH, int64_t dH_from_row,
+                                  float* dwb, void* workspace, size_t workspace_bytes, int64_t rows, int32_t h, void* stream) {
+    STC_REQUIRE(h == 16, STC_EUNSUPPORTED, "stc_head_bwd_g_f32: hidden width %d (built for 16)", h);
+    STC_REQUIRE(rows >= 0 && dwb, STC_EINVAL, "stc_head_bwd_g_f32: negative rows or null dwb");
+    STC_REQUIRE(dH_from_row >= 0 && dH_from_row <= rows, STC_EINVAL, "stc_head_bwd_g_f32: dH_from_row %lld outside [0, %lld]", (long long)dH_from_row,
+                (long long)rows);
+    hipStream_t s = static_cast<hipStream_t>(stream);
+    if (rows == 0) return stc::hip_status(hipMemsetAsync(dwb, 0, (size_t)(h + 1) * sizeof(float), s), "memset dwb");
+    STC_REQUIRE(H && w && y && dy && g && (dH || dH_from_row == rows), STC_EINVAL, "stc_head_bwd_g_f32: null pointer");
+    STC_REQUIRE(stc::aligned16(H) && stc::aligned16(dH) && workspace && stc::aligned16(workspace), STC_EALIGN,
+                "stc_head_bwd_g_f32: H/dH/workspace must be 16-byte aligned");
+    STC_REQUIRE(workspace_bytes >= stc_head_bwd_workspace_bytes(h), STC_EINVAL, "stc_head_bwd_g_f32: workspace too small");
+    STC_REQUIRE(stc::aligned16(w), STC_EALIGN, "stc_head_bwd_g_f32: w not 16-byte aligned");
+    STC_REQUIRE(reinterpret_cast<uintptr_t>(g) % 4 == 0, STC_EALIGN, "stc_head_bwd_g_f32: g not 4-byte aligned");
+    STC_REQUIRE(g != y && g != dy && g != H && g != w && dH != H && (const float*)dH != y && (const float*)dH != dy && dH != g, STC_EINVAL,
+                "stc_head_bwd_g_f32: g / dH alias an operand or each other");
+    constexpr int lpr = 4;
+    long long blocks = (rows * lpr + EW_THREADS - 1) / EW_THREADS;
+    const int grid = (int)(blocks < HEAD_PARTS ? blocks : HEAD_PARTS);
+    float* partial = static_cast<float*>(workspace);
+    hipLaunchKernelGGL(head_bwd_g_kernel<lpr>, dim3(grid), dim3(EW_THREADS), 0, s, H, w, y, dy, g, dH, (long long)dH_from_row, partial, (long long)rows, h);
+    hipLaunchKernelGGL(head_reduce_kernel, dim3(h + 1), dim3(EW_THREADS), 0, s, partial, grid, h + 1, dwb);
+    STC_LAUNCH_CHECK("stc_head_bwd_g_f32 launch");
+    return STC_OK;
+}
+
 extern "C" int stc_head_fwd_bf16(const void* H, const float* w, const float* b, float* y, int64_t rows, int32_t h, void* stream) {
     STC_REQUIRE(h == 16, STC_EUNSUPPORTED, "stc_head_fwd_bf16: hidden width %d (built for 16)", h);
     STC_EW_PROLOGUE("stc_head_fwd_bf16", rows, H && w && b && y);
diff --git a/stc-gnn_amd/csrc/stc_spmm_ring2.hip b/stc-gnn_amd/csrc/stc_spmm_ring2.hip
--- a/stc-gnn_amd/csrc/stc_spmm_ring2.hip
+++ b/stc-gnn_amd/csrc/stc_spmm_ring2.hip
@@ -30,16 +30,26 @@
     v4f *Y, *Y2, *Z;
     int n, F4;
     float alpha1, alpha2;
-    const v4f* add0[R2_MAX_ADD];
+    union {
+        const v4f* add0[R2_MAX_ADD];
+        struct { const float *hw, *hb, *hg; float* hy; };
+    };
     float scale0[R2_MAX_ADD];
 };
 
 enum { R2_SUM = 0, R2_BLEND = 1, R2_CHAIN = 2, R2_BLEND0 = 3 };
+enum { R2_HEAD_NONE = 0, R2_HEAD_G = 1, R2_HEAD_Y = 2 };
+
+__device__ __forceinline__ float mul_rounded(float a, float b) {
+#pragma clang fp contract(off)
+    return a * b;
+}
 
 __device__ __forceinline__ void lds_only_barrier() { asm volatile("s_waitcnt lgkmcnt(0)\n\ts_barrier" ::: "memory"); }
 
-template <int MODE, bool HAS_A2, int NADD, int N0 = 0>
+template <int MODE, bool HAS_A2, int NADD, int N0 = 0, int HEAD = R2_HEAD_NONE>
 __global__ __launch_bounds__(R2_THREADS, 2) void ring2_sum_kernel(Ring2Args a) {
+    static_assert(HEAD == R2_HEAD_NONE || (HEAD == R2_HEAD_G && MODE == R2_SUM) || (HEAD == R2_HEAD_Y && MODE == R2_BLEND), "the head rides in the sum or the blend form");
     static_assert((MODE != R2_BLEND && MODE != R2_BLEND0) || (NADD == 1 && !HAS_A2), "the blend forms: one addend (A), one gathered operand (Bm)");
     static_assert((MODE == R2_CHAIN) == (N0 > 0), "interior addends: the chain form, at least one");
     extern __shared__ __attribute__((aligned(16))) unsigned char lds[];
@@ -83,23 +93,36 @@
     };
     constexpr int NOP = MODE == R2_CHAIN ? NADD : MODE == R2_BLEND0 ? NADD + 1 : NADD + 2, NOPA = NOP > 0 ? NOP : 1;
     auto slot_at = [&](int i, int chunk) { return l1_off[i] + (unsigned)(chunk * R2_Q); };
-    auto request_slot = [&](v4f (&o)[NOPA], int i, int chunk) {
+    constexpr bool DEFER = HEAD == R2_HEAD_G && NADD == 2;
+    auto request_slot = [&](v4f (&o)[NOPA], float& g, int i, int chunk, int part = 0) {
         const unsigned at = slot_at(i, chunk);
-#pragma unroll
-        for (int k = 0; k < NADD; ++k) o[k] = a.add[k][at];
+        if (part != 2) {
+            if constexpr (HEAD == R2_HEAD_G) g = a.hg[at >> 2];
+#pragma unroll
+            for (int k = 0; k < NADD; ++k) o[k] = a.add[k][at];
+        }
         if constexpr (MODE != R2_CHAIN) {
-            o[NADD] = a.U[at];
-            if constexpr (MODE != R2_BLEND0) o[NADD + 1] = a.Cand[at];
+            if (part != 1) {
+                o[NADD] = a.U[at];
+                if constexpr (MODE != R2_BLEND0) o[NADD + 1] = a.Cand[at];
+            }
         }
     };
     v4f opn[NOPA];
+    float gn = 0.f, hbias = 0.f;
+    v4f wq = {0.f, 0.f, 0.f, 0.f};
+    if constexpr (HEAD != R2_HEAD_NONE) wq = *reinterpret_cast<const v4f*>(a.hw + 4 * (q & 3));
+    if constexpr (HEAD == R2_HEAD_Y) hbias = a.hb[0];
     request(0);
-    request_slot(opn, 0, 0);
+    request_slot(opn, gn, 0, 0);
     for (int chunk = 0; chunk < n_chunks; ++chunk) {
         if (chunk) lds_only_barrier();
 #pragma unroll
         for (int k = 0; k < R2_STAGE; ++k) tile[(k * 8 + hw) * R2_Q + q] = st[k];
         lds_only_barrier();
+        if constexpr (DEFER) {
+            if (chunk) request_slot(opn, gn, 0, chunk, 2);
+        }
         const bool more = chunk + 1 < n_chunks;
         v4f dy[R2_S1];
 #pragma unroll
@@ -109,11 +132,12 @@
             v4f cur[NOPA];
 #pragma unroll
             for (int k = 0; k < NOP; ++k) cur[k] = opn[k];
+            const float gcur = gn;
             if (i + 1 < R2_S1) {
-                request_slot(opn, i + 1, chunk);
+                request_slot(opn, gn, i + 1, chunk);
             } else if (more) {
                 request(chunk + 1);
-                request_slot(opn, 0, chunk + 1);
+                request_slot(opn, gn, 0, chunk + 1, DEFER ? 1 : 0);
             }
             v4f acc = {0.f, 0.f, 0.f, 0.f};
 #pragma unroll
@@ -127,14 +151,27 @@
             v4f dh = MODE == R2_CHAIN ? a.alpha1 * acc : acc;
 #pragma unroll
             for (int k = 0; k < NADD; ++k) dh += cur[k];
+            if constexpr (HEAD == R2_HEAD_G) {
+#pragma unroll
+                for (int c = 0; c < 4; ++c) dh[c] += mul_rounded(gcur, wq[c]);
+            }
             if constexpr (MODE == R2_CHAIN) {
                 if (a.Y != nullptr && interior) __builtin_nontemporal_store(dh, a.Y + slot_at(i, chunk));
                 dy[i] = dh;
             } else if constexpr (MODE == R2_SUM) {
                 const v4f u = cur[NOPA - 2], cd = cur[NOPA - 1];
                 if (interior) __builtin_nontemporal_store(dh, a.Y + slot_at(i, chunk));
-#pragma unroll
-                for (int c = 0; c < 4; ++c) dy[i][c] = dh[c] * u[c] * (1.f - cd[c] * cd[c]);
+                if constexpr (HEAD == R2_HEAD_G) {
+                    constexpr bool FUSED_FIRST = NADD != 0;
+#pragma unroll
+                    for (int c = 0; c < 4; ++c) {
+                        const float t = (FUSED_FIRST || i > 0) ? fmaf(-cd[c], cd[c], 1.f) : 1.f - mul_rounded(cd[c], cd[c]);
+                        dy[i][c] = dh[c] * u[c] * t;
+                    }
+                } else {
+#pragma unroll
+                    for (int c = 0; c < 4; ++c) dy[i][c] = dh[c] * u[c] * (1.f - cd[c] * cd[c]);
+                }
             } else {
                 const v4f u = cur[NADD], cd = MODE == R2_BLEND0 ? v4f{0.f, 0.f, 0.f, 0.f} : cur[NOPA - 1];
                 v4f cand;
@@ -148,6 +185,12 @@
                     if (a.Y != nullptr) __builtin_nontemporal_store(cand, a.Y + slot_at(i, chunk));
                     __builtin_nontemporal_store(dy[i], a.Y2 + slot_at(i, chunk));
                 }
+                if constexpr (HEAD == R2_HEAD_Y) {
+                    float s = fmaf(dy[i][0], wq[0], fmaf(dy[i][1], wq[1], fmaf(dy[i][2], wq[2], dy[i][3] * wq[3])));
+                    s += __shfl_xor(s, 2, 64);
+                    s += __shfl_xor(s, 1, 64);
+                    if (interior && (q & 3) == 0) a.hy[slot_at(i, chunk) >> 2] = stc_sigmoid_ieee(s + hbias);
+                }
             }
         }
         lds_only_barrier();
@@ -184,11 +227,18 @@
     }
 }
 
+using Kernel = void (*)(Ring2Args);
+
+int launch_ring2_kernel(Kernel kern, const Ring2Args& a, int batch, hipStream_t s) {
+    const size_t lds = (size_t)R2_L2 * R2_Q * 16 + (size_t)(R2_L1 + R2_INT) * R2_W * sizeof(int2);
+    static_assert((size_t)R2_L2 * R2_Q * 16 + (size_t)(R2_L1 + R2_INT) * R2_W * sizeof(int2) <= 64 * 1024, "within the default dynamic-LDS limit: no attribute to set");
+    const int per = (a.pl.n_patches + stc::kNumXcd - 1) / stc::kNumXcd;
+    hipLaunchKernelGGL(kern, dim3(per * stc::kNumXcd, batch), dim3(R2_THREADS), lds, s, a);
+    return stc::launched("stc_ring2 launch");
+}
+
 template <int MODE, bool HAS_A2>
 int launch_ring2(const Ring2Args& a, int batch, hipStream_t s, int n_add0 = 0) {
-    const size_t lds = (size_t)R2_L2 * R2_Q * 16 + (size_t)(R2_L1 + R2_INT) * R2_W * sizeof(int2);
-    static_assert((size_t)R2_L2 * R2_Q * 16 + (size_t)(R2_L1 + R2_INT) * R2_W * sizeof(int2) <= 64 * 1024, "within the default dynamic-LDS limit: no attribute to set");
-    using Kernel = void (*)(Ring2Args);
     Kernel kern = nullptr;
     if constexpr (MODE == R2_BLEND || MODE == R2_BLEND0) {
         kern = ring2_sum_kernel<MODE, false, 1>;
@@ -209,9 +259,7 @@
             default: kern = ring2_sum_kernel<R2_SUM, HAS_A2, 5>; break;
         }
     }
-    const int per = (a.pl.n_patches + stc::kNumXcd - 1) / stc::kNumXcd;
-    hipLaunchKernelGGL(kern, dim3(per * stc::kNumXcd, batch), dim3(R2_THREADS), lds, s, a);
-    return stc::launched("stc_ring2 launch");
+    return launch_ring2_kernel(kern, a, batch, s);
 }
 
 int check_ring2(const char* who, const void* l2_rows, const void* l1_rows, const void* int_rows, const void* t1, const void* t2, int n_patches, int n_rows,
@@ -230,7 +278,89 @@
 
 }
 
-#if !defined(STC_RING2_FIRST_UNIT)
+#if defined(STC_RING2_HEAD_UNIT)
+
+namespace {
+
+int check_head_operands(const char* who, const float* w, const float* x) {
+    STC_REQUIRE(w && x, STC_EINVAL, "%s: null pointer (head operand)", who);
+    STC_REQUIRE(stc::aligned16(w), STC_EALIGN, "%s: w not 16-byte aligned", who);
+    STC_REQUIRE(reinterpret_cast<uintptr_t>(x) % 4 == 0, STC_EALIGN, "%s: head operand not 4-byte aligned", who);
+    return STC_OK;
+}
+
+}
+
+extern "C" int stc_ring2_sum_head_f32(const int32_t* l2_rows, const int32_t* l1_rows, const int32_t* int_rows, const int32_t* t1, const int32_t* t2,
+                                      int32_t n_patches, int32_t n_rows,
+                                      const float* A, int32_t n_add, const float* const* add, const float* g, const float* w,
+                                      const float* U, const float* Cand, float* Y, float* Z,
+                                      int32_t batch, int32_t C, int32_t h, void* stream) {
+    const char* who = "stc_ring2_sum_head_f32";
+    if (int rc = stc::check_addend_count(who, "plane addend", n_add, 0, 2, STC_ELIMIT)) return rc;
+    if (int rc = check_ring2(who, l2_rows, l1_rows, int_rows, t1, t2, n_patches, n_rows, batch, C, h)) return rc;
+    if (batch == 0 || n_rows == 0) return STC_OK;
+    STC_REQUIRE(A && U && Cand && Y && Z && (n_add == 0 || add), STC_EINVAL, "%s: null pointer", who);
+    if (int rc = check_head_operands(who, w, g)) return rc;
+    STC_REQUIRE(stc::aligned16(A) && stc::aligned16(U) && stc::aligned16(Cand) && stc::aligned16(Y) && stc::aligned16(Z), STC_EALIGN,
+                "%s: planes must be 16-byte aligned", who);
+    STC_REQUIRE(Y != A && Z != A && Y != Z && Y != U && Y != Cand && Z != U && Z != Cand && (const float*)Y != g && (const float*)Z != g, STC_EINVAL,
+                "%s: results must not alias the gathered operand, the first ring's gate planes, g or each other", who);
+    Ring2Args a{};
+    a.pl = Ring2Plan{l2_rows, l1_rows, int_rows, t1, t2, n_patches};
+    a.A = reinterpret_cast<const v4f*>(A);
+    a.n_add = n_add;
+    if (int rc = stc::check_addends(who, "plane addend", add, n_add, Y, Z)) return rc;
+    for (int i = 0; i < n_add; ++i) a.add[i] = reinterpret_cast<const v4f*>(add[i]);
+    a.hg = g;
+    a.hw = w;
+    a.U = reinterpret_cast<const v4f*>(U);
+    a.Cand = reinterpret_cast<const v4f*>(Cand);
+    a.Y = reinterpret_cast<v4f*>(Y);
+    a.Z = reinterpret_cast<v4f*>(Z);
+    a.n = n_rows;
+    a.F4 = C * h / 4;
+    static constexpr Kernel table[3] = {ring2_sum_kernel<R2_SUM, false, 0, 0, R2_HEAD_G>, ring2_sum_kernel<R2_SUM, false, 1, 0, R2_HEAD_G>,
+                                        ring2_sum_kernel<R2_SUM, false, 2, 0, R2_HEAD_G>};
+    return launch_ring2_kernel(table[n_add], a, batch, static_cast<hipStream_t>(stream));
+}
+
+extern "C" int stc_ring2_blend_head_f32(const int32_t* l2_rows, const int32_t* l1_rows, const int32_t* int_rows, const int32_t* t1, const int32_t* t2,
+                                        int32_t n_patches, int32_t n_rows,
+                                        const float* Bm, const float* A, const float* U, const float* H, const float* w, const float* b,
+                                        float* Cand, float* Hnew, float* SHnew, float* y,
+                                        int32_t batch, int32_t C, int32_t h, void* stream) {
+    const char* who = "stc_ring2_blend_head_f32";
+    if (int rc = check_ring2(who, l2_rows, l1_rows, int_rows, t1, t2, n_patches, n_rows, batch, C, h)) return rc;
+    if (batch == 0 || n_rows == 0) return STC_OK;
+    STC_REQUIRE(Bm && A && U && H && Hnew && SHnew, STC_EINVAL, "%s: null pointer", who);
+    if (int rc = check_head_operands(who, w, b)) return rc;
+    if (int rc = check_head_operands(who, w, y)) return rc;
+    for (const void* q : {(const void*)Bm, (const void*)A, (const void*)U, (const void*)H, (const void*)Cand, (const void*)Hnew, (const void*)SHnew})
+        STC_REQUIRE(stc::aligned16(q), STC_EALIGN, "%s: planes must be 16-byte aligned", who);
+    for (const float* out : {Cand, Hnew, SHnew, y})
+        STC_REQUIRE(out != Bm && out != A && out != U && out != H && out != w && out != b, STC_EINVAL,
+                    "%s: a result aliases an operand (the first ring re-reads them)", who);
+    STC_REQUIRE(Cand != Hnew && Cand != SHnew && Hnew != SHnew && y != Cand && y != Hnew && y != SHnew, STC_EINVAL, "%s: results alias each other", who);
+    Ring2Args a{};
+    a.pl = Ring2Plan{l2_rows, l1_rows, int_rows, t1, t2, n_patches};
+    a.A = reinterpret_cast<const v4f*>(Bm);
+    a.n_add = 1;
+    a.add[0] = reinterpret_cast<const v4f*>(A);
+    a.U = reinterpret_cast<const v4f*>(U);
+    a.Cand = reinterpret_cast<const v4f*>(H);
+    a.hw = w;
+    a.hb = b;
+    a.Y = reinterpret_cast<v4f*>(Cand);
+    a.Y2 = reinterpret_cast<v4f*>(Hnew);
+    a.Z = reinterpret_cast<v4f*>(SHnew);
+    a.hy = y;
+    a.n = n_rows;
+    a.F4 = C * h / 4;
+    return launch_ring2_kernel(ring2_sum_kernel<R2_BLEND, false, 1, 0, R2_HEAD_Y>, a, batch, static_cast<hipStream_t>(stream));
+}
+
+#elif !defined(STC_RING2_FIRST_UNIT)
 
 extern "C" int stc_ring2_sum_f32(const int32_t* l2_rows, const int32_t* l1_rows, const int32_t* int_rows, const int32_t* t1, const int32_t* t2,
                                  int32_t n_patches, int32_t n_rows,
diff --git a/stc-gnn_amd/csrc/stc_spmm_ring2_head.hip b/stc-gnn_amd/csrc/stc_spmm_ring2_head.hip
--- /dev/null
+++ b/stc-gnn_amd/csrc/stc_spmm_ring2_head.hip
@@ -0,0 +1,2 @@
+#define STC_RING2_HEAD_UNIT
+#include "stc_spmm_ring2.hip"
diff --git a/stc-gnn_amd/stc_hip/_lib.py b/stc-gnn_amd/stc_hip/_lib.py
--- a/stc-gnn_amd/stc_hip/_lib.py
+++ b/stc-gnn_amd/stc_hip/_lib.py
@@ -10,7 +10,7 @@
 
 _PKG_ROOT = os.path.dirname(os.path.dirname(os.path.abspath(__file__)))
 LIB_PATH = os.path.join(_PKG_ROOT, 'libstc_hip.so')
-ABI_VERSION = 37
+ABI_VERSION = 38
 FMT_BF16X3, FMT_F16X2 = 0, 1
 MAX_K = 4
 SPMM_SUM_MAX_ADD, SPMM_SUM_BF16_MAX_ADD, RING2_MAX_ADD = 8, 5, 5
@@ -44,6 +44,8 @@
     'stc_ring2_sum_f32': (_int, [_p] * 5 + [_i32, _i32, _p, _p, _i32, _pp, _p, _p, _p, _p, _i32, _i32, _i32, _p]),
     'stc_ring2_blend_f32': (_int, [_p] * 5 + [_i32, _i32] + [_p] * 7 + [_i32, _i32, _i32, _p]),
     'stc_ring2_blend_first_f32': (_int, [_p] * 5 + [_i32, _i32] + [_p] * 6 + [_i32, _i32, _i32, _p]),
+    'stc_ring2_sum_head_f32': (_int, [_p] * 5 + [_i32, _i32, _p, _i32, _pp, _p, _p, _p, _p, _p, _p, _i32, _i32, _i32, _p]),
+    'stc_ring2_blend_head_f32': (_int, [_p] * 5 + [_i32, _i32] + [_p] * 10 + [_i32, _i32, _i32, _p]),
     'stc_ring2_chain_f32': (_int, [_p] * 5 + [_i32, _i32, _p, _p, _f32, _i32, _pp, _p, _f32, _i32, _pp, _pf, _p, _i32, _i32, _i32, _p]),
     'stc_spmm_blend_fwd_f32': (_int, [_p] * 6 + [_i32, _i32] + [_p] * 6 + [_p, _i32, _i32, _p, _i32, _p, _i32, _i32] + [_i32] * 3 + [_p]),
     'stc_spmm_blend_fwd_bf16': (_int, [_p] * 6 + [_i32, _i32] + [_p] * 6 + [_i32] * 3 + [_p]),
@@ -115,6 +117,7 @@
     'stc_head_bwd_workspace_bytes': (_size, [_i32]),
     'stc_head_bwd_f32': (_int, [_p, _p, _p, _p, _p, _p, _p, _size, _i64, _i32, _p]),
     'stc_head_bwd_bf16': (_int, [_p, _p, _p, _p, _p, _p, _p, _size, _i64, _i32, _p]),
+    'stc_head_bwd_g_f32': (_int, [_p, _p, _p, _p, _p, _p, _i64, _p, _p, _size, _i64, _i32, _p]),
     'stc_axpy_f32': (_int, [_f32, _p, _p, _i64, _p]),
     'stc_concat2_f32': (_int, [_p, _p, _p, _i64, _i32, _i32, _i32, _p]),
     'stc_split2_f32': (_int, [_p, _p, _p, _p, _p, _i64, _i32, _i32, _i32, _i32, _p, _p, _p]),
@@ -202,6 +205,7 @@
     patch_min_items = 1000
     optional_gate_stores = True
     first_step_cells = True
+    head_in_ring2 = True
 
     def __init__(self):
         self.lib = load_library()
@@ -404,6 +408,35 @@
                      _ptr(U), _ptr(Cand), _ptr(Y), _ptr(Z), B, Cc, h,
                      nbytes=colidx.numel() * 8 + 4 * (n + 1) + 4 * B * n * Cc * h * (1 + (X2 is not None) + len(addends) + 2 + 2))
 
+    def ring2_sum_head(self, rowptr, colidx, val, ring2, X, addends, g, w, U, Cand, Y, Z):
+        B, n, Cc, h = Y.shape
+        for name, t in (('Y', Y), ('Z', Z), ('X', X), ('U', U), ('Cand', Cand)):
+            _tensor('ring2_sum_head.' + name, t, (B, n, Cc, h))
+        _tensor('ring2_sum_head.g', g, (B, n, Cc))
+        _tensor('ring2_sum_head.w', w, (h,))
+        if len(addends) > 2:
+            raise StcError(f'ring2_sum_head: at most 2 plane addends, got {len(addends)}')
+        ptrs = (_p * 2)()
+        for i, t in enumerate(addends):
+            _tensor(f'ring2_sum_head.add{i}', t, (B, n, Cc, h))
+            ptrs[i] = t.data_ptr()
+        self._same_device(X, g, w, U, Cand, Y, Z, *addends)
+        self._launch('stc_ring2_sum_head_f32', Y, *self._ring2_ptrs('ring2_sum_head', ring2, Y), n, _ptr(X), len(addends), ptrs, _ptr(g), _ptr(w),
+                     _ptr(U), _ptr(Cand), _ptr(Y), _ptr(Z), B, Cc, h,
+                     nbytes=colidx.numel() * 8 + 4 * (n + 1) + 4 * B * n * Cc * (h * (1 + len(addends) + 2 + 2) + 1))
+
+    def ring2_blend_head(self, rowptr, colidx, val, ring2, Bm, A, U, H, w, b, Cand, Hnew, SHnew, y):
+        B, n, Cc, h = H.shape
+        for name, t in (('Bm', Bm), ('A', A), ('U', U), ('H', H), ('Hnew', Hnew), ('SHnew', SHnew)) + ((('Cand', Cand),) if Cand is not None else ()):
+            _tensor('ring2_blend_head.' + name, t, (B, n, Cc, h))
+        _tensor('ring2_blend_head.w', w, (h,))
+        _tensor('ring2_blend_head.b', b, (1,))
+        _tensor('ring2_blend_head.y', y, (B, n, Cc))
+        self._same_device(Bm, A, U, H, w, b, Cand, Hnew, SHnew, y)
+        self._launch('stc_ring2_blend_head_f32', H, *self._ring2_ptrs('ring2_blend_head', ring2, H), n, _ptr(Bm), _ptr(A), _ptr(U), _ptr(H), _ptr(w), _ptr(b),
+                     _ptr(Cand), _ptr(Hnew), _ptr(SHnew), _ptr(y), B, Cc, h,
+                     nbytes=colidx.numel() * 8 + 4 * (n + 1) + 4 * B * n * Cc * (h * (6 + (Cand is not None)) + 1))
+
     def _ring2_ptrs(self, what, ring2, on):
         l2, l1, own, t1, t2 = ring2
         n_p = l2.shape[0]
@@ -1315,6 +1348,20 @@
         self._launch('stc_head_bwd_bf16' if dt == torch.bfloat16 else 'stc_head_bwd_f32', H,
                      _ptr(H), _ptr(w), _ptr(y), _ptr(dy), _ptr(dH), _ptr(dwb), _ptr(ws), ws.numel(), rows, h)
 
+    def head_bwd_g(self, H, w, y, dy, g, dH, dH_from_row, dwb):
+        h = H.shape[-1]
+        rows = H.shape[:-1].numel()
+        _tensor('head.H', H)
+        _tensor('head.w', w, (h,))
+        for name, t in (('y', y), ('dy', dy), ('g', g)):
+            _tensor('head.' + name, t, tuple(H.shape[:-1]))
+        if dH is not None:
+            _tensor('head.dH', dH, tuple(H.shape))
+        _tensor('head.dwb', dwb, (h + 1,))
+        self._same_device(H, w, y, dy, g, dH, dwb)
+        ws = self._get_workspace(H.device, self.lib.stc_head_bwd_workspace_bytes(h))
+        self._launch('stc_head_bwd_g_f32', H, _ptr(H), _ptr(w), _ptr(y), _ptr(dy), _ptr(g), _ptr(dH), int(dH_from_row), _ptr(dwb), _ptr(ws), ws.numel(), rows, h)
+
     def axpy(self, a, x, y):
         n = self._same_numel('axpy', x, y)
         self._launch('stc_axpy_f32', x, float(a), _ptr(x), _ptr(y), n)
diff --git a/stc-gnn_amd/stc_hip/ops.py b/stc-gnn_amd/stc_hip/ops.py
--- a/stc-gnn_amd/stc_hip/ops.py
+++ b/stc-gnn_amd/stc_hip/ops.py
@@ -435,6 +435,8 @@
 _RING2 = True
 _RING2_FWD = True
 _FIRST_STEP = True
+_HEAD_IN_RING2 = True
+_HEAD_IN_RING2_FWD = True
 
 _ZEROS = {}
 
@@ -446,6 +448,16 @@
 def first_step_route(op: SpatialOperand, Tc, Ks: int, C: int, h: int, x_widths, dtype=torch.float32) -> bool:
     k = kernels()
     return Ks == 2 and _first_step_kernels(k, dtype, C, h) and not (_SMALL and small_graph_supported(k, op, Tc, Ks, C, h, x_widths, dtype))
+
+
+def _head_in_ring2(k, dtype, op: SpatialOperand, Ks: int, h: int) -> bool:
+    return bool(_HEAD_IN_RING2 and _RING2 and dtype == torch.float32 and getattr(k, 'head_in_ring2', False) and Ks == 2 and h == 16
+                and op.bwd_ring2 is not None and op.fwd_ring2 is not None and not op.ring2_clusters)
+
+
+def head_route(op: SpatialOperand, Tc, Ks: int, C: int, h: int, x_widths, dtype=torch.float32) -> bool:
+    k = kernels()
+    return _head_in_ring2(k, dtype, op, Ks, h) and not (_SMALL and small_graph_supported(k, op, Tc, Ks, C, h, x_widths, dtype))
 
 
 def zero_state(ref: torch.Tensor, shape, dtype=None) -> torch.Tensor:
@@ -549,6 +561,21 @@
         zero = {('ext', i) for i, t in enumerate(ext) if _is_zero_state(t)}
         can = _first_step_kernels(k, ext[0].dtype, self.C, self.h)
         self.first = [can and hs in zero and f is _Form.PLANAR_ONE_BWD for (_, _, hs), f in zip(schedule, forms)]
+        self.head = None
+
+    def take_head(self, w, b, out_slot):
+        y = self.ext[0].new_empty(len(out_slot), self.B, self.N, self.C)
+        self.head = (w, b, y, out_slot if _HEAD_IN_RING2_FWD else {}, set())
+        return y
+
+    def finish_head(self, out_stack):
+        w, b, y, _, done = self.head
+        todo = [i for i in range(y.shape[0]) if i not in done]
+        while todo:
+            n = next((m for m in range(1, len(todo)) if todo[m] != todo[0] + m), len(todo))
+            self.k.head_fwd(out_stack[todo[0]:todo[0] + n], w, b, y[todo[0]:todo[0] + n])
+            todo = todo[n:]
+        return y
 
     def source(self, src):
         if src[0] != 'ext':
@@ -640,6 +667,10 @@
             SHn = self.plane()
             if first:
                 k.ring2_blend_first(*self.graph[:3], op.fwd_ring2, Bm, A, U, Cand, Hnew, SHn)
+            elif self.head is not None and j in self.head[3]:
+                w, b, y, slot, done = self.head
+                k.ring2_blend_head(*self.graph[:3], op.fwd_ring2, Bm, A, U, Hprev, w, b, Cand, Hnew, SHn, y[slot[j]])
+                done.add(slot[j])
             else:
                 k.ring2_blend(*self.graph[:3], op.fwd_ring2, Bm, A, U, Hprev, Cand, Hnew, SHn)
             self.agg[('cell', j)] = SHn
@@ -706,6 +737,36 @@
         self.G = {}
         self.pieces = {}
         self.rows_of_set = {}
+        self.Gh, self.head_w = {}, None
+
+    def head_keeps(self, outputs):
+        consumers = {}
+        for d, (_, x, hs) in enumerate(self.schedule):
+            for src in {x, hs}:
+                if src[0] == 'cell':
+                    consumers.setdefault(src[1], []).append(d)
+        one = lambda c: self.forms[c] is _Form.PLANAR_ONE_BWD
+        ok = [bool(self.ring2 and one(j) and consumers.get(j) and all(one(d) for d in consumers[j])) for j in outputs]
+        return ok.index(False) if False in ok else len(ok)
+
+    def seed_head(self, outputs, out_stack, w, y, dy):
+        keep = self.head_keeps(outputs)
+        g, dwb = torch.empty_like(y), w.new_empty(w.numel() + 1)
+        dH = torch.empty_like(out_stack) if keep < len(outputs) else None
+        self.k.head_bwd_g(out_stack, w, y, dy, g, dH, keep * y[0].numel(), dwb)
+        self.head_w = w
+        for i, j in enumerate(outputs):
+            if i < keep:
+                self.Gh[j] = g[i]
+            else:
+                self.G[j] = dH[i]
+        return dwb
+
+    def head_plane(self, kid):
+        g = self.Gh.pop(kid, None)
+        if g is not None:
+            assert kid not in self.G
+            self.G[kid] = g.unsqueeze(-1) * self.head_w
 
     def grads_for(self, s_id):
         if s_id not in self.rows_of_set:
@@ -727,6 +788,7 @@
         pc['agg'].append(aggregated)
 
     def owed(self, kid, blend=None):
+        self.head_plane(kid)
         base = self.G.pop(kid, None)
         pc = self.pieces.pop(kid, None)
         if pc is None:
@@ -754,12 +816,16 @@
         if not self.ring2 or pc is None:
             return None
         add = pc['direct'] + ([self.G[kid]] if kid in self.G else [])
-        if len(add) > 2 or len(pc['agg']) != 1:
+        g = self.Gh.get(kid)
+        if len(add) + (g is not None) > 2 or len(pc['agg']) != 1:
             return None
         self.G.pop(kid, None)
         self.pieces.pop(kid)
         out, dBm_ = torch.empty_like(pc['agg'][0]), torch.empty_like(pc['agg'][0])
-        self.k.ring2_sum(*self.graph[:3], self.op.bwd_ring2, pc['agg'][0], None, add, U_, Cand_, out, dBm_)
+        if g is not None:
+            self.k.ring2_sum_head(*self.graph[:3], self.op.bwd_ring2, pc['agg'][0], add, self.Gh.pop(kid), self.head_w, U_, Cand_, out, dBm_)
+        else:
+            self.k.ring2_sum(*self.graph[:3], self.op.bwd_ring2, pc['agg'][0], None, add, U_, Cand_, out, dBm_)
         return out, dBm_
 
     def leave3(self, kid, d0, d1, d2):
@@ -921,14 +987,16 @@
     return p, stacks, out_stack, _out_slots(outputs)
 
 
-def _forward_only(op: SpatialOperand, Ks: int, schedule, outputs, n_ext: int, Tc, fwd_val, tensors):
+def _forward_only(op: SpatialOperand, Ks: int, schedule, outputs, n_ext: int, Tc, fwd_val, tensors, head=None):
     p, stacks, out_stack, out_slot = _begin_forward(op, Ks, schedule, outputs, n_ext, Tc, fwd_val, tensors, forward_only=True)
+    if head is not None:
+        p.take_head(_c(head[0]), _c(head[1]), out_slot)
     order = p.wavefront()
     last = p.last_uses(order)
     for j in order:
         p.cell(j, stacks[schedule[j][0]], out_stack[out_slot[j]] if j in out_slot else None)
         p.release(j, last, out_slot)
-    return out_stack
+    return out_stack if head is None else p.finish_head(out_stack)
 
 
 class _StcCellGraph(Function):
@@ -948,50 +1016,94 @@
     @staticmethod
     @once_differentiable
     def backward(ctx, grad_stack):
-        k = kernels().for_graph(_amplification(ctx.meta[0], ctx.meta[1]))
-        bf16 = grad_stack.dtype == torch.bfloat16
-        if bf16:
-            k = k.bf16
-        op, Ks, schedule, outputs, cin, n_sets, dims, forms = ctx.meta
         _check_guard(ctx)
-        Tc, *sv = ctx.saved_tensors
-        stacks, sv = _stacks(sv[:4 * n_sets]), sv[4 * n_sets:]
-        cells = []
-        for f in forms:
-            cells, sv = cells + [sv[:f.saved(Ks)]], sv[f.saved(Ks):]
-        p = _BackwardPass(k, op, Ks, Tc, schedule, stacks, cin, forms, dims, bf16, ctx.zmax_all)
-        grad_stack = _c(grad_stack)
-        for i, j in enumerate(outputs):
-            p.G[j] = grad_stack[i]
-        acc = [[None] * 4 for _ in stacks]
-
-        def add_to(s_id, grads):
-            acc[s_id] = [a if t is None else t if a is None else a.add_(t) for a, t in zip(acc[s_id], grads)]
-
-        for j in range(len(schedule) - 1, -1, -1):
-            if j not in p.G and j not in p.pieces:
-                continue
-            s_id, f = schedule[j][0], forms[j]
-            run = {_Form.PLANAR3: p.planar3, _Form.PLANAR_ONE_BWD: p.planar_one_bwd, _Form.PLANAR: p.planar}.get(f, p.rows_cell)
-            grads = run(j, *stacks[s_id], cells[j])
-            if not f.planar:
-                add_to(s_id, grads)
-        for s_id, (buf, _, _) in p.rows_of_set.items():
-            add_to(s_id, p.param_views(s_id, buf[0] if buf.shape[0] == 1 else buf.sum(0)))
-        flat = [None if prm is None else (g if g is not None else torch.zeros_like(prm)) for st, a in zip(stacks, acc) for prm, g in zip(st, a)]
+
+        def seed(p, outputs, rest):
+            for i, j in enumerate(outputs):
+                p.G[j] = grad_stack_c[i]
+
+        grad_stack_c = _c(grad_stack)
+        flat = _cell_graph_backward(ctx, grad_stack.dtype == torch.bfloat16, ctx.saved_tensors, seed)
         n_ext = len(ctx.needs_input_grad) - 7 - len(flat)
         return (None,) * 7 + (None,) * n_ext + tuple(flat)
 
 
-def stc_cell_graph(op: SpatialOperand, Tc, Ks: int, schedule, outputs, ext, stacks):
+def _cell_graph_backward(ctx, bf16: bool, saved_tensors, seed):
+    k = kernels().for_graph(_amplification(ctx.meta[0], ctx.meta[1]))
+    if bf16:
+        k = k.bf16
+    op, Ks, schedule, outputs, cin, n_sets, dims, forms = ctx.meta
+    Tc, *sv = saved_tensors
+    stacks, sv = _stacks(sv[:4 * n_sets]), sv[4 * n_sets:]
+    cells = []
+    for f in forms:
+        cells, sv = cells + [sv[:f.saved(Ks)]], sv[f.saved(Ks):]
+    p = _BackwardPass(k, op, Ks, Tc, schedule, stacks, cin, forms, dims, bf16, ctx.zmax_all)
+    seed(p, outputs, sv)
+    acc = [[None] * 4 for _ in stacks]
+
+    def add_to(s_id, grads):
+        acc[s_id] = [a if t is None else t if a is None else a.add_(t) for a, t in zip(acc[s_id], grads)]
+
+    for j in range(len(schedule) - 1, -1, -1):
+        if j not in p.G and j not in p.Gh and j not in p.pieces:
+            continue
+        s_id, f = schedule[j][0], forms[j]
+        run = {_Form.PLANAR3: p.planar3, _Form.PLANAR_ONE_BWD: p.planar_one_bwd, _Form.PLANAR: p.planar}.get(f, p.rows_cell)
+        grads = run(j, *stacks[s_id], cells[j])
+        if not f.planar:
+            add_to(s_id, grads)
+    for s_id, (buf, _, _) in p.rows_of_set.items():
+        add_to(s_id, p.param_views(s_id, buf[0] if buf.shape[0] == 1 else buf.sum(0)))
+    return [None if prm is None else (g if g is not None else torch.zeros_like(prm)) for st, a in zip(stacks, acc) for prm, g in zip(st, a)]
+
+
+class _StcCellGraphHead(Function):
+
+    @staticmethod
+    def forward(ctx, op: SpatialOperand, Ks: int, schedule, outputs, n_ext: int, Tc, fwd_val, w, b, *tensors):
+        p, stacks, out_stack, out_slot = _begin_forward(op, Ks, schedule, outputs, n_ext, Tc, fwd_val, tensors)
+        w, b = _c(w), _c(b)
+        p.take_head(w, b, out_slot)
+        saved = []
+        for j, (s_id, _, _) in enumerate(schedule):
+            saved += p.cell(j, stacks[s_id], _alias(out_stack, out_slot[j]) if j in out_slot else None)
+        y = p.finish_head(out_stack)
+        ctx.save_for_backward(p.Tc, *[t for st in stacks for t in st], *saved, out_stack, w, y)
+        ctx.meta = (op, Ks, schedule, tuple(outputs), p.cin, len(stacks), (p.B, p.N, p.C), p.forms)
+        ctx.zmax_all = p.zmax_all
+        return y
+
+    @staticmethod
+    @once_differentiable
+    def backward(ctx, dy):
+        dwb = []
+
+        def seed(p, outputs, rest):
+            out_stack, w, y = rest
+            dwb.append(p.seed_head(outputs, out_stack, w, y, _c(dy)))
+
+        flat = _cell_graph_backward(ctx, False, ctx.saved_tensors, seed)
+        n_ext = len(ctx.needs_input_grad) - 9 - len(flat)
+        return (None,) * 7 + (dwb[0][:-1], dwb[0][-1:]) + (None,) * n_ext + tuple(flat)
+
+
+def stc_cell_graph(op: SpatialOperand, Tc, Ks: int, schedule, outputs, ext, stacks, head=None):
     k = kernels()
-    if _SMALL and small_graph_supported(k, op, Tc, Ks, ext[0].shape[2], 16, {ext[x[1]].shape[-1] if x[0] == 'ext' else 16 for _, x, _ in schedule},
-                                        ext[0].dtype):
+    small = _SMALL and small_graph_supported(k, op, Tc, Ks, ext[0].shape[2], 16, {ext[x[1]].shape[-1] if x[0] == 'ext' else 16 for _, x, _ in schedule},
+                                             ext[0].dtype)
+    if head is not None and (small or not _head_in_ring2(k, ext[0].dtype, op, Ks, 16)):
+        return _Head.apply(stc_cell_graph(op, Tc, Ks, schedule, outputs, ext, stacks), *head)
+    if small:
         return stc_small_graph(k, op, Tc, Ks, schedule, outputs, ext, stacks)
     flat = [p for st in stacks for p in st]
-    if not torch.is_grad_enabled() or not any(t is not None and t.requires_grad for t in (Tc, op.fwd_val, *ext, *flat)):
+    if head is not None and (head[0].shape != (16,) or head[1].shape != (1,)):
+        raise ValueError(f'stc_cell_graph: head w {tuple(head[0].shape)} / b {tuple(head[1].shape)}, expected (16,) and (1,)')
+    if not torch.is_grad_enabled() or not any(t is not None and t.requires_grad for t in (Tc, op.fwd_val, *ext, *flat, *(head or ()))):
         with torch.no_grad():
-            return _forward_only(op, Ks, list(schedule), list(outputs), len(ext), Tc, op.fwd_val, (*ext, *flat))
+            return _forward_only(op, Ks, list(schedule), list(outputs), len(ext), Tc, op.fwd_val, (*ext, *flat), head=head)
+    if head is not None:
+        return _StcCellGraphHead.apply(op, Ks, list(schedule), list(outputs), len(ext), Tc, op.fwd_val, *head, *ext, *flat)
     return _StcCellGraph.apply(op, Ks, list(schedule), list(outputs), len(ext), Tc, op.fwd_val, *ext, *flat)
 
 
```

New measurement: 32.31 samples/s, median of 6. No clear change (+0.7%).
